# fbreitwieser/krakenuniq

Hardware: AMD Instinct MI355X
Metric: Mreads/s (150 bp) (higher is better)
Workload: dtype u64

## Files before the change

krakenuniq_amd/capi.py:

```python
from __future__ import annotations

import ctypes as C
import os

import numpy as np

_HERE = os.path.dirname(os.path.abspath(__file__))
LIB_PATH = os.environ.get("KU_LIB") or os.path.join(_HERE, "libkrakenuniq_amd.so")


def _hw_queues():
    try:
        have = int(os.environ.get("GPU_MAX_HW_QUEUES", "0"))
    except ValueError:
        have = 0
    try:
        want = int(os.environ["KU_HW_QUEUES"]) if "KU_HW_QUEUES" in os.environ else max(have, 8)
    except ValueError:
        want = max(have, 8)
    os.environ["GPU_MAX_HW_QUEUES"] = str(min(max(want, 4), 32))


_hw_queues()

# ... 231 lines not shown

    def __init__(self, kdb=None, idx=None, pairs=None, key_ct=None, k=None, offsets=None, nt=None, idx_type=2):
        self.h = C.c_void_p()
        if kdb is not None:
            _chk(lib().ku_db_open(kdb.encode(), idx.encode(), C.byref(self.h)), "ku_db_open")
        else:
            self._keep = (pairs, offsets)
            _chk(lib().ku_db_wrap(pairs.ctypes.data, key_ct, k, offsets.ctypes.data, nt, idx_type, C.byref(self.h)),
                 "ku_db_wrap")
        self.info = DbInfo()
        _chk(lib().ku_db_get_info(self.h, C.byref(self.info)), "ku_db_get_info")

    def close(self):
        if self.h and _lib is not None:
            _lib.ku_db_close(self.h)
            self.h = C.c_void_p()

    __del__ = close

    def shard_plan(self, n):
        b = np.zeros(n + 1, dtype=np.uint64)
        _chk(lib().ku_db_shard_plan(self.h, n, _p(b, u64p)), "ku_db_shard_plan")
        return b

    def chunk_plan(self, max_bytes, cap=4096):
        b = np.zeros(cap + 1, dtype=np.uint64)
        n = C.c_uint32()
        _chk(lib().ku_db_chunk_plan(self.h, max_bytes, _p(b, u64p), cap, C.byref(n)), "ku_db_chunk_plan")
        return b[:n.value + 1]

    def values(self):
        n = C.c_uint64()
        _chk(lib().ku_db_values(self.h, None, C.byref(n)), "ku_db_values")
        out = np.zeros(max(n.value, 1), dtype=np.uint32)
        n2 = C.c_uint64(len(out))
        _chk(lib().ku_db_values(self.h, _p(out, u32p), C.byref(n2)), "ku_db_values")
        return out[:n2.value]


class Tax:

    def __init__(self, path=None, ids=None, parents=None):
        self.h = C.c_void_p()
        if path is not None:
            _chk(lib().ku_tax_open(path.encode(), C.byref(self.h)), "ku_tax_open")
        else:
            ids = np.ascontiguousarray(ids, dtype=np.uint32)
            parents = np.ascontiguousarray(parents, dtype=np.uint32)
            _chk(lib().ku_tax_from_arrays(_p(ids, u32p), _p(parents, u32p), len(ids), C.byref(self.h)),
                 "ku_tax_from_arrays")

    def ids(self):
        out = np.zeros(max(int(lib().ku_tax_size(self.h)), 1), dtype=np.uint32)
        _chk(lib().ku_tax_ids(self.h, _p(out, u32p)), "ku_tax_ids")
        return out[:int(lib().ku_tax_size(self.h))]

    def close(self):
        if self.h and _lib is not None:
            _lib.ku_tax_close(self.h)
            self.h = C.c_void_p()

    __del__ = close

    def parent(self, taxid):
        return lib().ku_tax_parent(self.h, taxid)

    def __len__(self):
        return lib().ku_tax_size(self.h)


class UidMap:

    def __init__(self, path=None, blocks=None):
        self.h = C.c_void_p()
        if path is not None:
            _chk(lib().ku_uid_map_open(path.encode(), C.byref(self.h)), "ku_uid_map_open")
        else:
            b = np.ascontiguousarray(blocks, dtype=np.uint32).reshape(-1)
            _chk(lib().ku_uid_map_from_blocks(_p(b, u32p), len(b) // 2, C.byref(self.h)), "ku_uid_map_from_blocks")

    def __len__(self):
        return int(lib().ku_uid_map_size(self.h))

    def close(self):
        if self.h:
            lib().ku_uid_map_close(self.h)
            self.h = C.c_void_p()

    def __del__(self):
        try:
            self.close()
        except Exception:
            pass


def resolve_uids(tax, uid_map, rle, lens, k, n_threads=1):
    runs = np.ascontiguousarray(rle["runs"], dtype=np.uint32)
    roff = np.ascontiguousarray(rle["run_off"], dtype=np.uint64)
    rcnt = np.ascontiguousarray(rle["run_cnt"], dtype=np.uint32)
    lens = np.ascontiguousarray(lens, dtype=np.uint32)
    calls = np.zeros(max(len(lens), 1), dtype=np.uint32)
    _chk(lib().ku_resolve_uids(tax.h, uid_map.h, runs.ctypes.data, _p(roff, u64p), _p(rcnt, u32p), _p(lens, u32p), len(lens), k,
                               n_threads, _p(calls, u32p)), "ku_resolve_uids")
    return calls[:len(lens)]


class Ctx:

    def __init__(self, device=0, borrowed=None):
        self._keep = []
        self._borrowed = borrowed is not None
        if borrowed is not None:
            self.h = C.c_void_p(borrowed)
            return
        self.h = C.c_void_p()
        _chk(lib().ku_ctx_create(device, C.byref(self.h)), "ku_ctx_create")

    def close(self):
        if getattr(self, "h", None) and _lib is not None and not getattr(self, "_borrowed", False):
            _lib.ku_ctx_destroy(self.h)
        self.h = C.c_void_p()

    __del__ = close

    def load_db(self, db: Db, bin_lo=0, bin_hi=None):
        if bin_hi is None:
            bin_hi = db.info.n_bins
        _chk(lib().ku_ctx_load_db(self.h, db.h, bin_lo, bin_hi), "ku_ctx_load_db")

    def swap_shard(self, db: Db, bin_lo, bin_hi):
        _chk(lib().ku_ctx_swap_shard(self.h, db.h, int(bin_lo), int(bin_hi)), "ku_ctx_swap_shard")

    def prefetch_shard(self, db: Db, bin_lo, bin_hi):
        _chk(lib().ku_ctx_prefetch_shard(self.h, db.h, int(bin_lo), int(bin_hi)), "ku_ctx_prefetch_shard")

    def batch(self, buf, off, lens):
        return Batch(self, buf, off, lens)

    def add_db(self, db: Db):
        _chk(lib().ku_ctx_add_db(self.h, db.h), "ku_ctx_add_db")

    def adopt_db(self, d_pairs_ptr, n_pairs, d_offsets_ptr, k, nt, idx_type=2, bin_lo=0, bin_hi=None, keep=None):
        if bin_hi is None:
            bin_hi = 4 ** nt
        self._keep.append(keep)
        _chk(lib().ku_ctx_adopt_db(self.h, d_pairs_ptr, n_pairs, d_offsets_ptr, k, nt, idx_type, bin_lo, bin_hi),
             "ku_ctx_adopt_db")

    def db_layout(self):
        h, b = C.c_uint32(), C.c_uint64()
        _chk(lib().ku_ctx_db_layout(self.h, C.byref(h), C.byref(b)), "ku_ctx_db_layout")
        return {"hash": bool(h.value), "resident_bytes": b.value}

    def db_values(self):
        n = C.c_uint64()
        _chk(lib().ku_ctx_db_values(self.h, None, C.byref(n)), "ku_ctx_db_values")
        out = np.zeros(max(n.value, 1), dtype=np.uint32)
        n2 = C.c_uint64(len(out))
        _chk(lib().ku_ctx_db_values(self.h, _p(out, u32p), C.byref(n2)), "ku_ctx_db_values")
        return out[:n2.value]

    def set_taxonomy(self, tax: Tax, all_values=None):
        if all_values is None:
            _chk(lib().ku_ctx_set_taxonomy(self.h, tax.h, None, 0), "ku_ctx_set_taxonomy")
        else:
            v = np.ascontiguousarray(all_values, dtype=np.uint32)
            _chk(lib().ku_ctx_set_taxonomy(self.h, tax.h, _p(v, u32p), len(v)), "ku_ctx_set_taxonomy")

    def count_taxons(self, db_index=0):
        n = C.c_uint64()
        _chk(lib().ku_ctx_count_taxons_db(self.h, db_index, None, None, C.byref(n)), "ku_ctx_count_taxons_db")
        t = np.zeros(max(n.value, 1), dtype=np.uint32)
        c = np.zeros(max(n.value, 1), dtype=np.uint64)
        n2 = C.c_uint64(len(t))
        _chk(lib().ku_ctx_count_taxons_db(self.h, db_index, _p(t, u32p), _p(c, u64p), C.byref(n2)), "ku_ctx_count_taxons_db")
        return t[:n2.value], c[:n2.value]

    def enable_exact(self, capacity_log2=20):
        _chk(lib().ku_ctx_enable_exact(self.h, capacity_log2), "ku_ctx_enable_exact")

    def exact_counts(self):
        d = CountsDims()
        _chk(lib().ku_counts_dims_get(self.h, C.byref(d)), "ku_counts_dims_get")
        out = np.zeros(d.n_slots, dtype=np.uint64)
        _chk(lib().ku_counts_export_exact(self.h, _p(out, u64p)), "ku_counts_export_exact")
        return out

    def reset_counts(self):
        _chk(lib().ku_ctx_reset_counts(self.h), "ku_ctx_reset_counts")

    def enable_sparse(self, work_unit_nt=500000, global_log2=0):
        _chk(lib().ku_ctx_enable_sparse(self.h, work_unit_nt, global_log2), "ku_ctx_enable_sparse")

    def disable_sparse(self):
        _chk(lib().ku_ctx_disable_sparse(self.h), "ku_ctx_disable_sparse")

    def sparse_close_unit(self):
        _chk(lib().ku_sparse_close_unit(self.h), "ku_sparse_close_unit")

    def sparse_state(self):
        return lib().ku_ctx_sparse_state(self.h)

    def report(self, tax: "Tax", counts_paths=(), flags=0):
        out, n = C.c_void_p(), C.c_size_t()
        paths = (C.c_char_p * len(counts_paths))(*[p.encode() for p in counts_paths])
        if flags:
            _chk(lib().ku_ctx_report_cols(self.h, tax.h, paths, len(counts_paths), flags, C.byref(out), C.byref(n)), "ku_ctx_report_cols")
        else:
            _chk(lib().ku_ctx_report(self.h, tax.h, paths, len(counts_paths), C.byref(out), C.byref(n)), "ku_ctx_report")
        s = C.string_at(out, n.value).decode()
        lib().ku_free(out)
        return s

    def sparse_export(self):
        d = CountsDims()
        _chk(lib().ku_counts_dims_get(self.h, C.byref(d)), "ku_counts_dims_get")
        flags = np.zeros(d.n_slots, dtype=np.uint8)
        n = C.c_uint64()
        _chk(lib().ku_sparse_export(self.h, _p(flags, u8p), None, C.byref(n)), "ku_sparse_export")
        pairs = np.zeros(max(n.value, 1), dtype=np.uint64)
        n2 = C.c_uint64(len(pairs))
        _chk(lib().ku_sparse_export(self.h, _p(flags, u8p), _p(pairs, u64p), C.byref(n2)), "ku_sparse_export")
        return flags, pairs[:n2.value]

    def classify_batch(self, buf, off, lens, flags=0, min_hits=1, want_taxa=True):
        arr = np.frombuffer(buf, dtype=np.uint8) if isinstance(buf, (bytes, bytearray)) else buf
        off = np.ascontiguousarray(off, dtype=np.uint64)
        lens = np.ascontiguousarray(lens, dtype=np.uint32)
        n = len(lens)
        calls = np.zeros(max(n, 1), dtype=np.uint32)
        hits = np.zeros(max(n, 1), dtype=np.uint32)
        taxa = np.zeros(max(len(arr), 1), dtype=np.uint32) if want_taxa else None
        o = Opts(flags, min_hits, 0, 0)
        _chk(lib().ku_classify_batch(self.h, arr.ctypes.data, len(arr), _p(off, u64p), _p(lens, u32p), n, C.byref(o),
                                     _p(calls, u32p), _p(taxa, u32p), _p(hits, u32p)), "ku_classify_batch")
        return {"calls": calls[:n], "taxa": taxa, "hits": hits[:n]}

    def classify_batch_rle(self, buf, off, lens, flags=0, min_hits=1, out=None):
        arr = np.frombuffer(buf, dtype=np.uint8) if isinstance(buf, (bytes, bytearray)) else buf
        off = np.ascontiguousarray(off, dtype=np.uint64)
        lens = np.ascontiguousarray(lens, dtype=np.uint32)
        n = len(lens)
        out = out or {}
        calls = out["calls"] if "calls" in out else np.zeros(max(n, 1), dtype=np.uint32)
        hits = out["hits"] if "hits" in out else np.zeros(max(n, 1), dtype=np.uint32)
        roff = out["run_off"] if "run_off" in out else np.zeros(max(n, 1), dtype=np.uint64)
        rcnt = out["run_cnt"] if "run_cnt" in out else np.zeros(max(n, 1), dtype=np.uint32)
        o = Opts(flags, min_hits, 0, 0)
        total = C.c_uint64()
        _chk(lib().ku_classify_batch_rle(self.h, arr.ctypes.data, len(arr), _p(off, u64p), _p(lens, u32p), n, C.byref(o),
                                         _p(calls, u32p), _p(hits, u32p), _p(roff, u64p), _p(rcnt, u32p),
                                         C.byref(total)), "ku_classify_batch_rle")
        runs = out.get("runs")
        if runs is None or len(runs) < total.value:
            runs = np.zeros((max(total.value, 1), 2), dtype=np.uint32)
        _chk(lib().ku_fetch_runs(self.h, runs.ctypes.data, total.value), "ku_fetch_runs")
        return {"calls": calls[:n], "hits": hits[:n], "runs": runs[:total.value], "run_off": roff[:n], "run_cnt": rcnt[:n]}

    def replace_calls(self, new_calls):
        nc = np.ascontiguousarray(new_calls, dtype=np.uint32)
        dropped = C.c_uint64()
        _chk(lib().ku_ctx_replace_calls(self.h, _p(nc, u32p), len(nc), C.byref(dropped)), "ku_ctx_replace_calls")
        return int(dropped.value)

    def lookup_device(self, d_seqs, n_bytes, d_taxa, flags=0, stream=None):
        o = Opts(flags, 1, 0, 0)
        _chk(lib().ku_lookup_device(self.h, d_seqs, n_bytes, C.byref(o), d_taxa, stream), "ku_lookup_device")

    def resolve_device(self, d_seqs, d_off, d_len, n_reads, d_calls, d_taxa, d_hits=None, flags=0, min_hits=1,
                       max_read_len=0, stream=None):
        o = Opts(flags, min_hits, max_read_len, 0)
        _chk(lib().ku_resolve_device(self.h, d_seqs, d_off, d_len, n_reads, C.byref(o), d_calls, d_taxa, d_hits,
                                     stream), "ku_resolve_device")

    def rle_enqueue(self, buf, off, lens, flags=0, min_hits=1, runs_cap=0, out=None):
        arr = np.ascontiguousarray(np.frombuffer(buf, dtype=np.uint8) if isinstance(buf, (bytes, bytearray)) else buf, dtype=np.uint8)
        off = np.ascontiguousarray(off, dtype=np.uint64)
        lens = np.ascontiguousarray(lens, dtype=np.uint32)
        n = len(off)
        out = out or {}
        job = {"arr": arr, "off": off, "lens": lens, "n": n,
               "calls": out["calls"] if "calls" in out else np.zeros(max(n, 1), np.uint32),
               "hits": out["hits"] if "hits" in out else np.zeros(max(n, 1), np.uint32),
               "run_off": out["run_off"] if "run_off" in out else np.zeros(max(n, 1), np.uint64),
               "run_cnt": out["run_cnt"] if "run_cnt" in out else np.zeros(max(n, 1), np.uint32)}
        o = Opts(flags, min_hits, 0, 0)
        job["runs"] = out["runs"] if "runs" in out else (np.zeros((runs_cap, 2), np.uint32) if runs_cap else None)
        rc = len(job["runs"]) if job["runs"] is not None else 0
        _chk(lib().ku_classify_batch_rle_enqueue(self.h, arr.ctypes.data, len(arr), _p(off, u64p), _p(lens, u32p), n, C.byref(o),
                                                 _p(job["calls"], u32p), _p(job["hits"], u32p), _p(job["run_off"], u64p),
                                                 _p(job["run_cnt"], u32p), job["runs"].ctypes.data if rc else None, rc),
             "ku_classify_batch_rle_enqueue")
        return job

    def rle_finish(self, job):
        total = C.c_uint64(0)
        _chk(lib().ku_classify_batch_rle_finish(self.h, C.byref(total)), "ku_classify_batch_rle_finish")
        if job.get("runs") is not None and total.value <= lib().ku_classify_batch_rle_copied(self.h):
            runs = job["runs"][:total.value]
        else:
            runs = np.zeros((total.value, 2), np.uint32)
            _chk(lib().ku_fetch_runs(self.h, runs.ctypes.data, total.value), "ku_fetch_runs")
        n = job.get("n", len(job.get("calls", ())))
        return {"calls": job["calls"][:n], "hits": job["hits"][:n], "run_off": job["run_off"][:n], "run_cnt": job["run_cnt"][:n], "runs": runs}

    def rle_in_flight(self):
# ... 533 lines not shown
```

krakenuniq_amd/csrc/ku_api.cpp:

```cpp
#include "ku_build.h"
#include "ku_ctx.h"

static thread_local std::string g_last_error;
void ku_set_error(const std::string &s) { g_last_error = s; }

extern "C" const char *ku_strerror(int status) {
  switch (status) {
    case KU_OK: return "ok";
    case KU_EINVAL: return "invalid argument";
    case KU_EDATA: return "malformed database / index / taxonomy data";
    case KU_ENOINPUT: return "cannot open input";
    case KU_ENOMEM: return "out of memory";
    case KU_EHIP: return "HIP runtime error or no usable gfx950 device";
    case KU_ESTATE: return "call order violated";
    case KU_EUNSUP: return "not supported by this build";
    default: return "unknown status";
  }
}
extern "C" const char *ku_last_error(void) { return g_last_error.c_str(); }
extern "C" int ku_abi_version(void) { return KU_ABI_VERSION; }
extern "C" int ku_device_count(void) {
  int n = 0;
  if (hipGetDeviceCount(&n) != hipSuccess) return 0;
  return n;
// ... 131 lines not shown
  uint64_t last_dbx = 0;
  while (idx_pos < nb) {
    uint64_t first = idx_pos, count = nb - idx_pos;
    const uint64_t orig = idx_pos, data0 = db->offsets[orig];
    while (count > 0) {
      uint64_t step = count / 2, it = first + step;
      uint64_t size_index = (it + 1 - orig) * 8;
      uint64_t size_data = (db->offsets[it + 1] - data0) * ps;
      if (size_index + size_data + 8 <= max_bytes) { first = it + 1; count -= step + 1; }
      else count = step;
    }
    if (first == idx_pos) return fail(KU_EINVAL, "preload size too small for the largest minimizer bin");
    idx_pos = first;
    uint64_t dbx = db->offsets[idx_pos];
    if (dbx == last_dbx) continue;
    last_dbx = dbx;
    ++n;
    if (n <= cap) bounds[n] = idx_pos;
  }
  *n_chunks = n;
  return n <= cap ? KU_OK : fail(KU_EINVAL, "ku_db_chunk_plan: bounds array too small");
}

int ku_db_raw(const ku_db *db, const uint8_t **pairs, const uint64_t **offsets) {
  if (!db || !pairs || !offsets) return KU_EINVAL;
  *pairs = db->pairs;
  *offsets = db->offsets;
  return KU_OK;
}

extern "C" int ku_db_values(const ku_db *db, uint32_t *out, uint64_t *n) {
  if (!db || !n) return fail(KU_EINVAL, "ku_db_values: null argument");
  std::lock_guard<std::mutex> lk(db->values_mu);
  if (!db->values_ready) {
    const uint64_t np = db->info.key_ct, ps = db->info.key_len + 4, kl = db->info.key_len;
    constexpr uint32_t SMALL = 1u << 26;
    std::vector<std::atomic<uint64_t>> bits(SMALL / 64);
    for (auto &w : bits) w.store(0, std::memory_order_relaxed);
    unsigned nthr = std::max(1u, std::min(16u, std::thread::hardware_concurrency()));
    if (np < (1u << 20)) nthr = 1;
    std::vector<std::vector<uint32_t>> large(nthr);
    std::vector<std::thread> team;
    for (unsigned t = 0; t < nthr; ++t)
      team.emplace_back([&, t] {
        const uint64_t lo = np * t / nthr, hi = np * (t + 1) / nthr;
        uint32_t last = 0;
        for (uint64_t i = lo; i < hi; ++i) {
          uint32_t v;
          memcpy(&v, db->pairs + i * ps + kl, 4);
          if (v == last) continue;
          last = v;
          if (v >= SMALL) {
            large[t].push_back(v);
            if (large[t].size() >= (1u << 20)) {
              std::sort(large[t].begin(), large[t].end());
              large[t].erase(std::unique(large[t].begin(), large[t].end()), large[t].end());
            }
            continue;
          }
          std::atomic<uint64_t> &w = bits[v >> 6];
          const uint64_t m = 1ull << (v & 63);
          if (!(w.load(std::memory_order_relaxed) & m)) w.fetch_or(m, std::memory_order_relaxed);
        }
      });
    for (auto &th : team) th.join();
    std::vector<uint32_t> &vals = db->values;
    for (uint64_t wi = 0; wi < bits.size(); ++wi) {
      uint64_t w = bits[wi].load(std::memory_order_relaxed);
      if (wi == 0) w &= ~1ull;
      while (w) {
        vals.push_back((uint32_t)(wi * 64 + (uint64_t)__builtin_ctzll(w)));
        w &= w - 1;
      }
    }
    const size_t n_small = vals.size();
    for (auto &l : large) vals.insert(vals.end(), l.begin(), l.end());
    std::sort(vals.begin() + n_small, vals.end());
    vals.erase(std::unique(vals.begin() + n_small, vals.end()), vals.end());
    db->values_ready = true;
  }
  const uint64_t count = db->values.size();
  if (out) {
    if (count > *n) return fail(KU_EINVAL, "ku_db_values: output array too small");
    memcpy(out, db->values.data(), count * 4);
  }
  *n = count;
  return KU_OK;
}

extern "C" int ku_tax_open(const char *path, ku_tax **out) {
  if (!path || !out) return fail(KU_EINVAL, "ku_tax_open: null argument");
  *out = nullptr;
  FILE *f = fopen(path, "r");
  if (!f) return fail(KU_ENOINPUT, std::string("unable to open taxonomy index file ") + path);
  ku_tax *t = new ku_tax();
  char *line = nullptr;
  size_t lcap = 0;
  ssize_t ll;
  while ((ll = getline(&line, &lcap, f)) > 0) {
    if (line[ll - 1] == '\n') line[--ll] = 0;
    if (ll == 0) continue;
    char *p = line, *end;
    unsigned long id = strtoul(p, &end, 10);
    if (end == p) continue;
    p = end;
    unsigned long par = strtoul(p, &end, 10);
    if (end == p) continue;
    p = end;
    if (*p) ++p;
    char *tab = strchr(p, '\t');
    std::string name, rank;
    if (tab) { name.assign(p, tab - p); rank.assign(tab + 1); } else name.assign(p);
    if ((uint32_t)id > 1 && id == par) {
      free(line); fclose(f); delete t;
      return fail(KU_EDATA, "taxDB: the parent of " + std::to_string(id) + " is itself");
    }
    t->add((uint32_t)id, (uint32_t)par, name, rank);
  }
  free(line);
  fclose(f);
  t->add(0, 0, "unclassified", "no rank");
  t->finish();
  *out = t;
  return KU_OK;
}

extern "C" int ku_tax_from_arrays(const uint32_t *ids, const uint32_t *parents, uint64_t n, ku_tax **out) {
  if (!out || (n && (!ids || !parents))) return fail(KU_EINVAL, "ku_tax_from_arrays: null argument");
  ku_tax *t = new ku_tax();
  for (uint64_t i = 0; i < n; ++i) t->add(ids[i], parents[i], "", "");
  t->add(0, 0, "unclassified", "no rank");
  t->finish();
  *out = t;
  return KU_OK;
}
extern "C" void ku_tax_close(ku_tax *t) { delete t; }
extern "C" uint64_t ku_tax_size(const ku_tax *t) { return t ? t->ids.size() : 0; }
extern "C" int ku_tax_ids(const ku_tax *t, uint32_t *ids) {
  if (!t || (!ids && !t->ids.empty())) return fail(KU_EINVAL, "ku_tax_ids: null argument");
  if (!t->ids.empty()) memcpy(ids, t->ids.data(), t->ids.size() * 4);
  return KU_OK;
}
extern "C" uint32_t ku_tax_parent(const ku_tax *t, uint32_t taxid) {
  if (!t || taxid == 0) return KU_AMBIG;
  auto it = t->row.find(taxid);
  return it == t->row.end() ? KU_AMBIG : t->parent_map[it->second];
}

hipStream_t ku_ctx_stream_of(ku_ctx *ctx) { return ctx->stream; }
unsigned long long *ku_ctx_exact_unique_of(ku_ctx *ctx) { return ctx->d_exact_unique; }
int ku_ctx_device_of(const ku_ctx *ctx) { return ctx->device; }
int ku_ctx_cus_of(const ku_ctx *ctx) { return ctx->n_cu; }
uint32_t ku_ctx_k_of(const ku_ctx *ctx) { return ctx->m.db.k; }

int ctx_activate(ku_ctx *ctx) {
  if (hipSetDevice(ctx->device) != hipSuccess) return fail(KU_EHIP, "hipSetDevice failed");
  return KU_OK;
}

extern "C" int ku_ctx_create(int device, ku_ctx **out) {
  if (!out) return fail(KU_EINVAL, "ku_ctx_create: null argument");
  *out = nullptr;
  KU_TRY(ku_check_device(device));
  hipDeviceProp_t prop;
  HIP_TRY(hipGetDeviceProperties(&prop, device));
  if (strncmp(prop.gcnArchName, "gfx950", 6) != 0)
    return fail(KU_EHIP, std::string("device is ") + prop.gcnArchName + ", this library is built for gfx950 only");
  ku_ctx *ctx = new ku_ctx();
  ctx->device = device;
  ctx->n_cu = prop.multiProcessorCount > 0 ? prop.multiProcessorCount : 256;
  HIP_TRY(hipSetDevice(device));
  HIP_TRY(hipStreamCreateWithFlags(&ctx->stream, hipStreamNonBlocking));
  HIP_TRY(hipMalloc((void **)&ctx->d_scalar, 128));
  if (const char *e = getenv("KU_LAYOUT")) ctx->hash_layout = strcmp(e, "sorted") != 0;
  if (const char *e = getenv("KU_LOAD_FACTOR")) {
    double f = atof(e);
    if (f >= 0.05 && f <= 0.9) { ctx->load_factor = f; ctx->load_factor_set = true; }
  }
  *out = ctx;
  return KU_OK;
}

void store_free(DbStore &d) {
  if (d.d_table) (void)hipFree(d.d_table);
  if (d.db_owned && d.d_pairs) (void)hipFree(d.d_pairs);
  if (d.offsets_owned && d.d_offsets) (void)hipFree(d.d_offsets);
  d = DbStore{};
}
void ctx_drop_count_cache(ku_ctx *ctx) {
  ctx->count_cache.clear();
  ctx->count_cache_store = ctx->count_cache_pairs = nullptr;
  ctx->count_cache_lines = 0;
}
static void ctx_free_db(ku_ctx *ctx) {
  ctx_drop_count_cache(ctx);
  if (ctx->pf.valid) store_free(ctx->pf.store);
  ctx->pf.valid = false;
  store_free(ctx->m);
  for (DbStore &e : ctx->extra) store_free(e);
  ctx->extra.clear();
  ctx->db_loaded = false;
}
void ctx_free_sparse(ku_ctx *ctx) {
  KuSparseDev &d = ctx->sp.dev;
  for (void *p : {(void *)d.l_key, (void *)d.l_first, (void *)d.u_key, (void *)d.u_distinct, (void *)d.u_last, (void *)d.u_maxfirst,
                  (void *)d.g_key, (void *)d.dense, (void *)d.err, (void *)ctx->sp.d_counters})
    if (p) (void)hipFree(p);
  for (DevBuf *b : {&ctx->sp.unit, &ctx->sp.carry_l, &ctx->sp.carry_u, &ctx->sp.out, &ctx->sp.u_cnt, &ctx->sp.u_flag, &ctx->sp.list, &ctx->sp.tail_row,
                    &ctx->sp.t_seqs, &ctx->sp.t_off, &ctx->sp.t_len, &ctx->sp.t_taxa, &ctx->sp.t_unit})
    b->release();
  ctx->sp = ku_ctx::Sparse{};
}
int sparse_give_up(ku_ctx *ctx, hipStream_t also) {
  (void)ctx_sync_all_streams(ctx);
  if (also) (void)hipStreamSynchronize(also);
  (void)hipGetLastError();
  ctx_free_sparse(ctx);
  ctx->sp.gave_up = true;
  return KU_OK;
}
static void ctx_free_tax(ku_ctx *ctx) {
  for (uint32_t **p : {&ctx->d_node_parent, &ctx->d_node_slot, &ctx->d_node_taxid, &ctx->d_slot_node, &ctx->d_slot_taxid,
                       &ctx->d_slot_anc_off, &ctx->d_slot_anc}) {
    if (*p) (void)hipFree(*p);
    *p = nullptr;
  }
  if (ctx->cnt.registers) (void)hipFree(ctx->cnt.registers);
  if (ctx->cnt.hll_floor) (void)hipFree(ctx->cnt.hll_floor);
  if (ctx->cnt.n_kmers) (void)hipFree(ctx->cnt.n_kmers);
  if (ctx->cnt.n_reads) (void)hipFree(ctx->cnt.n_reads);
  if (ctx->d_exact_set) (void)hipFree(ctx->d_exact_set);
  if (ctx->d_exact_unique) (void)hipFree(ctx->d_exact_unique);
  ctx->d_exact_set = ctx->d_exact_unique = nullptr;
  ctx->exact_mask = 0;
  ctx_free_sparse(ctx);
  ctx->cnt = KuCountsDev{};
  ctx->tax_set = false;
}

int ctx_sync_all_streams(ku_ctx *ctx) {
  int st = KU_OK;
  for (hipStream_t s : {ctx->stream, ctx->k_streams[0], ctx->k_streams[1], ctx->h2d_stream, ctx->d2h_stream, ctx->fetch_stream, ctx->pf.stream})
    if (s && hipStreamSynchronize(s) != hipSuccess && st == KU_OK) st = fail(KU_EHIP, "ku_ctx_synchronize: a stream of the context failed");
  return st;
}

extern "C" void ku_ctx_destroy(ku_ctx *ctx) {
  if (!ctx) return;
  rle_times_print();
  (void)hipSetDevice(ctx->device);
  (void)ctx_sync_all_streams(ctx);
  ctx_free_db(ctx);
  ctx_free_tax(ctx);
  for (DevBuf *b : {&ctx->b_seqs, &ctx->b_off, &ctx->b_len, &ctx->b_calls, &ctx->b_taxa, &ctx->b_hits, &ctx->b_ws, &ctx->b_runs,
                    &ctx->b_roff, &ctx->b_rcnt})
    b->release();
  if (ctx->d_scalar) (void)hipFree(ctx->d_scalar);
  if (ctx->pf.d_scalar) (void)hipFree(ctx->pf.d_scalar);
  if (ctx->pf.stream) (void)hipStreamDestroy(ctx->pf.stream);
  for (RleJob &j : ctx->rle) j.release();
  if (ctx->h2d_stream) (void)hipStreamDestroy(ctx->h2d_stream);
  if (ctx->d2h_stream) (void)hipStreamDestroy(ctx->d2h_stream);
  for (hipStream_t &ks : ctx->k_streams) if (ks) { (void)hipStreamDestroy(ks); ks = nullptr; }
  if (ctx->main_ev) (void)hipEventDestroy(ctx->main_ev);
  if (ctx->fetch_stream) (void)hipStreamDestroy(ctx->fetch_stream);
  if (ctx->stream) (void)hipStreamDestroy(ctx->stream);
  delete ctx;
}

static int store_scan_values(ku_ctx *ctx, DbStore &d) {
  d.values.clear();
  uint32_t *d_bitmap = nullptr, *d_list = nullptr, *d_count = ctx->d_scalar;
  const uint32_t cap = 1u << 24;
  HIP_TRY(hipMalloc((void **)&d_bitmap, 1ull << 29));
  if (hipMalloc((void **)&d_list, (size_t)cap * 4) != hipSuccess) { (void)hipFree(d_bitmap); return fail(KU_ENOMEM, "hipMalloc values list"); }
  int st = KU_OK;
  uint32_t count = 0;
  if (hipMemsetAsync(d_bitmap, 0, 1ull << 29, ctx->stream) != hipSuccess ||
      hipMemsetAsync(d_count, 0, 4, ctx->stream) != hipSuccess)
    st = fail(KU_EHIP, "memset failed");
  if (st == KU_OK) st = ku_launch_mark_values(d.d_pairs, d.db.n_pairs, d_bitmap, ctx->stream);
  if (st == KU_OK) st = ku_launch_collect_values(d_bitmap, d_list, cap, d_count, ctx->stream);
  if (st == KU_OK && hipMemcpyAsync(&count, d_count, 4, hipMemcpyDeviceToHost, ctx->stream) != hipSuccess) st = fail(KU_EHIP, "memcpy failed");
  if (st == KU_OK && hipStreamSynchronize(ctx->stream) != hipSuccess) st = fail(KU_EHIP, "value scan kernel failed");
  if (st == KU_OK && count > cap) st = fail(KU_EUNSUP, "more than 2^24 distinct taxids in the database");
  if (st == KU_OK) {
    d.values.resize(count);
    if (count && hipMemcpy(d.values.data(), d_list, (size_t)count * 4, hipMemcpyDeviceToHost) != hipSuccess) st = fail(KU_EHIP, "memcpy failed");
    std::sort(d.values.begin(), d.values.end());
    if (!d.values.empty() && d.values[0] == 0) d.values.erase(d.values.begin());
  }
  (void)hipFree(d_bitmap);
  (void)hipFree(d_list);
  return st;
}

static void fill_db_dev(DbStore &d, uint64_t n_pairs, uint64_t pair_base, uint32_t k, uint32_t nt, uint32_t idx_type,
                        uint64_t bin_lo, uint64_t bin_hi) {
  d.db.pairs = d.d_pairs;
  d.db.table = nullptr;
  d.db.n_lines = 0;
  d.db.offsets = d.d_offsets;
  d.db.pair_base = pair_base;
  d.db.n_pairs = n_pairs;
  d.db.bin_lo = bin_lo;
  d.db.bin_hi = bin_hi;
  d.db.k = k;
  d.db.nt = nt;
  d.db.xor_mask = idx_type == 1 ? 0u : ku_index2_xor_mask(nt);
}

int store_upload(ku_ctx *ctx, DbStore &d, const ku_db *db, uint64_t bin_lo, uint64_t bin_hi, bool scan_values, hipStream_t stream) {
  if (!stream) stream = ctx->stream;
  const uint64_t p0 = db->offsets[bin_lo], p1 = db->offsets[bin_hi], np = p1 - p0;
  const uint32_t kl = db->info.key_len, ps = kl + 4;
  HIP_TRY(hipMalloc((void **)&d.d_pairs, std::max<uint64_t>(np, 1) * 12));
  d.db_owned = true;
  if (kl == 8) {
    if (np) HIP_TRY(hipMemcpy(d.d_pairs, db->pairs + p0 * 12, np * 12, hipMemcpyHostToDevice));
  } else if (np) {
    void *d_raw = nullptr;
    HIP_TRY(hipMalloc(&d_raw, np * ps));
    hipError_t e = hipMemcpy(d_raw, db->pairs + p0 * ps, np * ps, hipMemcpyHostToDevice);
    int st = e == hipSuccess ? ku_launch_repack((const uint8_t *)d_raw, np, kl, d.d_pairs, stream) : KU_EHIP;
    if (st == KU_OK && hipStreamSynchronize(stream) != hipSuccess) st = KU_EHIP;
    (void)hipFree(d_raw);
    if (st != KU_OK) return fail(st, "pair repack failed");
  }
  const uint64_t no = bin_hi - bin_lo + 1;
  HIP_TRY(hipMalloc((void **)&d.d_offsets, no * 8));
  d.offsets_owned = true;
  HIP_TRY(hipMemcpy(d.d_offsets, db->offsets + bin_lo, no * 8, hipMemcpyHostToDevice));
  fill_db_dev(d, np, p0, db->info.k, db->info.nt, db->info.idx_type, bin_lo, bin_hi);
  return scan_values ? store_scan_values(ctx, d) : KU_OK;
}

extern "C" int ku_ctx_load_db(ku_ctx *ctx, const ku_db *db, uint64_t bin_lo, uint64_t bin_hi) {
  if (!ctx || !db) return fail(KU_EINVAL, "ku_ctx_load_db: null argument");
  KU_TRY(rle_idle(ctx, "ku_ctx_load_db"));
  if (bin_lo > bin_hi || bin_hi > db->info.n_bins) return fail(KU_EINVAL, "bin range out of bounds");
  KU_TRY(ctx_activate(ctx));
  ctx_free_tax(ctx);
  ctx_free_db(ctx);
  KU_TRY(store_upload(ctx, ctx->m, db, bin_lo, bin_hi));
  ctx->db_loaded = true;
  return KU_OK;
}

bool store_whole(const DbStore &d) { return d.db.bin_lo == 0 && d.db.bin_hi == (1ull << (2 * d.db.nt)); }

extern "C" int ku_ctx_add_db(ku_ctx *ctx, const ku_db *db) {
  if (!ctx || !db) return fail(KU_EINVAL, "ku_ctx_add_db: null argument");
  KU_TRY(rle_idle(ctx, "ku_ctx_add_db"));
  if (!ctx->db_loaded) return fail(KU_ESTATE, "load the first database before adding further ones");
  if (ctx->tax_set) return fail(KU_ESTATE, "add every database before the taxonomy is set");
  if (db->info.k != ctx->m.db.k)
    return fail(KU_EINVAL, "different k-mer sizes in the databases: " + std::to_string(ctx->m.db.k) + " vs " + std::to_string(db->info.k));
  if (!store_whole(ctx->m)) return fail(KU_EUNSUP, "hierarchical multi-database runs need the first database resident as a whole");
  if (ctx->extra.size() >= 7) return fail(KU_EUNSUP, "at most 8 databases");
  KU_TRY(ctx_activate(ctx));
  ctx->extra.emplace_back();
  int st = store_upload(ctx, ctx->extra.back(), db, 0, db->info.n_bins);
  if (st != KU_OK) { store_free(ctx->extra.back()); ctx->extra.pop_back(); }
  return st;
}

extern "C" int ku_ctx_adopt_db(ku_ctx *ctx, void *d_pairs, uint64_t n_pairs, const uint64_t *d_offsets, uint32_t k,
                               uint32_t nt, uint32_t idx_type, uint64_t bin_lo, uint64_t bin_hi) {
  if (!ctx || (!d_pairs && n_pairs) || !d_offsets) return fail(KU_EINVAL, "ku_ctx_adopt_db: null argument");
  KU_TRY(rle_idle(ctx, "ku_ctx_adopt_db"));
  if (k < 1 || k > 31 || nt < 1 || nt > 15 || nt > k || (idx_type != 1 && idx_type != 2) || bin_lo > bin_hi ||
      bin_hi > (1ull << (2 * nt)))
    return fail(KU_EINVAL, "ku_ctx_adopt_db: bad geometry");
  KU_TRY(ctx_activate(ctx));
  ctx_free_tax(ctx);
  ctx_free_db(ctx);
  ctx->m.d_pairs = (uint32_t *)d_pairs;
  ctx->m.d_offsets = const_cast<uint64_t *>(d_offsets);
  uint64_t pair_base = 0;
  HIP_TRY(hipMemcpy(&pair_base, d_offsets, 8, hipMemcpyDeviceToHost));
  fill_db_dev(ctx->m, n_pairs, pair_base, k, nt, idx_type, bin_lo, bin_hi);
  ctx->db_loaded = true;
  return store_scan_values(ctx, ctx->m);
}

extern "C" int ku_ctx_db_layout(ku_ctx *ctx, uint32_t *is_hash, uint64_t *resident_bytes) {
  if (!ctx) return fail(KU_EINVAL, "null context");
  if (!ctx->db_loaded) return fail(KU_ESTATE, "no database loaded");
  const bool hash = ctx->m.db.table != nullptr;
  if (is_hash) *is_hash = hash ? 1u : 0u;
  if (resident_bytes)
    *resident_bytes = (hash ? ctx->m.db.n_lines * 128 : ctx->m.db.n_pairs * 12) + (ctx->m.db.bin_hi - ctx->m.db.bin_lo + 1) * 8;
  return KU_OK;
}

static std::vector<uint32_t> ctx_all_values(const ku_ctx *ctx) {
  std::vector<uint32_t> v(ctx->m.values);
  for (const DbStore &e : ctx->extra) v.insert(v.end(), e.values.begin(), e.values.end());
  std::sort(v.begin(), v.end());
  v.erase(std::unique(v.begin(), v.end()), v.end());
  return v;
}

extern "C" int ku_ctx_db_values(ku_ctx *ctx, uint32_t *out, uint64_t *n) {
  if (!ctx || !n) return fail(KU_EINVAL, "ku_ctx_db_values: null argument");
  if (!ctx->db_loaded) return fail(KU_ESTATE, "no database loaded");
  const std::vector<uint32_t> v = ctx_all_values(ctx);
  if (out) {
    if (*n < v.size()) return fail(KU_EINVAL, "output array too small");
    if (!v.empty()) memcpy(out, v.data(), v.size() * 4);
  }
  *n = v.size();
  return KU_OK;
}

template <typename T> static int upload(T **dst, const std::vector<T> &src) {
  HIP_TRY(hipMalloc((void **)dst, std::max<size_t>(src.size(), 1) * sizeof(T)));
  if (!src.empty()) HIP_TRY(hipMemcpy(*dst, src.data(), src.size() * sizeof(T), hipMemcpyHostToDevice));
  return KU_OK;
}

int store_finalize(ku_ctx *ctx, DbStore &d, hipStream_t stream, uint32_t *d_scalar) {
  if (!stream) stream = ctx->stream;
  if (!d_scalar) d_scalar = ctx->d_scalar;
  HIP_TRY(hipMemsetAsync(d_scalar, 0, 4, stream));
  KU_TRY(ku_launch_remap_values(d.d_pairs, d.db.n_pairs, ctx->d_slot_taxid, ctx->tax.n_slots, d_scalar, stream));
  uint32_t err = 0;
  HIP_TRY(hipMemcpyAsync(&err, d_scalar, 4, hipMemcpyDeviceToHost, stream));
  HIP_TRY(hipStreamSynchronize(stream));
  if (err) return fail(KU_EDATA, "internal: " + std::to_string(err) + " DB values missing from the slot table");
  d.hash_layout = ctx->hash_layout;
  if (d.hash_layout) {
    uint64_t n_lines = 0;
    size_t free_b = 0, total_b = 0;
    (void)hipMemGetInfo(&free_b, &total_b);
    std::vector<double> chain;
    if (ctx->load_factor_set) chain.push_back(ctx->load_factor);
    else if ((double)d.db.n_pairs / 0.2 / 8.0 * 128.0 <= 0.4 * (double)free_b) chain.push_back(0.2);
    for (double lf : {0.3, 0.45, 0.6, 0.8})
      if (chain.empty() || lf > chain.back()) chain.push_back(lf);
    for (double lf : chain) {
      n_lines = (uint64_t)((double)d.db.n_pairs / lf / 8.0) + 1;
      if (n_lines >= (1ull << 32)) { n_lines = 0; continue; }
      if (hipMalloc(&d.d_table, n_lines * 128) == hipSuccess) { d.table_lines = n_lines; break; }
      (void)hipGetLastError();
      d.d_table = nullptr;
      n_lines = 0;
    }
    if (!d.d_table) d.hash_layout = false;
  }
  d.slot_counts.clear();
  if (d.hash_layout && d.db.n_pairs) {
    unsigned long long *d_c = nullptr;
    const uint32_t ns = ctx->tax.n_slots;
    if (hipMalloc((void **)&d_c, (size_t)ns * 8) == hipSuccess) {
      std::vector<unsigned long long> h(ns);
      const bool ok = hipMemsetAsync(d_c, 0, (size_t)ns * 8, stream) == hipSuccess &&
                      ku_launch_count_slots(d.d_pairs, d.db.n_pairs, d_c, ns, stream) == KU_OK &&
                      hipMemcpyAsync(h.data(), d_c, (size_t)ns * 8, hipMemcpyDeviceToHost, stream) == hipSuccess &&
                      hipStreamSynchronize(stream) == hipSuccess;
      (void)hipFree(d_c);
      if (ok) d.slot_counts.swap(h);
      else (void)hipGetLastError();
    } else (void)hipGetLastError();
  }
  if (d.hash_layout) {
    const uint64_t n_lines = d.table_lines;
    unsigned long long *d_dup = (unsigned long long *)(d_scalar + 2);
    HIP_TRY(hipMemsetAsync(d_dup, 0, 8, stream));
    KU_TRY(ku_launch_build_table(d.d_pairs, d.db.n_pairs, d.d_table, n_lines, d.db.k, d.db.nt, d.db.xor_mask, d_dup,
                                 stream));
    unsigned long long dup = 0;
    HIP_TRY(hipMemcpyAsync(&dup, d_dup, 8, hipMemcpyDeviceToHost, stream));
    HIP_TRY(hipStreamSynchronize(stream));
    d.n_dup = dup;
    d.db.table = (const uint4 *)d.d_table;
    d.db.n_lines = n_lines;
    if (d.db_owned) (void)hipFree(d.d_pairs);
    d.d_pairs = nullptr;
    d.db_owned = false;
    d.db.pairs = nullptr;
  }
  return KU_OK;
}

extern "C" int ku_ctx_set_taxonomy(ku_ctx *ctx, const ku_tax *tax, const uint32_t *all_values, uint64_t n_values) {
  if (!ctx || !tax) return fail(KU_EINVAL, "ku_ctx_set_taxonomy: null argument");
  KU_TRY(rle_idle(ctx, "ku_ctx_set_taxonomy"));
  if (!ctx->db_loaded) return fail(KU_ESTATE, "load a database before the taxonomy");
  if (ctx->tax_set) return fail(KU_ESTATE, "taxonomy already set for this shard (values are remapped once)");
  KU_TRY(ctx_activate(ctx));
  std::vector<uint32_t> slots;
  slots.push_back(0);
  if (all_values) {
    for (uint64_t i = 0; i < n_values; ++i) if (all_values[i]) slots.push_back(all_values[i]);
    std::sort(slots.begin() + 1, slots.end());
    slots.erase(std::unique(slots.begin(), slots.end()), slots.end());
    const std::vector<uint32_t> mine = ctx_all_values(ctx);
    if (!std::includes(slots.begin(), slots.end(), mine.begin(), mine.end()))
      return fail(KU_EINVAL, "all_values does not cover this shard's values");
  } else {
    const std::vector<uint32_t> mine = ctx_all_values(ctx);
    slots.insert(slots.end(), mine.begin(), mine.end());
  }
  std::vector<uint32_t> nodes(tax->ids);
  nodes.insert(nodes.end(), slots.begin(), slots.end());
  nodes.push_back(0);
  nodes.push_back(1);
  std::sort(nodes.begin(), nodes.end());
  nodes.erase(std::unique(nodes.begin(), nodes.end()), nodes.end());
  auto node_of = [&](uint32_t taxid) { return (uint32_t)(std::lower_bound(nodes.begin(), nodes.end(), taxid) - nodes.begin()); };
  std::vector<uint32_t> node_parent(nodes.size(), 0), node_slot(nodes.size(), 0), slot_node(slots.size(), 0);
  for (size_t i = 0; i < tax->ids.size(); ++i) {
    uint32_t p = tax->parent_map[i];
    if (tax->ids[i] != 0 && p != 0) node_parent[node_of(tax->ids[i])] = node_of(p);
  }
  for (size_t s = 1; s < slots.size(); ++s) {
    uint32_t nd = node_of(slots[s]);
    slot_node[s] = nd;
    node_slot[nd] = (uint32_t)s;
  }
  std::vector<uint32_t> anc_off(slots.size() + 1, 0), anc;
  for (size_t s = 0; s < slots.size(); ++s) {
    anc_off[s] = (uint32_t)anc.size();
    if (s == 0) continue;
    uint32_t node = slot_node[s];
    for (uint32_t guard = 0; node > 0 && guard < 4096; ++guard) {
      if (node_slot[node]) anc.push_back(node_slot[node]);
      node = node_parent[node];
    }
  }
  anc_off[slots.size()] = (uint32_t)anc.size();
  ctx_free_tax(ctx);
  ctx->h_node_taxid = nodes;
  ctx->h_slot_taxid = slots;
  KU_TRY(upload(&ctx->d_node_parent, node_parent));
  KU_TRY(upload(&ctx->d_node_slot, node_slot));
  KU_TRY(upload(&ctx->d_node_taxid, nodes));
  KU_TRY(upload(&ctx->d_slot_node, slot_node));
  KU_TRY(upload(&ctx->d_slot_taxid, slots));
  KU_TRY(upload(&ctx->d_slot_anc_off, anc_off));
  KU_TRY(upload(&ctx->d_slot_anc, anc));
  ctx->tax.node_parent = ctx->d_node_parent;
  ctx->tax.node_slot = ctx->d_node_slot;
  ctx->tax.node_taxid = ctx->d_node_taxid;
  ctx->tax.slot_node = ctx->d_slot_node;
  ctx->tax.slot_taxid = ctx->d_slot_taxid;
  ctx->tax.slot_anc_off = ctx->d_slot_anc_off;
  ctx->tax.slot_anc = ctx->d_slot_anc;
  ctx->tax.n_nodes = (uint32_t)nodes.size();
  ctx->tax.n_slots = (uint32_t)slots.size();
  ctx->tax.node_one = 1;
  if (hipMalloc((void **)&ctx->cnt.registers, (size_t)slots.size() * KU_HLL_M) != hipSuccess ||
      hipMalloc((void **)&ctx->cnt.hll_floor, slots.size() * 4) != hipSuccess ||
      hipMalloc((void **)&ctx->cnt.n_kmers, slots.size() * 8) != hipSuccess ||
      hipMalloc((void **)&ctx->cnt.n_reads, nodes.size() * 8) != hipSuccess) {
    (void)hipGetLastError();
    ctx_free_tax(ctx);
    return fail(KU_ENOMEM, "device memory for the per-taxon counters");
  }
  int st = store_finalize(ctx, ctx->m);
  for (size_t e = 0; st == KU_OK && e < ctx->extra.size(); ++e) st = store_finalize(ctx, ctx->extra[e]);
  if (st != KU_OK) {
    ctx_free_tax(ctx);
    ctx->db_loaded = false;
    return st;
  }
  ctx->tax_set = true;
  return ku_ctx_reset_counts(ctx);
}

extern "C" int ku_ctx_reset_counts(ku_ctx *ctx) {
  if (!ctx || !ctx->tax_set) return fail(KU_ESTATE, "taxonomy not set");
  KU_TRY(rle_idle(ctx, "ku_ctx_reset_counts"));
  KU_TRY(ctx_activate(ctx));
  HIP_TRY(hipMemsetAsync(ctx->cnt.registers, 0, (size_t)ctx->tax.n_slots * KU_HLL_M, ctx->stream));
  HIP_TRY(hipMemsetAsync(ctx->cnt.hll_floor, 0, (size_t)ctx->tax.n_slots * 4, ctx->stream));
  HIP_TRY(hipMemsetAsync(ctx->cnt.n_kmers, 0, (size_t)ctx->tax.n_slots * 8, ctx->stream));
  HIP_TRY(hipMemsetAsync(ctx->cnt.n_reads, 0, (size_t)ctx->tax.n_nodes * 8, ctx->stream));
  if (ctx->d_exact_set) {
    HIP_TRY(hipMemsetAsync(ctx->d_exact_set, 0, (ctx->exact_mask + 1) * 8, ctx->stream));
    HIP_TRY(hipMemsetAsync(ctx->d_exact_unique, 0, (size_t)ctx->tax.n_slots * 8, ctx->stream));
    HIP_TRY(hipMemsetAsync(ctx->d_scalar + 6, 0, 4, ctx->stream));
  }
  if (ctx->m.seen_dirty && ctx->m.d_table) {
    KU_TRY(ku_launch_seen(2, ctx->m.d_table, ctx->m.db.n_lines, KuSparseDev{}, nullptr, ctx->stream));
    ctx->m.seen_dirty = false;
  }
  if (ctx->sp.on) {
    KuSparseDev &d = ctx->sp.dev;
    HIP_TRY(hipMemsetAsync(d.g_key, 0, (d.g_mask + 1) * 8, ctx->stream));
    HIP_TRY(hipMemsetAsync(d.dense, 0, (size_t)ctx->tax.n_slots * 4, ctx->stream));
    HIP_TRY(hipMemsetAsync(d.err, 0, 4, ctx->stream));
    HIP_TRY(hipMemsetAsync(ctx->sp.d_counters, 0, 32, ctx->stream));
    ctx->sp.acc_nt = 0;
    ctx->sp.open = false;
    ctx->sp.n_carry_l = ctx->sp.n_carry_u = 0;
    ctx->sp.g_count = 0;
    ctx->sp.tail_open = false;
    ctx->sp.tail_text.clear();
    ctx->sp.tail_len.clear();
  }
  HIP_TRY(hipStreamSynchronize(ctx->stream));
  return KU_OK;
}

int sparse_pass(ku_ctx *ctx, const void *d_seqs, const uint64_t *d_off, const uint32_t *d_len, const uint64_t *h_off,
                       const uint32_t *h_len, uint64_t n_reads, uint64_t n_bytes, const uint32_t *d_taxa, uint32_t quick_min_hits,
                       hipStream_t s);

extern "C" int ku_ctx_enable_exact(ku_ctx *ctx, uint32_t capacity_log2) {
  KU_TRY(check_ready(ctx));
  KU_TRY(rle_idle(ctx, "ku_ctx_enable_exact"));
  if (capacity_log2 < 10 || capacity_log2 > 36) return fail(KU_EINVAL, "ku_ctx_enable_exact: capacity_log2 out of range (10..36)");
  if (ctx->d_exact_set) { (void)hipFree(ctx->d_exact_set); ctx->d_exact_set = nullptr; }
  if (ctx->d_exact_unique) { (void)hipFree(ctx->d_exact_unique); ctx->d_exact_unique = nullptr; }
  ctx->exact_mask = 0;
  const uint64_t cells = 1ull << capacity_log2;
  if (hipMalloc((void **)&ctx->d_exact_set, cells * 8) != hipSuccess) { ctx->d_exact_set = nullptr; return fail(KU_ENOMEM, "device memory for the exact k-mer set"); }
  if (hipMalloc((void **)&ctx->d_exact_unique, (size_t)ctx->tax.n_slots * 8) != hipSuccess) {
    (void)hipFree(ctx->d_exact_set);
    ctx->d_exact_set = ctx->d_exact_unique = nullptr;
    return fail(KU_ENOMEM, "device memory for the exact counters");
  }
// ... 80 lines not shown
```

krakenuniq_amd/csrc/ku_ctx.h:

```cpp
#pragma once
#include <fcntl.h>
#include <sys/mman.h>
#include <sys/stat.h>
#include <time.h>
#include <unistd.h>

#include <algorithm>
#include <atomic>
#include <mutex>
#include <thread>
#include <cstdio>
#include <cstdlib>
#include <cstring>
#include <string>
#include <unordered_map>
#include <vector>

#include "ku_host.h"
#include "ku_internal.h"

void ku_set_error(const std::string &s);
static inline int fail(int code, const std::string &msg) {
  ku_set_error(msg);
  return code;
}
#define HIP_TRY(expr)                                                                          \
  do {                                                                                         \
    hipError_t e_ = (expr);                                                                    \
    if (e_ != hipSuccess)                                                                      \
      return fail(e_ == hipErrorOutOfMemory ? KU_ENOMEM : KU_EHIP,                             \
                  std::string(#expr) + ": " + hipGetErrorString(e_));                          \
  } while (0)
#define KU_TRY(expr)            \
  do {                          \
    int s_ = (expr);            \
    if (s_ != KU_OK) return s_; \
  } while (0)

static inline int ensure_stream(hipStream_t &s) { if (!s) HIP_TRY(hipStreamCreateWithFlags(&s, hipStreamNonBlocking)); return KU_OK; }
static inline int ensure_event(hipEvent_t &e, unsigned flags = hipEventDisableTiming) { if (!e) HIP_TRY(hipEventCreateWithFlags(&e, flags)); return KU_OK; }
static inline uint32_t ku_max_kmers(uint32_t k, uint32_t len) { return len >= k ? len - k + 1 : 0; }

struct ku_db {
  const uint8_t *pairs = nullptr;
  const uint64_t *offsets = nullptr;
  ku_db_info info{};
  void *map_kdb = nullptr, *map_idx = nullptr;
  size_t map_kdb_sz = 0, map_idx_sz = 0;
  mutable std::mutex values_mu;
  mutable std::vector<uint32_t> values;
  mutable bool values_ready = false;
};

struct DevBuf {
  void *p = nullptr;
  size_t cap = 0;
  int reserve(size_t bytes) {
    if (bytes <= cap) return KU_OK;
    if (p) (void)hipFree(p);
    p = nullptr; cap = 0;
    size_t want = bytes + bytes / 4 + 256;
    if (hipMalloc(&p, want) != hipSuccess) {
      if (hipMalloc(&p, bytes) != hipSuccess) { p = nullptr; return KU_ENOMEM; }
      want = bytes;
    }
    cap = want;
    return KU_OK;
  }
  void release() { if (p) (void)hipFree(p); p = nullptr; cap = 0; }
};

struct PinBuf {
  void *p = nullptr;
  size_t cap = 0;
  int reserve(size_t bytes) {
    if (bytes <= cap) return KU_OK;
    if (p) (void)hipHostFree(p);
    p = nullptr; cap = 0;
    const size_t want = bytes + bytes / 4 + 256;
    if (hipHostMalloc(&p, want, hipHostMallocDefault) != hipSuccess) { (void)hipGetLastError(); p = nullptr; return KU_ENOMEM; }
    cap = want;
    return KU_OK;
  }
  void release() { if (p) (void)hipHostFree(p); p = nullptr; cap = 0; }
};

struct RleBatch {
  const char *seqs;
  uint64_t n_bytes;
  const uint64_t *seq_off;
  const uint32_t *seq_len;
  uint64_t n_reads;
  ku_opts o;
  uint32_t max_n;
  bool monotonic;
  uint32_t *calls, *hits, *run_cnt;
  uint64_t *run_off;
  ku_run *runs;
  uint64_t runs_cap;
};

struct RleJob {
  DevBuf seqs, off, len, calls, runs, roff, rcnt, ws, unit, u_cnt, u_flag;
  PinBuf pin;
  PinBuf pin_unit;
  unsigned long long *d_counter = nullptr;
  hipEvent_t kernels_done = nullptr, done = nullptr;
  hipEvent_t t_k0 = nullptr, t_k1 = nullptr;
  std::vector<hipEvent_t> seg_events;
  bool busy = false;
  bool settled = false;
  bool runs_in_ctx = false;
  uint64_t runs_copied = 0;
  uint64_t n_runs = 0;
  RleBatch b{};
  uint64_t runs_cap = 0;
  bool sparse = false;
  bool cont_carry = false;
  bool cont_tail = false;
  bool open_after = false;
  uint32_t n_units = 0;
  uint64_t kmers = 0;
  uint64_t acc_after = 0;
  std::vector<uint64_t> unit_first_read;
  std::vector<char> tail_text;
  std::vector<uint32_t> tail_len;
  int reserve(uint64_t n_bytes, uint64_t n_reads, uint64_t runs_cap_, uint64_t ws_bytes, size_t n_seg, bool sparse_, uint64_t units, uint64_t n_slots) {
    if (seqs.reserve(n_bytes + 16) || off.reserve(n_reads * 8) || len.reserve(n_reads * 4) || calls.reserve(n_reads * 4) ||
        runs.reserve(runs_cap_ * 8) || roff.reserve(n_reads * 8) || rcnt.reserve(n_reads * 4) || ws.reserve(ws_bytes))
      return fail(KU_ENOMEM, "device batch buffers");
    units = std::max<uint64_t>(units, 1);
    if (sparse_ && (pin_unit.reserve(n_reads * 4) || unit.reserve(n_reads * 4) || u_cnt.reserve(std::max<uint64_t>(units * n_slots, 1) * 4) ||
                    u_flag.reserve((units + 3) & ~3ull)))
      return fail(KU_ENOMEM, "device memory for the work-unit counters");
    if (pin.reserve(64 + (size_t)units + 64)) return fail(KU_ENOMEM, "page-locked memory for the batch totals");
    KU_TRY(ensure_event(done));
    KU_TRY(ensure_event(kernels_done));
    seg_events.resize(std::max(seg_events.size(), n_seg), nullptr);
    for (hipEvent_t &e : seg_events) KU_TRY(ensure_event(e));
    return KU_OK;
  }
  void release() {
    for (DevBuf *d : {&seqs, &off, &len, &calls, &runs, &roff, &rcnt, &ws, &unit, &u_cnt, &u_flag}) d->release();
    pin.release();
    pin_unit.release();
    for (hipEvent_t *e : {&kernels_done, &done, &t_k0, &t_k1}) { if (*e) (void)hipEventDestroy(*e); *e = nullptr; }
    for (hipEvent_t e : seg_events) if (e) (void)hipEventDestroy(e);
    seg_events.clear();
  }
};

struct DbStore {
  bool db_owned = false, offsets_owned = false;
  bool hash_layout = true;
  bool seen_dirty = false;
  void *d_table = nullptr;
  uint64_t n_dup = 0;
  uint64_t table_lines = 0;
  uint32_t *d_pairs = nullptr;
  uint64_t *d_offsets = nullptr;
  KuDbDev db{};
  std::vector<uint32_t> values;
  std::vector<unsigned long long> slot_counts;
};

struct ku_ctx {
  int device = 0;
  int n_cu = 256;
  hipStream_t stream = nullptr;
  bool db_loaded = false, tax_set = false;
  bool hash_layout = true;
  double load_factor = 0.2;
  bool load_factor_set = false;
  DbStore m;
  std::vector<DbStore> extra;
  std::vector<uint32_t> h_node_taxid, h_slot_taxid;
  uint32_t *d_node_parent = nullptr, *d_node_slot = nullptr, *d_node_taxid = nullptr, *d_slot_node = nullptr,
           *d_slot_taxid = nullptr, *d_slot_anc_off = nullptr, *d_slot_anc = nullptr;
  KuTaxDev tax{};
  KuCountsDev cnt{};
  DevBuf b_seqs, b_off, b_len, b_calls, b_taxa, b_hits, b_ws, b_runs, b_roff, b_rcnt;
  hipStream_t h2d_stream = nullptr, d2h_stream = nullptr, fetch_stream = nullptr;
  hipStream_t k_streams[2] = {nullptr, nullptr};
  hipEvent_t main_ev = nullptr;
  hipEvent_t prev_kernels_done = nullptr;
  uint32_t *d_scalar = nullptr;
  RleJob rle[KU_RLE_MAX_IN_FLIGHT];
  int rle_head = 0, rle_in_flight = 0;
  const void *fetch_runs_src = nullptr;
  const void *last_calls_dev = nullptr;
  uint64_t last_runs_copied = 0;
  std::vector<unsigned long long> count_cache;
  const void *count_cache_store = nullptr, *count_cache_pairs = nullptr;
  uint64_t count_cache_lines = 0;
  uint64_t n_runs = 0;
  unsigned long long *d_exact_set = nullptr, *d_exact_unique = nullptr;
  uint64_t exact_mask = 0;
  struct Prefetch {
    bool valid = false;
    const ku_db *db = nullptr;
    uint64_t bin_lo = 0, bin_hi = 0;
    DbStore store;
    hipStream_t stream = nullptr;
    uint32_t *d_scalar = nullptr;
  } pf;
  struct Sparse {
    bool on = false;
    uint64_t unit_nt = 500000;
    uint64_t acc_nt = 0;
    bool open = false;
    KuSparseDev dev{};
    unsigned long long *d_counters = nullptr;
    DevBuf unit, carry_l, carry_u, out;
    DevBuf u_cnt, u_flag, list;
    uint64_t n_carry_l = 0, n_carry_u = 0, cap_carry_l = 0, cap_carry_u = 0;
    uint64_t g_count = 0;
    bool gave_up = false;
    bool tail_open = false;
    std::vector<char> tail_text;
    std::vector<uint32_t> tail_len;
    DevBuf tail_row;
    DevBuf t_seqs, t_off, t_len, t_taxa, t_unit;
  } sp;
};


struct ku_batch {
  ku_ctx *ctx = nullptr;
  uint64_t n_bytes = 0, n_reads = 0;
  uint32_t max_len = 0;
  bool finished = false;
  void *d_seqs = nullptr;
  uint64_t *d_off = nullptr;
  uint32_t *d_len = nullptr, *d_taxa = nullptr;
  std::vector<uint64_t> h_off;
  std::vector<uint32_t> h_len;
};

int ctx_activate(ku_ctx *ctx);
int ctx_sync_all_streams(ku_ctx *ctx);
void store_free(DbStore &d);
void ctx_drop_count_cache(ku_ctx *ctx);
void ctx_free_sparse(ku_ctx *ctx);
int sparse_give_up(ku_ctx *ctx, hipStream_t also = nullptr);
int store_upload(ku_ctx *ctx, DbStore &d, const ku_db *db, uint64_t bin_lo, uint64_t bin_hi, bool scan_values = true, hipStream_t stream = nullptr);
bool store_whole(const DbStore &d);
int store_finalize(ku_ctx *ctx, DbStore &d, hipStream_t stream = nullptr, uint32_t *d_scalar = nullptr);
int sparse_reserve_global(ku_ctx *ctx, uint64_t incoming, hipStream_t s);
int sparse_pass_tables(ku_ctx *ctx, uint64_t n_entries, KuSparseDev *view, hipStream_t s);
int sparse_pass(ku_ctx *ctx, const void *d_seqs, const uint64_t *d_off, const uint32_t *d_len, const uint64_t *h_off, const uint32_t *h_len, uint64_t n_reads, uint64_t n_bytes, const uint32_t *d_taxa, uint32_t quick_min_hits, hipStream_t s);
int sparse_close_open_unit(ku_ctx *ctx);
int ctx_seen_harvest(ku_ctx *ctx);
int check_ready(ku_ctx *ctx);
int classify_device_impl(ku_ctx *ctx, const void *d_seqs, uint64_t n_bytes, const uint64_t *d_seq_off, const uint32_t *d_seq_len, uint64_t n_reads, const ku_opts *opts, uint32_t *d_calls, uint32_t *d_taxa, uint32_t *d_hits, void *stream, const uint64_t *h_off, const uint32_t *h_len);
int rle_and_fetch(ku_ctx *ctx, const uint32_t *d_taxa, const uint64_t *d_off, const uint32_t *d_len, uint64_t n_reads, uint64_t runs_cap, bool quick, uint32_t *calls, uint32_t *hits, uint64_t *run_off, uint32_t *run_cnt, uint64_t *n_runs);
int sparse_tail_to_carry(ku_ctx *ctx);
int sparse_tail_close(ku_ctx *ctx);
void rle_times_print();
int rle_idle(const ku_ctx *ctx, const char *who);
int rle_drain_batches(ku_ctx *ctx);
```

krakenuniq_amd/csrc/ku_device.h:

```cpp
#pragma once
#include "ku_internal.h"

#define KU_CT_LOG2 9
#define KU_CT_CAP (1 << KU_CT_LOG2)

__device__ __forceinline__ uint64_t ku_fmix64(uint64_t key) {
  key += 1;
  key ^= key >> 33;
  key *= 0xff51afd7ed558ccdULL;
  key ^= key >> 33;
  key *= 0xc4ceb9fe1a85ec53ULL;
  key ^= key >> 33;
  return key;
}

__device__ __forceinline__ uint64_t ku_revcomp64(uint64_t x, uint32_t n) {
  uint64_t r = __builtin_bitreverse64(x);
  r = ((r >> 1) & 0x5555555555555555ULL) | ((r & 0x5555555555555555ULL) << 1);
  return (~r) >> (64 - 2 * n);
}
__device__ __forceinline__ uint32_t ku_revcomp32(uint32_t x, uint32_t n) {
  uint32_t r = __builtin_bitreverse32(x);
  r = ((r >> 1) & 0x55555555u) | ((r & 0x55555555u) << 1);
  return (~r) >> (32 - 2 * n);
// ... 38 lines not shown
}
template <int LOG2 = KU_CT_LOG2>
__device__ __forceinline__ void ku_ct_clear(uint32_t *ct_key, uint32_t *ct_cnt, uint32_t *used) {
  for (int i = threadIdx.x; i < (1 << LOG2); i += blockDim.x) {
    ct_key[i] = 0;
    ct_cnt[i] = 0;
  }
  if (threadIdx.x == 0) *used = 0;
}
template <int LOG2 = KU_CT_LOG2>
__device__ __forceinline__ void ku_ct_flush(uint32_t *ct_key, uint32_t *ct_cnt, unsigned long long *global) {
  for (int i = threadIdx.x; i < (1 << LOG2); i += blockDim.x) {
    uint32_t kk = ct_key[i];
    if (kk) atomicAdd(&global[kk - 1], (unsigned long long)ct_cnt[i]);
  }
}
template <int LOG2 = KU_CT_LOG2>
__device__ __forceinline__ void ku_ct_maybe_flush(uint32_t *ct_key, uint32_t *ct_cnt, uint32_t *used,
                                                  unsigned long long *global) {
  if (*used > (1u << LOG2) / 2) {
    __syncthreads();
    ku_ct_flush<LOG2>(ct_key, ct_cnt, global);
    __syncthreads();
    ku_ct_clear<LOG2>(ct_key, ct_cnt, used);
    __syncthreads();
  }
}

__device__ __forceinline__ uint8_t *ku_hll_locate(uint8_t *registers, uint32_t slot, uint64_t h, uint32_t &rank) {
  const uint32_t idx = (uint32_t)(h >> (64 - KU_HLL_P));
  const uint64_t rest = (h << KU_HLL_P) | (1ull << (KU_HLL_P - 1));
  rank = (uint32_t)__builtin_clzll(rest) + 1;
  return registers + (size_t)slot * KU_HLL_M + idx;
}
__device__ __forceinline__ void ku_hll_raise(uint8_t *r, uint32_t seen, uint32_t rank) {
  if (seen < rank) {
    uint32_t *w = (uint32_t *)((uintptr_t)r & ~(uintptr_t)3);
    uint32_t sh = ((uint32_t)(uintptr_t)r & 3u) * 8;
    uint32_t old = __hip_atomic_load(w, __ATOMIC_RELAXED, __HIP_MEMORY_SCOPE_AGENT);
    while (((old >> sh) & 0xffu) < rank) {
      uint32_t nw = (old & ~(0xffu << sh)) | (rank << sh);
      uint32_t prev = atomicCAS(w, old, nw);
      if (prev == old) break;
      old = prev;
    }
  }
}
__device__ __forceinline__ void ku_hll_update(uint8_t *registers, uint32_t slot, uint64_t h) {
  uint32_t rank;
  uint8_t *r = ku_hll_locate(registers, slot, h, rank);
  ku_hll_raise(r, *r, rank);
}

#define KS_PPRIME 25
__device__ __forceinline__ uint32_t ks_encode(uint64_t h) {
  const uint32_t idx = (uint32_t)(h >> (64 - KS_PPRIME)) << (32 - KS_PPRIME);
  if ((uint32_t)(idx << KU_HLL_P) == 0) {
    const uint64_t rest = h << KS_PPRIME;
    const uint32_t add = rest ? (uint32_t)__builtin_clzll(rest) + 1 : (64 - KS_PPRIME + 1);
    return idx | (add << 1) | 1u;
  }
  return idx;
}

__device__ __forceinline__ uint64_t ks_mix(unsigned long long k) {
  k ^= k >> 31;
  k *= 0x9E3779B97F4A7C15ULL;
  k ^= k >> 29;
  return k;
}

__device__ __forceinline__ bool ks_g_insert(unsigned long long *g_key, uint64_t g_mask, uint32_t slot, uint32_t enc, uint32_t *err) {
  const unsigned long long gk = ((unsigned long long)(slot + 1) << 32) | enc;
  uint64_t h = ks_mix(gk) & g_mask;
  for (uint32_t probe = 0; probe < 4096; ++probe) {
    const unsigned long long old = atomicCAS(&g_key[h], 0ull, gk);
    if (old == 0ull) return true;
    if (old == gk) return false;
    h = (h + 1) & g_mask;
  }
  atomicOr(err, 4u);
  return false;
}

struct __attribute__((packed, aligned(4))) KuPair {
  uint32_t key_lo, key_hi, slot;
};

__device__ __forceinline__ void ku_pack_dword(uint32_t d, uint32_t &codes8, uint32_t &amb4) {
  const uint32_t c = d & 0xDFDFDFDFu;
  const uint32_t x = ((c >> 1) ^ (c >> 2)) & 0x03030303u;
  codes8 = (x * 0x40100401u) >> 24;
  const uint32_t b0 = x & 0x01010101u, b1 = (x >> 1) & 0x01010101u, b01 = b0 & b1;
  const uint32_t expect = 0x41414141u + (b0 << 1) + (b1 << 2) + (b1 << 1) + (b01 << 3) + (b01 << 1) + b01;
  const uint32_t diff = c ^ expect;
  const uint32_t nz = (((diff & 0x7F7F7F7Fu) + 0x7F7F7F7Fu) | diff) & 0x80808080u;
  amb4 = (((nz >> 7) * 0x08040201u) >> 24) & 0xFu;
}

__device__ __forceinline__ void ku_pack_byte(uint32_t b, uint32_t j, uint32_t &word, uint32_t &amb) {
  uint32_t c = b & 0xDFu;
  uint32_t code = ((c >> 1) ^ (c >> 2)) & 3u;
  uint32_t valid = (c == 'A') | (c == 'C') | (c == 'G') | (c == 'T');
  word |= code << (30 - 2 * j);
  amb |= (valid ^ 1u) << (15 - j);
}

#define KU_LINE_DWORDS 32
#define KU_LINE_SLOTS 8
#define KU_LINE_ENTRY0 4
#define KU_LINE_SEEN0 28
__device__ __forceinline__ void ku_seen_mark(const uint32_t *line, uint32_t entry) {
  reinterpret_cast<uint8_t *>(const_cast<uint32_t *>(line) + KU_LINE_SEEN0)[entry] = 1;
}
__device__ __forceinline__ uint32_t ku_table_tag(uint64_t h) {
  const uint32_t t = (uint32_t)(h >> 28) & 0x7FFFu;
  return t ? t : 1u;
}
#ifdef KU_TAG_FIELDWISE
__device__ __forceinline__ uint32_t ku_tag_dword(uint32_t i) { return i >> 1; }
__device__ __forceinline__ uint32_t ku_tag_shift(uint32_t i) { return (i & 1u) * 16u; }
__device__ __forceinline__ uint32_t ku_tag_matches(uint4 h4, uint32_t tag) {
  uint32_t m = 0;
  m |= ((h4.x & 0x7FFFu) == tag) << 0;
  m |= ((h4.x >> 16) == tag) << 1;
  m |= ((h4.y & 0xFFFFu) == tag) << 2;
  m |= ((h4.y >> 16) == tag) << 3;
  m |= ((h4.z & 0xFFFFu) == tag) << 4;
  m |= ((h4.z >> 16) == tag) << 5;
  m |= ((h4.w & 0xFFFFu) == tag) << 6;
  m |= ((h4.w >> 16) == tag) << 7;
  return m;
}
#else
__device__ __forceinline__ uint32_t ku_tag_dword(uint32_t i) { return i & 3u; }
__device__ __forceinline__ uint32_t ku_tag_shift(uint32_t i) { return (i >> 2) * 16u; }
__device__ __forceinline__ uint32_t ku_pk_min_u16(uint32_t a, uint32_t b) {
  uint32_t r;
  asm("v_pk_min_u16 %0, %1, %2" : "=v"(r) : "v"(a), "v"(b));
  return r;
}
__device__ __forceinline__ uint32_t ku_tag_matches(uint4 h4, uint32_t tag) {
  const uint32_t t2 = tag | (tag << 16), one = 0x00010001u;
  const uint32_t e0 = ku_pk_min_u16((h4.x & 0xFFFF7FFFu) ^ t2, one);
  const uint32_t e1 = ku_pk_min_u16(h4.y ^ t2, one), e2 = ku_pk_min_u16(h4.z ^ t2, one), e3 = ku_pk_min_u16(h4.w ^ t2, one);
  const uint32_t differ = ((((e3 << 1) | e2) << 1 | e1) << 1) | e0;
  const uint32_t m = ~differ & 0x000F000Fu;
  return (m | (m >> 12)) & 0xFFu;
}
#endif
__device__ __forceinline__ bool ku_line_spilled(uint4 h4) { return (h4.x & 0x8000u) != 0; }

#define KU_FLANK 8
#ifndef KU_OFFCLASS
#define KU_OFFCLASS 4
#endif

__device__ __forceinline__ uint32_t ku_key_shift(uint32_t m) { return m > 13 ? 2 * m - 26 : 0; }
#define KU_PK_KEYSHIFT 6
__device__ __forceinline__ uint32_t ku_pk_make(uint32_t value, uint32_t key_shift, bool fwd_le) {
  return ((value >> key_shift) << KU_PK_KEYSHIFT) | (uint32_t)fwd_le;
}
__device__ __forceinline__ uint32_t ku_pk_combine(uint32_t own, uint32_t nb, uint32_t s, bool &tie) {
  nb += s << 1;
  tie |= (own ^ nb) < (1u << KU_PK_KEYSHIFT);
  return min(own, nb);
}
__device__ __forceinline__ uint32_t ku_pk_combine_overlap(uint32_t own, uint32_t nb, uint32_t s, bool &tie) {
  nb += s << 1;
  tie |= ((own ^ nb) - 2u) < (1u << KU_PK_KEYSHIFT) - 2u;
  return min(own, nb);
}
__device__ __forceinline__ uint32_t ku_anchor_exact(const uint32_t *raw, uint32_t w, uint32_t key_shift, bool is_fwd,
                                                    uint32_t &a, uint32_t &bin) {
  const int32_t j0 = is_fwd ? 0 : (int32_t)w - 1, dj = is_fwd ? 1 : -1;
  uint32_t best = 0xFFFFFFFFu, mn = 0xFFFFFFFFu;
  a = 0;
  for (uint32_t t = 0; t < w; ++t) {
    const uint32_t vv = raw[j0 + dj * (int32_t)t], kk = vv >> key_shift;
    const bool lt = kk < best;
    best = lt ? kk : best;
    a = lt ? t : a;
    mn = min(mn, vv);
  }
  bin = mn;
  return best;
}
__device__ __forceinline__ uint64_t ku_locus_assemble(uint64_t canon, uint32_t key, uint32_t a, bool plus, uint32_t k,
                                                      uint32_t m) {
  const uint32_t w = k - m + 1;
  const uint32_t ap = plus ? a : w - 1 - a;
  const uint32_t left = ap, right = w - 1 - ap;
  const bool use_r = right >= left;
  const uint32_t side = use_r ? right : left;
  const uint32_t flen = (w - 1) / 2 >= KU_FLANK ? (uint32_t)KU_FLANK : (side < KU_FLANK ? side : KU_FLANK);
  const uint32_t end = use_r ? ap + m + flen : ap;
  const uint32_t seg = (uint32_t)(canon >> (2 * (plus ? k - end : end - flen))) & ((1u << (2 * flen)) - 1u);
  const uint32_t flank = flen ? (plus ? seg : ku_revcomp32(seg, flen)) : 0u;
  return ((uint64_t)key << 32) | ((uint64_t)flank << 12) | (flen << 8) | ((side / KU_OFFCLASS) << 1) | (uint32_t)use_r;
}
__device__ __forceinline__ uint64_t ku_locus_key(uint64_t c, uint32_t k, uint32_t m, uint32_t xor_mask, uint32_t &bin) {
  const uint32_t w = k - m + 1, sh = ku_key_shift(m);
  const uint32_t mask = (1u << (2 * m)) - 1u;
  uint32_t best = 0xFFFFFFFFu, mn = 0xFFFFFFFFu, a = 0;
  bool plus = true;
  for (uint32_t j = 0; j < w; ++j) {
    const uint32_t mm = (uint32_t)(c >> (2 * (k - m - j))) & mask;
    const uint32_t rcmm = ku_revcomp32(mm, m);
    const uint32_t v = (mm < rcmm ? mm : rcmm) ^ xor_mask, kk = v >> sh;
    const bool lt = kk < best;
    best = lt ? kk : best;
    a = lt ? j : a;
    plus = lt ? (mm <= rcmm) : plus;
    mn = min(mn, v);
  }
  bin = mn;
  return ku_locus_assemble(c, best, a, plus, k, m);
}
__device__ __forceinline__ uint32_t ku_locus_prehash(uint64_t locus) {
  uint32_t g = (uint32_t)locus * 0x9E3779B1u ^ __builtin_rotateleft32((uint32_t)(locus >> 32) * 0x85EBCA77u, 15);
  g ^= g >> 15;
  g *= 0x2C1B3C6Du;
  g ^= g >> 13;
  return g;
}
__device__ __forceinline__ uint64_t ku_locus_line(uint64_t locus, uint64_t n_lines) {
  return __umulhi(ku_locus_prehash(locus), (uint32_t)n_lines);
}

__device__ __forceinline__ uint32_t ku_lca_nodes(const uint32_t *__restrict__ parent, uint32_t a, uint32_t b) {
  if (a == 0 || b == 0) return a ? a : b;
  for (uint32_t guard_b = 0; b > 1 && guard_b < 4096; ++guard_b) {
    uint32_t x = a;
    for (uint32_t guard_a = 0; x > 1 && guard_a < 4096; ++guard_a) {
      if (x == b) return b;
      x = parent[x];
    }
    b = parent[b];
  }
  return 1;
}
```

krakenuniq_amd/csrc/ku_internal.h:

```cpp
#pragma once
#include <hip/hip_runtime.h>
#include <stdint.h>

#include <string>

#include "../../include/krakenuniq_amd.h"

struct KuDbDev {
  const uint32_t *pairs;
  const uint4 *table;
  uint64_t n_lines;
  const uint64_t *offsets;
  uint64_t pair_base;
  uint64_t n_pairs;
  uint64_t bin_lo, bin_hi;
  uint32_t k, nt;
  uint32_t xor_mask;
  uint32_t pad;
};

struct KuTaxDev {
  const uint32_t *node_parent;
  const uint32_t *node_slot;
  const uint32_t *node_taxid;
  const uint32_t *slot_node;
  const uint32_t *slot_taxid;
  const uint32_t *slot_anc_off;
  const uint32_t *slot_anc;
  uint32_t n_nodes, n_slots;
  uint32_t node_one;
  uint32_t pad;
};

struct KuCountsDev {
  uint8_t *registers;
  unsigned long long *n_kmers;
  unsigned long long *n_reads;
  uint32_t *hll_floor;
};

#define KU_ROUTE_CHUNK 64u
#define KU_ROUTE_CURSOR_STRIDE 16u
#define KU_ROUTE_NONE (~0ull)
#define KU_ROUTE_MISS 0xFFFFFFFEu
#define KU_ROUTE_MAX_RECORDS ((1u << 27) - 2u)
__host__ __device__ static inline uint32_t ku_route_maxn(uint32_t k, uint32_t nt) {
  const uint32_t w = k - nt + 1, room = 57u - k;
  const uint32_t a = w < room ? w : room;
  return a < 31u ? a : 31u;
}
struct KuRouteDev {
  const uint64_t *own_lo, *own_hi;
  unsigned long long *cursor;
  uint4 *q_rec;
  uint64_t cap;
  uint32_t world;
  uint32_t chunk;
};
struct KuSparseDev {
  unsigned long long *l_key;
  uint32_t *l_first;
  uint64_t l_mask;
  unsigned long long *u_key;
  uint32_t *u_distinct, *u_last, *u_maxfirst;
  uint64_t u_mask;
  unsigned long long *g_key;
  uint64_t g_mask;
  uint32_t *dense;
  uint32_t *err;
  unsigned long long *g_count;
};
#define KU_SPARSE_MAX_UNITS 16000u
#define KU_SPARSE_MAX_SLOTS (1u << 18)
int ku_launch_sparse_insert(const KuSparseDev &s, uint32_t k, const uint8_t *d_seqs, const uint64_t *d_seq_off,
                            const uint32_t *d_seq_len, const uint32_t *d_unit, uint64_t n_reads, const uint32_t *d_taxa,
                            uint32_t quick_min_hits, int n_cu, hipStream_t stream);
int ku_launch_sparse_clear(const KuSparseDev &s, hipStream_t stream);
int ku_launch_zero3(void *a, uint64_t a_dwords, void *b, uint64_t b_dwords, void *c, uint64_t c_dwords, hipStream_t stream);
int ku_launch_add_u32(uint32_t *dst, const uint32_t *src, uint64_t n, hipStream_t stream);
int ku_launch_sparse_close(const KuSparseDev &s, uint32_t n_closed, hipStream_t stream, bool skip_hits = false);
int ku_launch_sparse_carry_out(const KuSparseDev &s, uint32_t unit, unsigned long long *d_carry_l, uint32_t *d_carry_u,
                               unsigned long long *d_counters, uint64_t cap_l, uint64_t cap_u, hipStream_t stream);
int ku_launch_sparse_carry_in(const KuSparseDev &s, const unsigned long long *d_carry_l, uint64_t n_l, const uint32_t *d_carry_u,
                              uint64_t n_u, hipStream_t stream);
int ku_launch_sparse_flag_units(const uint32_t *d_u_cnt, uint64_t n_cells, uint32_t n_slots, const uint32_t *d_dense, uint8_t *d_unit_flag,
                                hipStream_t stream);
int ku_launch_sparse_insert_runs(const KuSparseDev &s, uint32_t k, const uint8_t *d_seqs, const uint64_t *d_seq_off, const uint32_t *d_seq_len,
                                 const uint32_t *d_list_read, const uint32_t *d_list_unit, const uint32_t *d_list_urow, uint64_t n_list,
                                 const void *d_runs, const uint64_t *d_run_off, const uint32_t *d_run_cnt, const uint32_t *d_slot_taxid,
                                 uint32_t n_slots, const uint32_t *d_u_cnt, int n_cu, hipStream_t stream, uint32_t pos_base = 0);
int ku_launch_sparse_rehash(const KuSparseDev &s, const unsigned long long *d_old_keys, uint64_t old_cells, hipStream_t stream);
int ku_launch_sparse_export(const KuSparseDev &s, unsigned long long *d_out, uint64_t cap, unsigned long long *d_counter,
                            hipStream_t stream);
int ku_launch_warm_scratch(int n_cu, hipStream_t stream);
int ku_launch_seen(int what, void *d_table, uint64_t n_lines, const KuSparseDev &s, unsigned long long *d_count, hipStream_t stream);

#define KU_ROLLUP_BINS 80
int ku_launch_rollup_dense(const uint8_t *d_registers, const uint32_t *d_member_off, const uint32_t *d_member_slot,
                           const uint8_t *d_clade_dense, uint32_t n_clades, uint32_t *d_hist, hipStream_t stream);
#define KU_ROLLUP_HOT 48
struct KuRollupPlan {
  const uint32_t *dense;
  const uint32_t *slot_fast;
  const uint32_t *slot_off, *slot_clade;
  const unsigned long long *set_off;
  const uint32_t *set_cells;
  const uint16_t *clade_hot;
  const uint32_t *hot_clades;
  uint32_t n_hot, pad;
  uint32_t *set, *hist, *err;
  const uint32_t *bm_of;
  uint32_t *bm;
};
int ku_launch_rollup_sparse(const unsigned long long *d_g_key, uint64_t g_cells, const KuRollupPlan &plan, int n_cu, hipStream_t stream);
int ku_launch_rollup_table(const void *d_table, uint64_t n_lines, const KuRollupPlan &plan, int n_cu, hipStream_t stream);
#define KU_BM_WORDS (1u << 20)
#define KU_BM_NONE 0xFFFFFFFFu
#define KU_FAST_SKIP 0xFFFFFFFFu
#define KU_FAST_WALK 0xFFFFFFFEu
int ku_launch_bitmap_or_children(uint32_t *d_bm, const uint32_t *d_parents, uint32_t n_parents, const uint32_t *d_child_off,
                                 const uint32_t *d_child, hipStream_t stream);
int ku_launch_bitmap_hist(const uint32_t *d_bm, const uint32_t *d_bm_clade, uint32_t n_bm, uint32_t *d_hist, hipStream_t stream);
int ku_launch_replace_calls(const uint32_t *d_old, const uint32_t *d_new, uint64_t n, const uint32_t *d_node_taxid, uint32_t n_nodes,
                            unsigned long long *d_n_reads, unsigned long long *d_dropped, hipStream_t stream);

struct ku_db;
int ku_db_raw(const ku_db *db, const uint8_t **pairs, const uint64_t **offsets);

struct ku_ctx;
int ku_ctx_sparse_on(const ku_ctx *ctx);
uint64_t ku_ctx_sparse_unit_nt(const ku_ctx *ctx);
int ku_ctx_sparse_pass_slots(ku_ctx *ctx, const void *d_seqs, const uint64_t *d_off, const uint32_t *d_len, const uint64_t *h_off,
                             const uint32_t *h_len, uint64_t n_reads, uint64_t n_bytes, const uint32_t *d_taxa, uint32_t quick_min_hits,
                             hipStream_t s);
int ku_ctx_sparse_move_open_unit(ku_ctx *src, ku_ctx *dst);
int ku_ctx_sparse_finish(ku_ctx *ctx, uint32_t *h_dense);
int ku_ctx_sparse_set_dense(ku_ctx *ctx, const uint32_t *h_dense);
int ku_ctx_sparse_absorb(ku_ctx *dst, ku_ctx *src);
int ku_launch_sparse_absorb(const KuSparseDev &s, const unsigned long long *d_keys, uint64_t n, hipStream_t stream);

int ku_ctx_route_info(const ku_ctx *ctx, uint64_t *bin_lo, uint64_t *bin_hi, int *is_hash, int *single_db);
int ku_ctx_route_scan(ku_ctx *ctx, const void *d_seqs, uint64_t n_bytes, uint32_t *d_taxa, const KuRouteDev &rt, hipStream_t s);
int ku_ctx_route_resolve_prepare(ku_ctx *ctx, const ku_opts *opts, hipStream_t s);
int ku_ctx_route_resolve(ku_ctx *ctx, const uint64_t *d_off, const uint32_t *d_len, uint64_t n_reads, const ku_opts *opts, uint32_t *d_calls,
                         uint32_t *d_taxa, uint32_t *d_hits, const uint32_t *d_kb, const uint32_t *d_ret, hipStream_t s);
int ku_ctx_route_owner(ku_ctx *ctx, const void *d_rec, uint64_t n_rec, const uint32_t *d_kb, uint32_t *d_slots, bool do_counts, hipStream_t s);
struct ku_ctx;
hipStream_t ku_ctx_stream_of(ku_ctx *ctx);
unsigned long long *ku_ctx_exact_unique_of(ku_ctx *ctx);
int ku_ctx_device_of(const ku_ctx *ctx);
int ku_ctx_cus_of(const ku_ctx *ctx);
uint32_t ku_ctx_k_of(const ku_ctx *ctx);
void ku_set_error(const std::string &s);

int ku_launch_lookup(const KuDbDev &db, const KuCountsDev &cnt, const uint8_t *d_seqs, uint64_t n_bytes,
                     uint32_t *d_taxa, bool do_counts, bool prior, bool merge_chunk, int n_cu, hipStream_t stream);
int ku_launch_route_scan(const KuDbDev &db, const uint8_t *d_seqs, uint64_t n_bytes, uint32_t *d_taxa, const KuRouteDev &rt, int n_cu,
                         hipStream_t stream);
unsigned ku_route_scan_grid(uint64_t n_bytes, int n_cu);
uint64_t ku_route_prefix_work_bytes(uint64_t n_rec);
int ku_launch_route_prefix(const void *d_rec, uint64_t n_rec, uint64_t cap, const unsigned long long *d_cursor, uint32_t *d_kb,
                           unsigned long long *d_tot, void *d_work, hipStream_t stream);
int ku_launch_route_owner(const KuDbDev &db, const KuCountsDev &cnt, const void *d_rec, uint64_t n_rec, const uint32_t *d_kb,
                          uint32_t *d_slots, bool do_counts, int n_cu, hipStream_t stream);
int ku_launch_route_gather(uint32_t *d_taxa, uint64_t n, const uint32_t *d_kb, const uint32_t *d_ret, hipStream_t stream);
int ku_launch_lookup_stats(const KuDbDev &db, const uint8_t *d_seqs, uint64_t n_bytes, unsigned long long *d_stats,
                           int n_cu, hipStream_t stream);
int ku_launch_resolve(const KuDbDev &db, const KuTaxDev &tax, const KuCountsDev &cnt, const uint8_t *d_seqs,
                      const uint64_t *d_seq_off, const uint32_t *d_seq_len, uint64_t n_reads, uint32_t flags,
                      uint32_t min_hits, uint32_t max_read_len, uint32_t *d_calls, uint32_t *d_taxa,
                      uint32_t *d_hits, void *d_workspace, uint64_t workspace_bytes, int n_cu,
                      hipStream_t stream);
struct KuRunsOut {
  uint2 *runs;
  unsigned long long *counter;
  unsigned long long cap;
  uint64_t *run_off;
  uint32_t *run_cnt;
  uint32_t chunk;
  uint32_t pre_base1;
};
struct KuSparseFast {
  unsigned long long *g_key;
  uint64_t g_mask;
  unsigned long long *g_count;
  const uint32_t *dense;
  uint32_t *u_cnt;
  const uint32_t *unit_of;
  uint32_t *err;
  uint32_t n_slots;
  uint32_t unit_base;
};
struct KuRouteIn {
  const uint32_t *kb;
  const uint32_t *ret;
};
#define KU_SPARSE_SWITCH_INSERTS 1025u
uint32_t ku_short_max_kmers(const KuDbDev &db);
uint32_t ku_short_max_kmers_windowed(const KuDbDev &db);
uint64_t ku_short_workspace_bytes(uint32_t max_kmers, uint32_t n_slots, uint64_t n_reads, int n_cu);
int ku_launch_classify_short(const KuDbDev &db, const KuTaxDev &tax, const KuCountsDev &cnt, const uint8_t *d_seqs,
                             uint64_t n_bytes, const uint64_t *d_seq_off, const uint32_t *d_seq_len, uint64_t n_reads,
                             uint32_t max_kmers, uint32_t flags, uint32_t *d_calls, uint32_t *d_taxa, uint32_t *d_hits,
                             void *d_workspace, uint64_t workspace_bytes, int n_cu, hipStream_t stream,
                             const KuRunsOut *runs_out = nullptr, const KuSparseFast *sparse = nullptr);
uint32_t ku_route_resolve_max_kmers();
int ku_launch_route_resolve(const KuDbDev &db, const KuTaxDev &tax, const KuCountsDev &cnt, const uint64_t *d_seq_off,
                            const uint32_t *d_seq_len, uint64_t n_reads, uint32_t max_kmers, uint32_t flags, uint32_t *d_calls,
                            uint32_t *d_taxa, uint32_t *d_hits, const uint32_t *d_kb, const uint32_t *d_ret, void *d_workspace,
                            uint64_t workspace_bytes, int n_cu, hipStream_t stream, const KuRunsOut *runs_out = nullptr);
uint64_t ku_short_grid_waves(uint64_t n_reads, uint32_t max_kmers, int n_cu);
uint64_t ku_resolve_workspace_bytes(uint32_t max_read_len, uint32_t k, int n_cu);
int ku_launch_exact(uint32_t k, const uint8_t *d_seqs, const uint64_t *d_seq_off, const uint32_t *d_seq_len, uint64_t n_reads,
                    const uint32_t *d_taxa, unsigned long long *d_set, uint64_t mask, unsigned long long *d_unique,
                    uint32_t *d_overflow, int n_cu, hipStream_t stream, uint32_t quick_min_hits = 0);
int ku_launch_rle(const uint32_t *d_taxa, uint32_t k, const uint64_t *d_seq_off, const uint32_t *d_seq_len,
                  uint64_t n_reads, uint64_t n_bytes, void *d_runs, uint64_t runs_cap, unsigned long long *d_counter,
                  uint64_t *d_run_off, uint32_t *d_run_cnt, int n_cu, hipStream_t stream);
int ku_launch_max_len(const uint32_t *d_seq_len, uint64_t n_reads, uint32_t *d_out, hipStream_t stream);
int ku_launch_quick_chunked(const KuTaxDev &tax, const KuCountsDev &cnt, uint32_t k, const uint64_t *d_seq_off,
                            const uint32_t *d_seq_len, uint64_t n_reads, uint32_t flags, uint32_t min_hits, uint32_t *d_calls,
                            uint32_t *d_taxa, uint32_t *d_hits, int n_cu, hipStream_t stream);
int ku_launch_merge_max_u32(uint32_t *dst, const uint32_t *src, uint64_t n, hipStream_t stream);
int ku_launch_merge_max_u8(uint8_t *dst, const uint8_t *src, uint64_t n, hipStream_t stream);
int ku_launch_replace_u32(uint32_t *p, uint64_t n, uint32_t from, uint32_t to, hipStream_t stream);
#define KU_FOREIGN_MARK 0xFEFEFEFEu
int ku_exact_owned_step(ku_ctx *ctx, const void *d_seqs, const uint64_t *d_off, const uint32_t *d_len, uint64_t n_reads, uint64_t n_bytes,
                        const ku_opts *opts, uint32_t *d_taxa, hipStream_t s);
int ku_launch_merge_add_u64(unsigned long long *dst, const unsigned long long *src, uint64_t n, hipStream_t stream);
int ku_launch_repack(const uint8_t *d_raw, uint64_t n_pairs, uint32_t key_len, uint32_t *d_pairs,
                     hipStream_t stream);
int ku_launch_mark_values(const uint32_t *d_pairs, uint64_t n_pairs, uint32_t *d_bitmap, hipStream_t stream);
int ku_launch_collect_values(const uint32_t *d_bitmap, uint32_t *d_out, uint32_t cap, uint32_t *d_count,
                             hipStream_t stream);
int ku_launch_remap_values(uint32_t *d_pairs, uint64_t n_pairs, const uint32_t *d_slot_taxid, uint32_t n_slots,
                           uint32_t *d_err, hipStream_t stream);
int ku_launch_build_table(const uint32_t *d_pairs, uint64_t n_pairs, void *d_table, uint64_t n_lines, uint32_t k,
                          uint32_t m, uint32_t xor_mask, unsigned long long *d_spilled, hipStream_t stream);
int ku_launch_count_table(const void *d_table, uint64_t n_lines, unsigned long long *d_counts, hipStream_t stream);
int ku_launch_count_slots(const uint32_t *d_pairs, uint64_t n_pairs, unsigned long long *d_counts,
                          uint32_t n_slots, hipStream_t stream);
```

krakenuniq_amd/csrc/ku_kernels.hip:

```cpp
#include <algorithm>
#include <cstdlib>

#include "ku_device.h"

#define KU_THREADS 256
#ifndef KU_MIN_WAVES
#define KU_MIN_WAVES 8
#endif
#ifndef KU_ITEMS
#define KU_ITEMS 1
#endif
#define KU_CTL_MERGE 16u
#define KU_TILE (KU_THREADS * KU_ITEMS)
#define KU_PACKW ((KU_TILE + 64) / 16)

template <int MODE, int LAYOUT, bool SHARDED, bool PRIOR, int ITEMS = KU_ITEMS>
__global__ __launch_bounds__(KU_THREADS, KU_MIN_WAVES) void ku_lookup_kernel(KuDbDev db, KuCountsDev cnt,
                                                               const uint8_t *__restrict__ seqs,
                                                               uint64_t n_bytes, uint32_t *__restrict__ taxa,
                                                               unsigned long long *stats, uint32_t ablate, KuRouteDev rt) {
  constexpr int TILE = KU_THREADS * ITEMS;
  constexpr int PACKW = (TILE + 64) / 16;
  constexpr bool DO_COUNTS = MODE == 1;
  constexpr bool NEED_MIN = true;
// ... 40 lines not shown
    const uint64_t tile0 = tile * TILE;
    __syncthreads();
    if (DO_COUNTS) ku_ct_maybe_flush(s_ctk, s_ctc, &s_ctu, cnt.n_kmers);
    static_assert(4 * (PACKW + 4) <= KU_THREADS, "one packing pass");
    if (tid < 4 * (PACKW + 4)) {
      const uint32_t wi = tid >> 2, q4 = tid & 3u;
      const uint64_t b0 = tile0 + 4ull * tid;
      uint32_t c8 = 0, a4 = 0xFu;
      if (wi < PACKW && b0 < n_bytes) {
        const uint8_t *src = seqs + b0;
        const uintptr_t mis = (uintptr_t)src & 3u;
        uint32_t d;
        if (b0 + 8 - mis <= n_bytes) {
          const uint32_t *q = reinterpret_cast<const uint32_t *>(src - mis);
          d = mis ? __builtin_amdgcn_alignbyte(q[1], q[0], (uint32_t)mis) : q[0];
        } else {
          d = 0;
          for (uint32_t j = 0; j < 4; ++j) d |= (b0 + j < n_bytes ? (uint32_t)src[j] : (uint32_t)'N') << (8 * j);
        }
        ku_pack_dword(d, c8, a4);
      }
      uint32_t word = c8 << (24 - 8 * q4), amb = a4 << (12 - 4 * q4);
      word |= ku_quad_xor1(word);
      amb |= ku_quad_xor1(amb);
      word |= ku_quad_xor2(word);
      amb |= ku_quad_xor2(amb);
      if (q4 == 0) {
        s_codes[wi] = word;
        s_amb16[wi ^ 1u] = (uint16_t)amb;
      }
    }
    __syncthreads();

    uint64_t canon[ITEMS];
    uint64_t kfwd[ROUTE ? ITEMS : 1];
    bool is_fwd[ITEMS];
    bool ok[ITEMS];
    bool foreign[ITEMS];
    uint32_t pk[ITEMS + 1];
    bool tie = false;
#pragma unroll
    for (int j = 0; j <= ITEMS; ++j) {
      uint32_t p = j * KU_THREADS + tid;
      pk[j] = 0;
      if (j == ITEMS && (!NEED_MIN || p >= n_pos)) break;
      uint32_t wi = p >> 4, sh = (p & 15u) * 2;
      const uint32_t c0 = s_codes[wi], c1 = s_codes[wi + 1], c2 = s_codes[wi + 2];
      uint64_t x = ((((uint64_t)c0 << 32) | c1) << sh >> 32 << 32) | ((((uint64_t)c1 << 32) | c2) << sh >> 32);
      if (NEED_MIN) {
        uint32_t mm = (uint32_t)(x >> (64 - 2 * m));
        uint32_t mrc = ku_revcomp32(mm, m);
        const uint32_t val = (mm < mrc ? mm : mrc) ^ db.xor_mask;
        s_mm[p] = val;
        if (PK) {
          pk[j] = ku_pk_make(val, key_shift, mm <= mrc);
          s_pa[p] = pk[j];
          if ((m & 1u) == 0) tie |= mm == mrc;
        }
      }
      if (j < ITEMS) {
        uint64_t fwd = x >> (64 - 2 * k);
        if (ROUTE) {
          kfwd[j] = fwd;
          canon[j] = 0;
          is_fwd[j] = true;
        } else {
          uint64_t rc = ku_revcomp64(fwd, k);
          canon[j] = fwd <= rc ? fwd : rc;
          is_fwd[j] = fwd <= rc;
        }
        uint32_t ai = p >> 5, as = p & 31u;
        uint64_t a = (((uint64_t)s_amb[ai] << 32) | s_amb[ai + 1]) << as;
        ok[j] = (a >> (64 - k)) == 0 && (tile0 + p + k <= n_bytes);
        foreign[j] = false;
      }
    }

    uint32_t prior[ITEMS];
#pragma unroll
    for (int j = 0; j < ITEMS; ++j) prior[j] = (PRIOR && ok[j]) ? taxa[tile0 + (uint64_t)j * KU_THREADS + tid] : 0u;

    uint32_t n_b[ITEMS];
    uint32_t tro[ITEMS];
    const uint32_t *bp[ITEMS];
    uint64_t locus[ITEMS];
    if (NEED_MIN) {
      __syncthreads();
      uint32_t key[ITEMS], aoff[ITEMS], bin_v[ITEMS];
      bool plus[ITEMS];
#pragma unroll
      for (int j = 0; j < ITEMS; ++j) tro[j] = 0;
      if (PK) {
        uint32_t *src = s_pa, *dst = s_pb;
        uint32_t blk = 1;
        for (uint32_t st = 1; 2 * st <= w; st <<= 1) {
#pragma unroll
          for (int j = 0; j <= ITEMS; ++j) {
            const uint32_t p = j * KU_THREADS + tid;
            if (p < n_pos) {
              pk[j] = ku_pk_combine(pk[j], src[p + st], st, tie);
              dst[p] = pk[j];
            }
          }
          __syncthreads();
          uint32_t *t = src; src = dst; dst = t;
          blk = 2 * st;
        }
        if (w > blk) {
#pragma unroll
          for (int j = 0; j < ITEMS; ++j) {
            const uint32_t p = j * KU_THREADS + tid;
            pk[j] = ku_pk_combine_overlap(pk[j], src[p + (w - blk)], w - blk, tie);
          }
        }
        if (tie) s_tie = 1;
        __syncthreads();
        const bool exact = s_tie != 0;
#pragma unroll
        for (int j = 0; j < ITEMS; ++j) {
          const uint32_t p = j * KU_THREADS + tid;
          if (!exact) {
            const uint32_t t = (pk[j] >> 1) & 31u;
            key[j] = pk[j] >> KU_PK_KEYSHIFT;
            aoff[j] = is_fwd[j] ? t : w - 1 - t;
            plus[j] = ((pk[j] & 1u) != 0) == is_fwd[j];
            tro[j] = t;
            bin_v[j] = (SHARDED && key_shift) ? s_mm[p + t] : key[j];
          } else if (ok[j]) {
            if (ROUTE) is_fwd[j] = kfwd[j] <= ku_revcomp64(kfwd[j], k);
            key[j] = ku_anchor_exact(s_mm + p, w, key_shift, is_fwd[j], aoff[j], bin_v[j]);
            tro[j] = is_fwd[j] ? aoff[j] : w - 1 - aoff[j];
            const uint32_t q = p + tro[j];
            const uint32_t wi = q >> 4, sh = (q & 15u) * 2;
            const uint64_t two = ((uint64_t)s_codes[wi] << 32) | s_codes[wi + 1];
            const uint32_t mmf = (uint32_t)((two << sh) >> (64 - 2 * m));
            const uint32_t rcm = ku_revcomp32(mmf, m);
            plus[j] = is_fwd[j] ? (mmf <= rcm) : (rcm <= mmf);
          } else {
            key[j] = 0; aoff[j] = 0; plus[j] = true; bin_v[j] = 0;
          }
        }
        if (exact) {
          __syncthreads();
          if (tid == 0) s_tie = 0;
        }
      }
#pragma unroll
      for (int j = 0; j < ITEMS; ++j) {
        uint32_t p = j * KU_THREADS + tid;
        n_b[j] = 0;
        if (ok[j]) {
          uint32_t mn = 0xFFFFFFFFu;
          if (PK) {
            locus[j] = ku_locus_assemble(canon[j], key[j], aoff[j], plus[j], k, m);
            mn = bin_v[j];
          } else {
            for (uint32_t i = 0; i < w; ++i) mn = min(mn, s_mm[p + i]);
          }
          uint64_t bin = mn;
          if (ROUTE) {
            uint32_t q = 0;
            for (uint32_t nq = rt.world; nq > 1;) {
              const uint32_t half = nq >> 1;
              if (s_olo[q + half] <= bin) q += half;
              nq -= half;
            }
            n_b[j] = (bin >= s_olo[q] && bin < s_ohi[q]) ? q : 0xFFu;
          } else
          if (!SHARDED || (bin >= db.bin_lo && bin < db.bin_hi)) {
            if (LAYOUT == 0 || MODE == 2) {
              const uint64_t *o = db.offsets + (bin - db.bin_lo);
              uint64_t lo = o[0], hi = o[1];
              n_b[j] = (uint32_t)(hi - lo);
              bp[j] = db.pairs + 3 * (lo - db.pair_base);
            }
          } else {
            ok[j] = false;
            foreign[j] = true;
          }
        }
      }
    }

    if (ROUTE) {
      uint32_t idx[ITEMS], rs[ITEMS], rn[ITEMS];
      bool st[ITEMS];
      const uint32_t lane = tid & 63u;
      const unsigned long long below = (1ull << lane) - 1ull, incl = below | (1ull << lane);
      const uint32_t nmax = ku_route_maxn(k, m);
#pragma unroll
      for (int j = 0; j < ITEMS; ++j) {
        const uint32_t p = j * KU_THREADS + tid;
        const bool go = ok[j] && n_b[j] != 0xFFu;
        const uint32_t qa = p + tro[j];
        const uint32_t up_q = ku_wave_up1(qa), up_go = ku_wave_up1((uint32_t)go);
        bool start = go && (lane == 0 || up_go == 0 || up_q != qa);
        unsigned long long sm = __ballot(start);
        uint32_t r0 = (sm & incl) ? 63u - (uint32_t)__builtin_clzll(sm & incl) : lane;
        start = start || (go && lane - r0 == nmax);
        sm = __ballot(start);
        r0 = (sm & incl) ? 63u - (uint32_t)__builtin_clzll(sm & incl) : lane;
        rs[j] = r0;
        const unsigned long long bound = sm | ~__ballot(go);
        const unsigned long long rest = lane == 63u ? 0ull : (bound >> (lane + 1u));
        rn[j] = rest ? (uint32_t)__builtin_ctzll(rest) + 1u : 64u - lane;
        st[j] = start;
        idx[j] = start ? atomicAdd(&s_rcnt[n_b[j]], 1u) : 0u;
      }
      __syncthreads();
      if (tid < rt.world) {
        const uint32_t n = s_rcnt[tid], used = s_cused[tid];
        const unsigned long long base = s_cbase[tid];
        s_rbase[tid] = base == KU_ROUTE_NONE ? KU_ROUTE_NONE : base + used;
        if (used + n <= rt.chunk) {
          s_rsplit[tid] = n;
          s_cused[tid] = used + n;
        } else {
          const uint32_t need = n - (rt.chunk - used), nch = (need + rt.chunk - 1u) / rt.chunk;
          unsigned long long nb = atomicAdd(&rt.cursor[tid * KU_ROUTE_CURSOR_STRIDE], (unsigned long long)nch * rt.chunk);
          if (nb + (unsigned long long)nch * rt.chunk > rt.cap) nb = KU_ROUTE_NONE;
          s_rsplit[tid] = rt.chunk - used;
          s_rbase1[tid] = nb;
          s_cbase[tid] = nb == KU_ROUTE_NONE ? KU_ROUTE_NONE : nb + (unsigned long long)(nch - 1u) * rt.chunk;
          s_cused[tid] = need - (nch - 1u) * rt.chunk;
        }
      }
      __syncthreads();
#pragma unroll
      for (int j = 0; j < ITEMS; ++j) {
        const uint32_t p = j * KU_THREADS + tid;
        uint32_t e32 = 0xFFFFFFFFu;
        if (st[j]) {
          const uint32_t o = n_b[j], split = s_rsplit[o];
          const unsigned long long at = idx[j] < split ? s_rbase[o] : s_rbase1[o];
          if (at != KU_ROUTE_NONE) {
            const unsigned long long e = (unsigned long long)o * rt.cap + at + (idx[j] < split ? idx[j] : idx[j] - split);
            const uint32_t wi = p >> 4, sh = (p & 15u) * 2;
            const uint32_t c0 = s_codes[wi], c1 = s_codes[wi + 1], c2 = s_codes[wi + 2], c3 = s_codes[wi + 3], c4 = s_codes[wi + 4];
            uint4 rec;
            rec.x = (uint32_t)(((((uint64_t)c0 << 32) | c1) << sh) >> 32);
            rec.y = (uint32_t)(((((uint64_t)c1 << 32) | c2) << sh) >> 32);
            rec.z = (uint32_t)(((((uint64_t)c2 << 32) | c3) << sh) >> 32);
            rec.w = ((uint32_t)(((((uint64_t)c3 << 32) | c4) << sh) >> 32) & 0xFFFF0000u) | (tro[j] << 8) | rn[j];
            rt.q_rec[e] = rec;
            e32 = (uint32_t)e;
          }
        }
        const uint32_t eb = (uint32_t)__shfl((int)e32, (int)rs[j]);
        const uint64_t pos = tile0 + p;
        if (pos < n_bytes)
          taxa[pos] = !ok[j] ? KU_AMBIG : ((n_b[j] == 0xFFu || eb == 0xFFFFFFFFu) ? KU_ROUTE_MISS : ((eb << 5) | (lane - rs[j])));
      }
      __syncthreads();
      if (tid < 64) s_rcnt[tid] = 0;
      continue;
    }
    if (MODE == 2) {
#pragma unroll
      for (int j = 0; j < ITEMS; ++j)
        if (ok[j]) {
          st_q += 1;
          st_lg += n_b[j] ? 32 - __builtin_clz(n_b[j]) : 0;
          st_ne += n_b[j] != 0;
          st_nb += n_b[j];
        }
      continue;
    }

    uint32_t slot[ITEMS];
    uint64_t hh[ITEMS];
    if (LAYOUT == 1) {
      const uint32_t *lp[ITEMS];
      uint32_t tag[ITEMS], cand[ITEMS];
      bool act[ITEMS], ovf[ITEMS];
      uint4 h4[ITEMS];
      const uint32_t *tab = reinterpret_cast<const uint32_t *>(db.table);
#pragma unroll
      for (int j = 0; j < ITEMS; ++j) {
        hh[j] = ku_fmix64(canon[j]);
        lp[j] = tab + (ok[j] ? ku_locus_line(locus[j], db.n_lines) : 0) * KU_LINE_DWORDS;
        tag[j] = ku_table_tag(hh[j]);
        slot[j] = 0;
        act[j] = ok[j] && !(ablate & 1u) && !(PRIOR && prior[j]);
      }
#pragma unroll
      for (int j = 0; j < ITEMS; ++j)
        if (act[j]) h4[j] = *reinterpret_cast<const uint4 *>(lp[j]);
#pragma unroll
      for (int j = 0; j < ITEMS; ++j) {
        cand[j] = 0;
        ovf[j] = false;
        if (act[j]) {
          cand[j] = ku_tag_matches(h4[j], tag[j]);
          ovf[j] = ku_line_spilled(h4[j]);
          act[j] = cand[j] != 0 || ovf[j];
        }
      }
      KuPair pr[ITEMS];
#pragma unroll
      for (int j = 0; j < ITEMS; ++j)
        if (cand[j]) pr[j] = *reinterpret_cast<const KuPair *>(lp[j] + KU_LINE_ENTRY0 + 3 * (__builtin_ctz(cand[j])));
#pragma unroll
      for (int j = 0; j < ITEMS; ++j)
        if (cand[j]) {
          if ((((uint64_t)pr[j].key_hi << 32) | pr[j].key_lo) == canon[j]) {
            slot[j] = pr[j].slot;
            act[j] = false;
// ... 29 lines not shown
              if ((((uint64_t)e[j].key_hi << 32) | e[j].key_lo) == canon[j]) {
                slot[j] = e[j].slot;
                act[j] = false;
              }
            } else {
              cand[j] = ku_tag_matches(a4[j], tag[j]);
              ovf[j] = ku_line_spilled(a4[j]);
            }
            if (act[j]) act[j] = cand[j] != 0 || ovf[j];
            any |= act[j];
          }
        }
      }
    } else {
      uint32_t lo[ITEMS], hi[ITEMS];
#pragma unroll
      for (int j = 0; j < ITEMS; ++j) {
        lo[j] = 0;
        hi[j] = ((ablate & 1u) || (PRIOR && prior[j])) ? 0 : n_b[j];
        slot[j] = 0;
        if (DO_COUNTS) hh[j] = ku_fmix64(canon[j]);
      }
      bool any = true;
      while (any) {
        any = false;
        KuPair pr[ITEMS];
        uint32_t mid[ITEMS];
#pragma unroll
        for (int j = 0; j < ITEMS; ++j) {
          mid[j] = (lo[j] + hi[j]) >> 1;
          if (lo[j] < hi[j]) pr[j] = reinterpret_cast<const KuPair *>(bp[j])[mid[j]];
        }
#pragma unroll
        for (int j = 0; j < ITEMS; ++j) {
          if (lo[j] < hi[j]) {
            uint64_t key = ((uint64_t)pr[j].key_hi << 32) | pr[j].key_lo;
            if (key == canon[j]) {
              slot[j] = pr[j].slot;
              lo[j] = hi[j];
            } else if (key < canon[j]) {
              lo[j] = mid[j] + 1;
            } else {
              hi[j] = mid[j];
            }
            any |= lo[j] < hi[j];
          }
        }
      }
    }

#pragma unroll
    for (int j = 0; j < ITEMS; ++j) {
      uint64_t pos = tile0 + (uint64_t)j * KU_THREADS + tid;
      if (PRIOR && prior[j]) slot[j] = prior[j];
      if (DO_COUNTS) {
        if (ok[j] && !(ablate & 2u)) ku_hll_update(cnt.registers, slot[j], hh[j]);
        const bool okc = ok[j] && !(ablate & 4u);
        const unsigned long long booked = __ballot(okc);
        if (booked) {
          const uint32_t lead = (uint32_t)__ffsll((long long)booked) - 1;
          const uint32_t s0 = ku_wave_bcast(slot[j], lead);
          if (__ballot(okc && slot[j] == s0) == booked) {
            if ((tid & 63u) == lead) ku_ct_add(s_ctk, s_ctc, &s_ctu, s0, (uint32_t)__popcll(booked), cnt.n_kmers);
          } else if (okc) {
            ku_ct_add(s_ctk, s_ctc, &s_ctu, slot[j], 1, cnt.n_kmers);
          }
        }
      }
      if (pos < n_bytes && !(ablate & 8u) && !((ablate & KU_CTL_MERGE) && foreign[j])) {
        taxa[pos] = ok[j] ? slot[j] : (foreign[j] ? 0u : KU_AMBIG);
      }
    }
  }
  if (DO_COUNTS) {
    __syncthreads();
    ku_ct_flush(s_ctk, s_ctc, cnt.n_kmers);
  }
  if (ROUTE) {
    __syncthreads();
    for (uint32_t o = 0; o < rt.world; ++o) {
      const unsigned long long base = s_cbase[o];
      if (base == KU_ROUTE_NONE) continue;
      for (uint32_t i = s_cused[o] + tid; i < rt.chunk; i += KU_THREADS)
        rt.q_rec[(unsigned long long)o * rt.cap + base + i] = make_uint4(0u, 0u, 0u, 0u);
    }
  }
  if (MODE == 2) {
    unsigned long long v[4] = {st_q, st_lg, st_ne, st_nb};
#pragma unroll
    for (int i = 0; i < 4; ++i) {
#pragma unroll
      for (int o = 32; o > 0; o >>= 1) v[i] += __shfl_xor(v[i], o);
      if ((tid & 63) == 0 && v[i]) atomicAdd(&stats[i], v[i]);
    }
  }
}

static unsigned ku_lookup_grid(uint64_t n_bytes, int n_cu) {
  uint64_t n_tiles = (n_bytes + KU_TILE - 1) / KU_TILE;
  uint64_t max_blocks = (uint64_t)n_cu * 2 * KU_MIN_WAVES;
  return (unsigned)(n_tiles < max_blocks ? n_tiles : max_blocks);
}

int ku_launch_lookup(const KuDbDev &db, const KuCountsDev &cnt, const uint8_t *d_seqs, uint64_t n_bytes,
                     uint32_t *d_taxa, bool do_counts, bool prior, bool merge_chunk, int n_cu, hipStream_t stream) {
  if (n_bytes == 0) return KU_OK;
  const dim3 grid(ku_lookup_grid(n_bytes, n_cu)), block(KU_THREADS);
  unsigned long long *ns = nullptr;
  const bool sharded = !(db.bin_lo == 0 && db.bin_hi == (1ull << (2 * db.nt)));
  const char *ab = getenv("KU_ABLATE");
  const uint32_t ablate = ((ab ? (uint32_t)atoi(ab) : 0u) & ~KU_CTL_MERGE) | (merge_chunk ? KU_CTL_MERGE : 0u);
  if (prior && sharded) return KU_EUNSUP;
#define KU_LAUNCH(M, L, S, P) hipLaunchKernelGGL((ku_lookup_kernel<M, L, S, P>), grid, block, 0, stream, db, cnt, d_seqs, n_bytes, d_taxa, ns, ablate, KuRouteDev{})
  if (prior) {
    if (db.table) { if (do_counts) KU_LAUNCH(1, 1, false, true); else KU_LAUNCH(0, 1, false, true); }
    else { if (do_counts) KU_LAUNCH(1, 0, true, true); else KU_LAUNCH(0, 0, true, true); }
  } else if (db.table) {
    if (do_counts) { if (sharded) KU_LAUNCH(1, 1, true, false); else KU_LAUNCH(1, 1, false, false); }
    else { if (sharded) KU_LAUNCH(0, 1, true, false); else KU_LAUNCH(0, 1, false, false); }
  } else {
    if (do_counts) KU_LAUNCH(1, 0, true, false); else KU_LAUNCH(0, 0, true, false);
  }
#undef KU_LAUNCH
  return hipGetLastError() == hipSuccess ? KU_OK : KU_EHIP;
}

int ku_launch_lookup_stats(const KuDbDev &db, const uint8_t *d_seqs, uint64_t n_bytes, unsigned long long *d_stats,
                           int n_cu, hipStream_t stream) {
  if (n_bytes == 0) return KU_OK;
  hipLaunchKernelGGL((ku_lookup_kernel<2, 0, true, false>), dim3(ku_lookup_grid(n_bytes, n_cu)), dim3(KU_THREADS), 0, stream,
                     db, KuCountsDev{}, d_seqs, n_bytes, (uint32_t *)nullptr, d_stats, 0u, KuRouteDev{});
  return hipGetLastError() == hipSuccess ? KU_OK : KU_EHIP;
}

#ifndef KU_ROUTE_ITEMS
#define KU_ROUTE_ITEMS 2
#endif
unsigned ku_route_scan_grid(uint64_t n_bytes, int n_cu) {
  const uint64_t tile = (uint64_t)KU_THREADS * KU_ROUTE_ITEMS, n_tiles = (n_bytes + tile - 1) / tile;
  const uint64_t max_blocks = (uint64_t)n_cu * 2 * KU_MIN_WAVES;
  return (unsigned)std::max<uint64_t>(1, std::min<uint64_t>(std::min(n_tiles, max_blocks), (n_tiles + 7) / 8));
}
int ku_launch_route_scan(const KuDbDev &db, const uint8_t *d_seqs, uint64_t n_bytes, uint32_t *d_taxa, const KuRouteDev &rt, int n_cu,
                         hipStream_t stream) {
  if (n_bytes == 0) return KU_OK;
  if (!db.table || rt.world == 0 || rt.world > 64 || rt.cap == 0 || rt.chunk == 0 || rt.chunk % KU_ROUTE_CHUNK || rt.cap % rt.chunk) return KU_EINVAL;
  if ((uint64_t)rt.world * rt.cap > KU_ROUTE_MAX_RECORDS) return KU_EUNSUP;
  hipLaunchKernelGGL((ku_lookup_kernel<3, 1, true, false, KU_ROUTE_ITEMS>), dim3(ku_route_scan_grid(n_bytes, n_cu)), dim3(KU_THREADS), 0, stream, db,
                     KuCountsDev{}, d_seqs, n_bytes, d_taxa, (unsigned long long *)nullptr, 0u, rt);
  return hipGetLastError() == hipSuccess ? KU_OK : KU_EHIP;
}

__global__ void ku_build_table_kernel(const uint32_t *__restrict__ pairs, uint64_t n, uint32_t *table, uint64_t n_lines,
                                      uint32_t k, uint32_t m, uint32_t xor_mask, unsigned long long *n_spilled) {
  for (uint64_t i = blockIdx.x * (uint64_t)blockDim.x + threadIdx.x; i < n; i += (uint64_t)gridDim.x * blockDim.x) {
    const uint32_t klo = pairs[3 * i], khi = pairs[3 * i + 1], val = pairs[3 * i + 2];
    const uint64_t key = ((uint64_t)khi << 32) | klo;
    const uint32_t tag = ku_table_tag(ku_fmix64(key));
    uint32_t bin;
    uint64_t line = ku_locus_line(ku_locus_key(key, k, m, xor_mask, bin), n_lines);
    for (uint32_t hops = 0;; ++hops) {
      uint32_t *lp = table + line * KU_LINE_DWORDS;
      int got = -1;
      for (int i = 0; i < KU_LINE_SLOTS && got < 0; ++i) {
        uint32_t *w = lp + ku_tag_dword((uint32_t)i);
        const uint32_t sh = ku_tag_shift((uint32_t)i);
        uint32_t cur = __hip_atomic_load(w, __ATOMIC_RELAXED, __HIP_MEMORY_SCOPE_AGENT);
        while (((cur >> sh) & 0x7FFFu) == 0) {
          const uint32_t prev = atomicCAS(w, cur, cur | (tag << sh));
          if (prev == cur) { got = i; break; }
          cur = prev;
        }
      }
      if (got >= 0) {
        uint32_t *e = lp + KU_LINE_ENTRY0 + 3 * got;
        e[0] = klo; e[1] = khi; e[2] = val;
        if (hops) atomicAdd(n_spilled, 1ull);
        break;
      }
      atomicOr(lp, 0x8000u);
      line = line + 1 == n_lines ? 0 : line + 1;
    }
  }
}
int ku_launch_build_table(const uint32_t *d_pairs, uint64_t n_pairs, void *d_table, uint64_t n_lines, uint32_t k,
                          uint32_t m, uint32_t xor_mask, unsigned long long *d_spilled, hipStream_t stream) {
  if (hipMemsetAsync(d_table, 0, n_lines * 128, stream) != hipSuccess) return KU_EHIP;
  if (n_pairs == 0) return KU_OK;
  uint64_t nb = (n_pairs + 255) / 256;
  hipLaunchKernelGGL(ku_build_table_kernel, dim3((unsigned)(nb < 8192 ? nb : 8192)), dim3(256), 0, stream, d_pairs,
                     n_pairs, (uint32_t *)d_table, n_lines, k, m, xor_mask, d_spilled);
  return hipGetLastError() == hipSuccess ? KU_OK : KU_EHIP;
}

__global__ __launch_bounds__(256) void ku_count_table_kernel(const uint32_t *__restrict__ table, uint64_t n_lines,
                                                             unsigned long long *counts) {
  __shared__ uint32_t s_ctk[KU_CT_CAP];
  __shared__ uint32_t s_ctc[KU_CT_CAP];
  __shared__ uint32_t s_ctu;
  ku_ct_clear(s_ctk, s_ctc, &s_ctu);
  __syncthreads();
  const uint64_t stride = (uint64_t)gridDim.x * blockDim.x;
  for (uint64_t base = blockIdx.x * (uint64_t)blockDim.x; base < n_lines; base += stride) {
    uint64_t l = base + threadIdx.x;
    if (l < n_lines) {
      const uint32_t *lp = table + l * KU_LINE_DWORDS;
      for (uint32_t i = 0; i < KU_LINE_SLOTS; ++i)
        if ((lp[ku_tag_dword(i)] >> ku_tag_shift(i)) & 0x7FFFu) ku_ct_add(s_ctk, s_ctc, &s_ctu, lp[KU_LINE_ENTRY0 + 3 * i + 2], 1, counts);
    }
    __syncthreads();
    ku_ct_maybe_flush(s_ctk, s_ctc, &s_ctu, counts);
  }
  __syncthreads();
  ku_ct_flush(s_ctk, s_ctc, counts);
}
int ku_launch_count_table(const void *d_table, uint64_t n_lines, unsigned long long *d_counts, hipStream_t stream) {
  hipLaunchKernelGGL(ku_count_table_kernel, dim3(2048), dim3(256), 0, stream, (const uint32_t *)d_table, n_lines,
                     d_counts);
  return hipGetLastError() == hipSuccess ? KU_OK : KU_EHIP;
}

template <int MODE> struct KuResolveCfg;
template <> struct KuResolveCfg<0> { static constexpr int GROUP = 64, CAP_LOG2 = 9, MAX_N = 384; };
template <> struct KuResolveCfg<1> { static constexpr int GROUP = 1024, CAP_LOG2 = 14, MAX_N = 12288; };
template <> struct KuResolveCfg<2> { static constexpr int GROUP = 256, CAP_LOG2 = 0, MAX_N = 0x7fffffff; };

template <int GROUP> __device__ __forceinline__ uint32_t ku_group_max(uint32_t v, uint32_t *s_red) {
  v = ku_wave_max_u32(v);
  if (GROUP > 64) {
    __syncthreads();
    if ((threadIdx.x & 63) == 0) s_red[threadIdx.x >> 6] = v;
    __syncthreads();
    v = s_red[0];
#pragma unroll
    for (int i = 1; i < GROUP / 64; ++i) v = max(v, s_red[i]);
  }
  return v;
}
template <int GROUP> __device__ __forceinline__ uint32_t ku_group_min(uint32_t v, uint32_t *s_red) {
  return ~ku_group_max<GROUP>(~v, s_red);
}
template <int GROUP> __device__ __forceinline__ uint32_t ku_group_sum(uint32_t v, uint32_t *s_red) {
#pragma unroll
  for (int o = 32; o > 0; o >>= 1) v += (uint32_t)__shfl_xor((int)v, o);
  if (GROUP > 64) {
    __syncthreads();
    if ((threadIdx.x & 63) == 0) s_red[threadIdx.x >> 6] = v;
    __syncthreads();
    v = 0;
#pragma unroll
    for (int i = 0; i < GROUP / 64; ++i) v += s_red[i];
  }
  return v;
}

template <int MODE>
__global__ __launch_bounds__(KuResolveCfg<MODE>::GROUP) void ku_resolve_kernel(
    KuTaxDev tax, KuCountsDev cnt, uint32_t k, const uint64_t *__restrict__ seq_off,
    const uint32_t *__restrict__ seq_len, uint64_t n_reads, uint32_t min_n, uint32_t flags,
    uint32_t *__restrict__ calls, uint32_t *__restrict__ taxa, uint32_t *__restrict__ hits_out, uint32_t *ws,
    uint32_t ws_cap_log2) {
  using Cfg = KuResolveCfg<MODE>;
  constexpr int GROUP = Cfg::GROUP;
  extern __shared__ __attribute__((aligned(16))) uint32_t smem[];
  __shared__ uint32_t s_red[16];
  __shared__ uint32_t s_n_list;
  __shared__ uint32_t s_bcast;
  constexpr int RCT = 7;
  __shared__ uint32_t s_ctk[1 << RCT];
  __shared__ uint32_t s_ctc[1 << RCT];
  __shared__ uint32_t s_ctu;

  const uint32_t tid = threadIdx.x;
  auto gsync = [&]() {
    if (GROUP == 64) {
      __builtin_amdgcn_fence(__ATOMIC_RELEASE, "wavefront");
      __builtin_amdgcn_wave_barrier();
      __builtin_amdgcn_fence(__ATOMIC_ACQUIRE, "wavefront");
    } else {
      __syncthreads();
    }
  };
  const uint32_t cap_log2 = MODE == 2 ? ws_cap_log2 : (uint32_t)Cfg::CAP_LOG2;
  const uint32_t cap = 1u << cap_log2;
  uint32_t *t_key, *t_cnt, *t_score, *t_list;
  if (MODE == 2) {
    uint32_t *base = ws + (size_t)blockIdx.x * 4 * cap;
    t_key = base;
    t_cnt = base + cap;
    t_score = base + 2 * (size_t)cap;
    t_list = base + 3 * (size_t)cap;
  } else {
    t_key = smem;
    t_cnt = smem + cap;
    t_score = nullptr;
    t_list = smem + 2 * cap;
  }
  uint16_t *t_list16 = reinterpret_cast<uint16_t *>(t_list);
  const bool do_counts = !(flags & KU_F_NO_COUNTS);
  const bool keep_slots = (flags & KU_F_KEEP_SLOTS) != 0;

  ku_ct_clear<RCT>(s_ctk, s_ctc, &s_ctu);
  for (uint32_t i = tid; i < cap; i += GROUP) {
    t_key[i] = 0;
    t_cnt[i] = 0;
    if (MODE == 2) t_score[i] = 0;
  }
  __syncthreads();

  constexpr int NV = MODE == 0 ? (Cfg::MAX_N + 63) / 64 : 1;
  const uint64_t stride = gridDim.x;
  uint32_t p_len = 0, pp_len = 0, pv[NV];
  uint64_t p_off = 0, pp_off = 0;
  auto request_codes = [&](uint32_t plen, uint64_t poff) {
    const uint32_t pn = plen >= k ? plen - k + 1 : 0;
#pragma unroll
    for (int c = 0; c < NV; ++c) {
      const uint32_t i = c * 64 + tid;
      pv[c] = (i < pn && pn <= (uint32_t)Cfg::MAX_N) ? taxa[poff + i] : 0u;
    }
  };
  if (MODE == 0) {
    const uint64_t r0 = blockIdx.x;
    if (r0 < n_reads) { p_len = seq_len[r0]; p_off = seq_off[r0]; request_codes(p_len, p_off); }
    if (r0 + stride < n_reads) { pp_len = seq_len[r0 + stride]; pp_off = seq_off[r0 + stride]; }
  }

  for (uint64_t r = blockIdx.x; r < n_reads; r += gridDim.x) {
    const uint32_t len = MODE == 0 ? p_len : seq_len[r];
    const uint64_t off = MODE == 0 ? p_off : seq_off[r];
    uint32_t v[NV];
    if (MODE == 0) {
#pragma unroll
      for (int c = 0; c < NV; ++c) v[c] = pv[c];
      p_len = pp_len;
      p_off = pp_off;
      if (r + stride < n_reads) request_codes(p_len, p_off);
      if (r + 2 * stride < n_reads) { pp_len = seq_len[r + 2 * stride]; pp_off = seq_off[r + 2 * stride]; }
    }
    const uint32_t n = len >= k ? len - k + 1 : 0;
    if (n < min_n || n > (uint32_t)Cfg::MAX_N) continue;
    if (GROUP > 64 || s_ctu > (1u << RCT) / 2) ku_ct_maybe_flush<RCT>(s_ctk, s_ctc, &s_ctu, cnt.n_reads);
    uint32_t call_node = 0, uni_taxid = 0;
    bool resolved = false;
// ... 647 lines not shown
```

krakenuniq_amd/csrc/ku_mgpu.cpp:

```cpp
#include <set>

#include "ku_mgpu_route.h"

extern "C" int ku_mgpu_unique_id(uint8_t *id) {
  if (!id) return mfail(KU_EINVAL, "ku_mgpu_unique_id: null argument");
  M_TRY(rccl_ready());
  static_assert(sizeof(ncclUniqueId) == KU_MGPU_ID_BYTES, "RCCL unique id size");
  ncclUniqueId u;
  M_NCCL(g_rccl.GetUniqueId(&u));
  memcpy(id, &u, sizeof u);
  return KU_OK;
}

extern "C" void ku_mgpu_destroy(ku_mgpu *m) {
  if (!m) return;
  for (auto &r : m->ranks) {
    (void)hipSetDevice(r.device);
    if (r.ctx) (void)ku_ctx_synchronize(r.ctx);
    if (r.comm && g_rccl.CommDestroy) (void)g_rccl.CommDestroy(r.comm);
    r.release();
    if (r.ctx) ku_ctx_destroy(r.ctx);
  }
  if (m->sh.bar_init) pthread_barrier_destroy(&m->sh.bar);
  delete m;
}

extern "C" int ku_mgpu_create(const int *devices, uint32_t n_local, uint32_t first_rank, uint32_t world, const uint8_t *id,
                              uint32_t flags, ku_mgpu **out) {
  if (!out || !devices || n_local == 0 || world == 0 || first_rank + n_local > world)
    return mfail(KU_EINVAL, "ku_mgpu_create: bad rank layout");
  *out = nullptr;
  const bool all_here = first_rank == 0 && n_local == world;
  if (!all_here && !id) return mfail(KU_EINVAL, "ku_mgpu_create: a world that spans processes needs the unique id of rank 0");
  if (!all_here && n_local != 1) return mfail(KU_EUNSUP, "ku_mgpu_create: one rank per process, or all ranks in one process");
  ku_mgpu *m = new ku_mgpu();
  m->world = world;
  m->first_rank = first_rank;
  m->n_local = n_local;
  m->flags = flags;
  m->ranks.resize(n_local);
  for (auto *v : {&m->sh.ptr_a, &m->sh.ptr_b, &m->sh.ptr_c}) v->assign(n_local, nullptr);
  m->sh.vals.resize(n_local);
  m->sh.u64s.resize(n_local);
  m->sh.offs.assign(n_local, nullptr);
  m->sh.dev.assign(devices, devices + n_local);
  std::set<int> distinct(devices, devices + n_local);
  m->use_rccl = (world > 1 || getenv("KU_MGPU_FORCE_RCCL")) &&
                (!all_here || (distinct.size() == n_local && !(flags & KU_MGPU_NO_RCCL)));
  if (n_local > 1) {
    if (pthread_barrier_init(&m->sh.bar, nullptr, n_local) != 0) { delete m; return mfail(KU_ENOMEM, "pthread_barrier_init"); }
    m->sh.bar_init = true;
  }
  for (uint32_t i = 0; i < n_local; ++i) {
    auto &r = m->ranks[i];
    r.rank = first_rank + i;
    r.local = i;
    r.device = devices[i];
    int st = ku_ctx_create(devices[i], &r.ctx);
    if (st != KU_OK) { ku_mgpu_destroy(m); return st; }
  }
  if (m->use_rccl) {
    int st = rccl_ready();
    if (st != KU_OK) { ku_mgpu_destroy(m); return st; }
    if (all_here && !(id && n_local == 1)) {
      std::vector<ncclComm_t> comms(n_local);
      ncclResult_t e = g_rccl.CommInitAll(comms.data(), (int)n_local, devices);
      if (e != ncclSuccess) { ku_mgpu_destroy(m); return mfail(KU_EHIP, std::string("ncclCommInitAll: ") + g_rccl.GetErrorString(e)); }
      for (uint32_t i = 0; i < n_local; ++i) m->ranks[i].comm = comms[i];
    } else {
      ncclUniqueId u;
      memcpy(&u, id, sizeof u);
      if (hipSetDevice(devices[0]) != hipSuccess) { ku_mgpu_destroy(m); return mfail(KU_EHIP, "hipSetDevice failed"); }
      ncclResult_t e = g_rccl.CommInitRank(&m->ranks[0].comm, (int)world, u, (int)first_rank);
      if (e != ncclSuccess) { ku_mgpu_destroy(m); return mfail(KU_EHIP, std::string("ncclCommInitRank: ") + g_rccl.GetErrorString(e)); }
    }
  }
  *out = m;
  return KU_OK;
}

extern "C" ku_ctx *ku_mgpu_ctx(ku_mgpu *m, uint32_t local_index) {
  return (m && local_index < m->n_local) ? m->ranks[local_index].ctx : nullptr;
}
extern "C" int ku_mgpu_uses_rccl(const ku_mgpu *m) { return m && m->use_rccl ? 1 : 0; }
extern "C" int ku_mgpu_uses_routing(const ku_mgpu *m) { return m && m->route && !m->exact ? 1 : 0; }

extern "C" int ku_mgpu_set_timing(ku_mgpu *m, int on) {
  if (!m) return mfail(KU_EINVAL, "ku_mgpu_set_timing: null argument");
  m->timing = on != 0;
  return KU_OK;
}
extern "C" int ku_mgpu_step_times(ku_mgpu *m, uint32_t local_index, double *out) {
  if (!m || !out || local_index >= m->n_local) return mfail(KU_EINVAL, "ku_mgpu_step_times: bad argument");
  ku_mgpu::Rank &r = m->ranks[local_index];
  for (int i = 0; i < 6; ++i) out[i] = 0;
  if (hipSetDevice(r.device) != hipSuccess) return mfail(KU_EHIP, "hipSetDevice failed");
  for (auto &t : r.tev) {
    float ms = 0;
    if (hipEventSynchronize(t.second.second) != hipSuccess || hipEventElapsedTime(&ms, t.second.first, t.second.second) != hipSuccess)
      return mfail(KU_EHIP, "ku_mgpu_step_times: an event of the last step is not complete");
    if (t.first >= 0 && t.first < 3) out[t.first] += ms;
  }
  out[3] = r.t_rounds;
  out[4] = r.t_rec;
  out[5] = r.t_kmers;
  return KU_OK;
}

extern "C" int ku_mgpu_set_taxonomy(ku_mgpu *m, const ku_tax *tax) {
  if (!m || !tax) return mfail(KU_EINVAL, "ku_mgpu_set_taxonomy: null argument");
  M_TRY(ranks_idle(m, "ku_mgpu_set_taxonomy"));
  M_TRY(run_all(m, [&](ku_mgpu::Rank &r) -> int {
    uint64_t n = 0;
    int st = ku_ctx_db_values(r.ctx, nullptr, &n);
    std::vector<uint32_t> mine(st == KU_OK ? n : 0), all;
    if (st == KU_OK && n) st = ku_ctx_db_values(r.ctx, mine.data(), &n);
    st = comm_allgather_values(m, r, st, mine, all);
    if (st != KU_OK) return st;
    st = ku_ctx_set_taxonomy(r.ctx, tax, all.data(), all.size());
    uint64_t info[4] = {0, 0, 0, 0};
    int is_hash = 0, single = 0;
    if (st == KU_OK) st = ku_ctx_route_info(r.ctx, &info[0], &info[1], &is_hash, &single);
    info[2] = (uint64_t)(is_hash && single);
    std::vector<uint64_t> allinfo;
    st = comm_allgather_u64(m, r, st, info, 4, allinfo, ku_ctx_stream_of(r.ctx));
    if (st == KU_OK && r.local == 0) {
      m->own_lo.assign(m->world, 0);
      m->own_hi.assign(m->world, 0);
      bool ok = true;
      for (uint32_t q = 0; q < m->world; ++q) { m->own_lo[q] = allinfo[4 * q]; m->own_hi[q] = allinfo[4 * q + 1]; ok = ok && allinfo[4 * q + 2]; }
      for (uint32_t q = 0; q + 1 < m->world; ++q) ok = ok && m->own_lo[q] <= m->own_hi[q] && m->own_hi[q] <= m->own_lo[q + 1];
      if (std::getenv("KU_ROUTE_DEBUG")) {
        fprintf(stderr, "[ku_route] rank %u: hash+single everywhere / ascending ranges: %d;", r.rank, (int)ok);
        for (uint32_t q = 0; q < m->world; ++q) fprintf(stderr, " [%llu, %llu) flag %llu", (unsigned long long)m->own_lo[q], (unsigned long long)m->own_hi[q], (unsigned long long)allinfo[4 * q + 2]);
        fprintf(stderr, "\n");
      }
      const char *ex = getenv("KU_MGPU_EXCHANGE");
      m->ring_reduce = ex && !strcmp(ex, "reduce");
      m->route = ok && (m->world > 1 || std::getenv("KU_MGPU_FORCE_ROUTE")) && m->world <= 64 && !(m->flags & KU_MGPU_REPLICAS) && !(ex && (!strcmp(ex, "slots") || m->ring_reduce));
    }
    return st;
  }));
  m->tax_set = true;
  return KU_OK;
}

extern "C" int ku_mgpu_load_dbs(ku_mgpu *m, const ku_db *const *dbs, uint32_t n_dbs, const ku_tax *tax) {
  if (!m || !dbs || !n_dbs || !tax) return mfail(KU_EINVAL, "ku_mgpu_load_dbs: null argument");
  M_TRY(ranks_idle(m, "ku_mgpu_load_dbs"));
  if (n_dbs == 1) return ku_mgpu_load(m, dbs[0], tax);
  if (!(m->flags & KU_MGPU_REPLICAS)) return mfail(KU_EUNSUP, "several databases on several GPUs need the replicas mode (KU_MGPU_REPLICAS)");
  ku_db_info info;
  M_TRY(ku_db_get_info(dbs[0], &info));
  M_TRY(run_all(m, [&](ku_mgpu::Rank &r) -> int {
    M_TRY(ku_ctx_load_db(r.ctx, dbs[0], 0, info.n_bins));
    for (uint32_t i = 1; i < n_dbs; ++i) M_TRY(ku_ctx_add_db(r.ctx, dbs[i]));
    return KU_OK;
  }));
  m->loaded = true;
  return ku_mgpu_set_taxonomy(m, tax);
}

extern "C" int ku_mgpu_load(ku_mgpu *m, const ku_db *db, const ku_tax *tax) {
  if (!m || !db || !tax) return mfail(KU_EINVAL, "ku_mgpu_load: null argument");
  M_TRY(ranks_idle(m, "ku_mgpu_load"));
  ku_db_info info;
  M_TRY(ku_db_get_info(db, &info));
  std::vector<uint64_t> bounds(m->world + 1);
  M_TRY(ku_db_shard_plan(db, m->world, bounds.data()));
  const bool replicas = (m->flags & KU_MGPU_REPLICAS) != 0;
  M_TRY(run_all(m, [&](ku_mgpu::Rank &r) -> int {
    return replicas ? ku_ctx_load_db(r.ctx, db, 0, info.n_bins) : ku_ctx_load_db(r.ctx, db, bounds[r.rank], bounds[r.rank + 1]);
  }));
  m->loaded = true;
  return ku_mgpu_set_taxonomy(m, tax);
}

extern "C" int ku_mgpu_enable_sparse(ku_mgpu *m, uint64_t work_unit_nt, uint32_t global_log2) {
  if (!m) return mfail(KU_EINVAL, "ku_mgpu_enable_sparse: null argument");
  M_TRY(ranks_idle(m, "ku_mgpu_enable_sparse"));
  if (!m->tax_set) return mfail(KU_ESTATE, "ku_mgpu_enable_sparse: load the database and the taxonomy first");
  if (!single_process(m)) return mfail(KU_EUNSUP, "the sparse-mode emulation over several GPUs needs the group in one process");
  if (work_unit_nt == 0) return mfail(KU_EUNSUP, "ku_mgpu_enable_sparse: a work unit size is needed (the ranks take whole units)");
  M_TRY(run_all(m, [&](ku_mgpu::Rank &r) -> int { return ku_ctx_enable_sparse(r.ctx, work_unit_nt, global_log2); }));
  m->sparse = true;
  m->unit_nt = work_unit_nt;
  m->acc_nt = 0;
  m->open_rank = -1;
  return KU_OK;
}
extern "C" int ku_mgpu_sparse_close_unit(ku_mgpu *m) {
  if (!m) return mfail(KU_EINVAL, "ku_mgpu_sparse_close_unit: null argument");
  M_TRY(ranks_idle(m, "ku_mgpu_sparse_close_unit"));
  if (!m->sparse) return KU_OK;
  if (m->open_rank >= 0) {
    ku_mgpu::Rank &r = m->ranks[m->open_rank];
    if (hipSetDevice(r.device) != hipSuccess) return mfail(KU_EHIP, "hipSetDevice failed");
    M_TRY(ku_sparse_close_unit(r.ctx));
  }
  m->acc_nt = 0;
  m->open_rank = -1;
  return KU_OK;
}
extern "C" int ku_mgpu_sparse_state(const ku_mgpu *m) {
  if (!m) return 0;
  int worst = m->sparse_gave_up ? 2 : (m->sparse ? 1 : 0);
  for (const auto &r : m->ranks) {
    const int s = ku_ctx_sparse_state(r.ctx);
    if (s == 2) worst = 2;
  }
  return worst;
}
// ... 287 lines not shown
```

krakenuniq_amd/csrc/ku_route.hip:

```cpp
#include <algorithm>
#include <cstdlib>

#include "ku_device.h"

#define KR_WAVES 4
#define KR_ITEMS 2
#define KR_KCT_LOG2 8
#define KR_OWN_BYTES 2048

__device__ __forceinline__ void kr_wave_sync() {
  __builtin_amdgcn_fence(__ATOMIC_RELEASE, "wavefront");
  __builtin_amdgcn_wave_barrier();
  __builtin_amdgcn_fence(__ATOMIC_ACQUIRE, "wavefront");
}

#define KR_PFX_THREADS 256
#define KR_PFX_PER 4
#define KR_PFX_TILE (KR_PFX_THREADS * KR_PFX_PER)

__device__ __forceinline__ uint32_t kr_rec_n(const uint4 *__restrict__ rec, uint64_t i, uint64_t n_rec, uint64_t cap,
                                             const unsigned long long *__restrict__ cursor) {
  if (i >= n_rec) return 0;
  if (cap) {
    const uint64_t q = i / cap, within = i - q * cap;
// ... 65 lines not shown
    }
    carry += tot;
  }
  if (threadIdx.x == 0) bsum[n_blocks] = carry;
}
__global__ __launch_bounds__(KR_PFX_THREADS) void ku_route_prefix_write_kernel(const uint4 *__restrict__ rec, uint64_t n_rec, uint64_t cap,
                                                                                const unsigned long long *__restrict__ cursor,
                                                                                const uint32_t *__restrict__ bsum, uint32_t n_blocks,
                                                                                uint32_t *__restrict__ kb) {
  __shared__ uint32_t s_w[KR_PFX_THREADS / 64];
  if (blockIdx.x == 0 && threadIdx.x == 0) kb[n_rec] = bsum[n_blocks];
  if (kr_tile_unused((uint64_t)blockIdx.x * KR_PFX_TILE, n_rec, cap, cursor)) return;
  const uint64_t base = (uint64_t)blockIdx.x * KR_PFX_TILE + (uint64_t)threadIdx.x * KR_PFX_PER;
  uint32_t n[KR_PFX_PER], v = 0;
#pragma unroll
  for (int u = 0; u < KR_PFX_PER; ++u) {
    n[u] = kr_rec_n(rec, base + u, n_rec, cap, cursor);
    v += n[u];
  }
  uint32_t tot;
  uint32_t run = bsum[blockIdx.x] + kr_block_scan(v, s_w, &tot) - v;
#pragma unroll
  for (int u = 0; u < KR_PFX_PER; ++u) {
    if (base + u < n_rec) kb[base + u] = run;
    run += n[u];
  }
}
__global__ void ku_route_totals_kernel(const uint32_t *__restrict__ kb, uint64_t cap, uint32_t world,
                                       const unsigned long long *__restrict__ cursor, unsigned long long *__restrict__ tot) {
  const uint32_t q = threadIdx.x;
  if (q < world) {
    tot[2 * q] = cursor[q * KU_ROUTE_CURSOR_STRIDE];
    tot[2 * q + 1] = (unsigned long long)(kb[(uint64_t)(q + 1) * cap] - kb[(uint64_t)q * cap]);
  }
  if (q == world) tot[2 * world] = cap;
}

uint64_t ku_route_prefix_work_bytes(uint64_t n_rec) { return ((n_rec + KR_PFX_TILE - 1) / KR_PFX_TILE + 2) * 4; }

int ku_launch_route_prefix(const void *d_rec, uint64_t n_rec, uint64_t cap, const unsigned long long *d_cursor, uint32_t *d_kb,
                           unsigned long long *d_tot, void *d_work, hipStream_t stream) {
  if (!d_kb || !d_work || (n_rec && !d_rec) || (cap && (!d_cursor || n_rec % cap))) return KU_EINVAL;
  const uint64_t n_blocks = (n_rec + KR_PFX_TILE - 1) / KR_PFX_TILE;
  if (n_blocks >= (1ull << 31)) return KU_EUNSUP;
  const uint4 *rec = (const uint4 *)d_rec;
  uint32_t *bsum = (uint32_t *)d_work;
  if (n_blocks)
    hipLaunchKernelGGL(ku_route_prefix_sums_kernel, dim3((unsigned)n_blocks), dim3(KR_PFX_THREADS), 0, stream, rec, n_rec, cap, d_cursor, bsum);
  hipLaunchKernelGGL(ku_route_prefix_blocks_kernel, dim3(1), dim3(KR_PFX_THREADS), 0, stream, bsum, (uint32_t)n_blocks);
  hipLaunchKernelGGL(ku_route_prefix_write_kernel, dim3((unsigned)std::max<uint64_t>(n_blocks, 1)), dim3(KR_PFX_THREADS), 0, stream, rec, n_rec,
                     cap, d_cursor, bsum, (uint32_t)n_blocks, d_kb);
  if (d_tot && cap) {
    const uint32_t world = (uint32_t)(n_rec / cap);
    if (world > 64) return KU_EINVAL;
    hipLaunchKernelGGL(ku_route_totals_kernel, dim3(1), dim3(128), 0, stream, d_kb, cap, world, d_cursor, d_tot);
  }
  return hipGetLastError() == hipSuccess ? KU_OK : KU_EHIP;
}

__device__ __forceinline__ uint32_t kr_word(const uint4 &r, uint32_t i) { return i == 0 ? r.x : (i == 1 ? r.y : (i == 2 ? r.z : (i == 3 ? r.w : 0u))); }

template <int LOG2>
__device__ __forceinline__ void kr_ct_flush(uint32_t *key, uint32_t *cnt, uint32_t *used, unsigned long long *global, uint32_t lane) {
  kr_wave_sync();
  for (uint32_t i = lane; i < (1u << LOG2); i += 64) {
    const uint32_t kk = key[i];
    if (kk) atomicAdd(&global[kk - 1], (unsigned long long)cnt[i]);
    key[i] = 0;
    cnt[i] = 0;
  }
  if (lane == 0) *used = 0;
  kr_wave_sync();
}

template <bool DO_COUNTS, int KK, int MM>
__global__ __launch_bounds__(64 * KR_WAVES) void ku_route_owner_kernel(KuDbDev db, KuCountsDev cnt, const uint4 *__restrict__ rec,
                                                                        uint64_t n_groups, const uint32_t *__restrict__ kb,
                                                                        uint32_t *__restrict__ slots) {
  __shared__ uint4 s_rec[KR_WAVES][64];
  __shared__ uint32_t s_m0[KR_WAVES][64];
  __shared__ uint32_t s_m1[KR_WAVES][64];
  __shared__ uint8_t s_own[KR_WAVES][KR_OWN_BYTES];
  __shared__ uint32_t s_kk[KR_WAVES][1 << KR_KCT_LOG2], s_kc[KR_WAVES][1 << KR_KCT_LOG2];
  __shared__ uint32_t s_misc[KR_WAVES][2];

  const uint32_t lane = threadIdx.x & 63u;
  const uint32_t wv = (uint32_t)__builtin_amdgcn_readfirstlane((int)(threadIdx.x >> 6));
  uint4 *w_rec = s_rec[wv];
  uint32_t *w_m0 = s_m0[wv], *w_m1 = s_m1[wv], *misc = s_misc[wv];
  uint8_t *w_own = s_own[wv];
  const uint32_t k = KK ? (uint32_t)KK : db.k, m = KK ? (uint32_t)MM : db.nt, w = k - m + 1;
  const uint32_t key_shift = ku_key_shift(m);
  const uint32_t *tab = reinterpret_cast<const uint32_t *>(db.table);
  if (DO_COUNTS) {
    for (uint32_t i = lane; i < (1u << KR_KCT_LOG2); i += 64) { s_kk[wv][i] = 0; s_kc[wv][i] = 0; }
    if (lane == 0) misc[0] = 0;
  }
  kr_wave_sync();

  const uint64_t n_waves = (uint64_t)gridDim.x * KR_WAVES;
  uint4 R_n = make_uint4(0u, 0u, 0u, 0u);
  uint32_t kb_n = 0;
  {
    const uint64_t g0 = (uint64_t)blockIdx.x * KR_WAVES + wv;
    if (g0 < n_groups) { R_n = rec[g0 * 64 + lane]; kb_n = kb[g0 * 64 + lane]; }
  }
  for (uint64_t g = (uint64_t)blockIdx.x * KR_WAVES + wv; g < n_groups; g += n_waves) {
    if (DO_COUNTS && misc[0] > (1u << KR_KCT_LOG2) / 2) kr_ct_flush<KR_KCT_LOG2>(s_kk[wv], s_kc[wv], &misc[0], cnt.n_kmers, lane);
    const uint4 R = R_n;
    const uint32_t kb_l = kb_n;
    if (g + n_waves < n_groups) { R_n = rec[(g + n_waves) * 64 + lane]; kb_n = kb[(g + n_waves) * 64 + lane]; }
    const uint32_t kb0 = (uint32_t)__builtin_amdgcn_readfirstlane((int)kb_l);
    const uint32_t n = R.w & 31u, a0 = (R.w >> 8) & 63u, pre = kb_l - kb0;
    const uint32_t T = (uint32_t)__builtin_amdgcn_readlane((int)(pre + n), 63);
    {
      const uint32_t wi = a0 >> 4, sh = (a0 & 15u) * 2;
      const uint64_t two = ((uint64_t)kr_word(R, wi) << 32) | kr_word(R, wi + 1);
      const uint32_t mmf = (uint32_t)((two << sh) >> (64 - 2 * m));
      const uint32_t rcm = ku_revcomp32(mmf, m);
      const uint32_t val = (mmf < rcm ? mmf : rcm) ^ db.xor_mask;
      w_m0[lane] = ((val >> key_shift) << 6) | a0;
      w_m1[lane] = pre | ((uint32_t)(mmf <= rcm) << 16) | ((uint32_t)(rcm <= mmf) << 17);
      w_rec[lane] = R;
      for (uint32_t i = 0; i < n; ++i) w_own[pre + i] = (uint8_t)lane;
    }
    kr_wave_sync();

    for (uint32_t e0 = 0; e0 < T; e0 += 64 * KR_ITEMS) {
      uint32_t v[KR_ITEMS];
      uint64_t hh[KR_ITEMS], canon[KR_ITEMS];
      bool ok[KR_ITEMS];
      const uint32_t *lp[KR_ITEMS];
      uint32_t tag[KR_ITEMS], cand[KR_ITEMS];
      bool act[KR_ITEMS], ovf[KR_ITEMS];
#pragma unroll
      for (int j = 0; j < KR_ITEMS; ++j) {
        const uint32_t e = e0 + j * 64 + lane;
        ok[j] = e < T;
        const uint32_t r = (uint32_t)w_own[ok[j] ? e : 0u];
        const uint4 Q = w_rec[r];
        const uint32_t m0 = w_m0[r], m1 = w_m1[r];
        const uint32_t pj = ok[j] ? e - (m1 & 0xFFFFu) : 0u;
        const uint32_t wi = pj >> 4, sh = (pj & 15u) * 2;
        const uint32_t c0 = wi ? Q.y : Q.x, c1 = wi ? Q.z : Q.y, c2 = wi ? Q.w : Q.z;
        const uint64_t x = ((((uint64_t)c0 << 32) | c1) << sh >> 32 << 32) | ((((uint64_t)c1 << 32) | c2) << sh >> 32);
        const uint64_t fwd = x >> (64 - 2 * k);
        const uint64_t rc = ku_revcomp64(fwd, k);
        const bool is_fwd = fwd <= rc;
        canon[j] = is_fwd ? fwd : rc;
        const uint32_t anc = m0 & 63u;
        const uint32_t t = ok[j] ? anc - pj : 0u;
        const uint32_t aoff = is_fwd ? t : w - 1 - t;
        const bool plus = ((m1 >> (is_fwd ? 16 : 17)) & 1u) != 0;
        const uint64_t locus = ku_locus_assemble(canon[j], m0 >> 6, aoff, plus, k, m);
        hh[j] = ku_fmix64(canon[j]);
        const uint64_t line = ku_locus_line(locus, db.n_lines);
        lp[j] = tab + (ok[j] ? line : 0) * KU_LINE_DWORDS;
        tag[j] = ku_table_tag(hh[j]);
        act[j] = ok[j];
        v[j] = 0;
      }
      uint4 h4[KR_ITEMS];
#pragma unroll
      for (int j = 0; j < KR_ITEMS; ++j) h4[j] = *reinterpret_cast<const uint4 *>(lp[j]);
      KuPair pr[KR_ITEMS];
      const uint32_t *ep[KR_ITEMS];
#pragma unroll
      for (int j = 0; j < KR_ITEMS; ++j) {
        cand[j] = ku_tag_matches(h4[j], tag[j]) & (act[j] ? 0xFFu : 0u);
        ovf[j] = act[j] && ku_line_spilled(h4[j]);
        ep[j] = lp[j] + KU_LINE_ENTRY0 + 3 * (__builtin_ctz(cand[j] | 0x100u) & 7u);
      }
#pragma unroll
      for (int j = 0; j < KR_ITEMS; ++j) pr[j] = *reinterpret_cast<const KuPair *>(ep[j]);
#pragma unroll
      for (int j = 0; j < KR_ITEMS; ++j) {
        const bool hit = cand[j] != 0 && (((uint64_t)pr[j].key_hi << 32) | pr[j].key_lo) == canon[j];
        v[j] = hit ? pr[j].slot : 0u;
        cand[j] &= cand[j] - 1;
        act[j] = !hit && (cand[j] != 0 || ovf[j]);
      }
      bool any = false;
#pragma unroll
      for (int j = 0; j < KR_ITEMS; ++j) any |= act[j];
      while (any) {
        any = false;
        KuPair en[KR_ITEMS];
        uint4 a4[KR_ITEMS];
#pragma unroll
        for (int j = 0; j < KR_ITEMS; ++j) {
          if (act[j]) {
            if (cand[j]) {
              en[j] = *reinterpret_cast<const KuPair *>(lp[j] + KU_LINE_ENTRY0 + 3 * (__builtin_ctz(cand[j])));
            } else {
              lp[j] += KU_LINE_DWORDS;
              if (lp[j] == tab + db.n_lines * KU_LINE_DWORDS) lp[j] = tab;
              a4[j] = *reinterpret_cast<const uint4 *>(lp[j]);
            }
          }
        }
#pragma unroll
        for (int j = 0; j < KR_ITEMS; ++j) {
          if (act[j]) {
            if (cand[j]) {
              cand[j] &= cand[j] - 1;
              if ((((uint64_t)en[j].key_hi << 32) | en[j].key_lo) == canon[j]) {
                v[j] = en[j].slot;
                act[j] = false;
              }
            } else {
              cand[j] = ku_tag_matches(a4[j], tag[j]);
              ovf[j] = ku_line_spilled(a4[j]);
            }
            if (act[j]) act[j] = cand[j] != 0 || ovf[j];
            any |= act[j];
          }
        }
      }
      if (DO_COUNTS) {
        uint8_t *reg[KR_ITEMS];
        uint32_t rank[KR_ITEMS], seen[KR_ITEMS];
#pragma unroll
        for (int j = 0; j < KR_ITEMS; ++j) {
          reg[j] = ku_hll_locate(cnt.registers, ok[j] ? v[j] : 0u, hh[j], rank[j]);
          seen[j] = ok[j] ? (uint32_t)*reg[j] : 0xFFu;
        }
#pragma unroll
        for (int j = 0; j < KR_ITEMS; ++j) {
          ku_hll_raise(reg[j], seen[j], rank[j]);
          unsigned long long todo = __ballot(ok[j]);
          while (todo) {
            const uint32_t lead = (uint32_t)__ffsll((long long)todo) - 1u;
            const uint32_t s0 = ku_wave_bcast(v[j], lead);
            const unsigned long long same = __ballot(ok[j] && v[j] == s0);
            if (lane == lead) ku_ct_add<KR_KCT_LOG2>(s_kk[wv], s_kc[wv], &misc[0], s0, (uint32_t)__popcll(same), cnt.n_kmers);
            todo &= ~same;
          }
        }
      }
#pragma unroll
      for (int j = 0; j < KR_ITEMS; ++j)
        if (ok[j]) slots[(uint64_t)kb0 + e0 + j * 64 + lane] = v[j];
    }
    kr_wave_sync();
  }
  if (DO_COUNTS) kr_ct_flush<KR_KCT_LOG2>(s_kk[wv], s_kc[wv], &misc[0], cnt.n_kmers, lane);
}

int ku_launch_route_owner(const KuDbDev &db, const KuCountsDev &cnt, const void *d_rec, uint64_t n_rec, const uint32_t *d_kb,
                          uint32_t *d_slots, bool do_counts, int n_cu, hipStream_t stream) {
  if (n_rec == 0) return KU_OK;
  if (!db.table || !d_rec || !d_kb || !d_slots || n_rec % 64) return KU_EINVAL;
  const uint64_t n_groups = n_rec / 64, want = (n_groups + KR_WAVES - 1) / KR_WAVES;
  const char *oe = getenv("KU_ROUTE_BLOCKS_PER_CU");
  const uint64_t cap = (uint64_t)n_cu * (oe ? (uint64_t)atoi(oe) : 6ull);
  const dim3 grid((unsigned)(want < cap ? want : cap)), block(64 * KR_WAVES);
  const int geo = db.k != 31 ? 0 : (db.nt == 13 ? 13 : (db.nt == 15 ? 15 : 0));
#define KR_LAUNCH(C, K, M) \
  hipLaunchKernelGGL((ku_route_owner_kernel<C, K, M>), grid, block, 0, stream, db, cnt, (const uint4 *)d_rec, n_groups, d_kb, d_slots)
  if (do_counts) { if (geo == 13) KR_LAUNCH(true, 31, 13); else if (geo == 15) KR_LAUNCH(true, 31, 15); else KR_LAUNCH(true, 0, 0); }
  else { if (geo == 13) KR_LAUNCH(false, 31, 13); else if (geo == 15) KR_LAUNCH(false, 31, 15); else KR_LAUNCH(false, 0, 0); }
#undef KR_LAUNCH
  return hipGetLastError() == hipSuccess ? KU_OK : KU_EHIP;
}

__global__ void ku_route_gather_kernel(uint32_t *__restrict__ taxa, uint64_t n, const uint32_t *__restrict__ kb,
                                       const uint32_t *__restrict__ ret) {
  for (uint64_t i = blockIdx.x * (uint64_t)blockDim.x + threadIdx.x; i < n; i += (uint64_t)gridDim.x * blockDim.x) {
    const uint32_t t = taxa[i];
    if (t == KU_AMBIG) continue;
    taxa[i] = t == KU_ROUTE_MISS ? 0u : ret[(uint64_t)kb[t >> 5] + (t & 31u)];
  }
}

int ku_launch_route_gather(uint32_t *d_taxa, uint64_t n, const uint32_t *d_kb, const uint32_t *d_ret, hipStream_t stream) {
  if (n == 0) return KU_OK;
  if (!d_taxa || !d_kb) return KU_EINVAL;
  const uint64_t want = (n + 255) / 256;
  hipLaunchKernelGGL(ku_route_gather_kernel, dim3((unsigned)(want < 16384 ? want : 16384)), dim3(256), 0, stream, d_taxa, n, d_kb, d_ret);
  return hipGetLastError() == hipSuccess ? KU_OK : KU_EHIP;
}
```

krakenuniq_amd/csrc/ku_short.hip:

```cpp
#include <cstdlib>
#include <type_traits>

#include "ku_device.h"

#define KS_WAVES 4
#ifndef KS_KCT_LOG2
#define KS_KCT_LOG2 8
#endif
#define KS_FLOOR_EVERY 64u
#define KS_HQ 64
#define KS_PAD 16
#ifdef KU_ABLATION
#define KS_ABL(bit) ((ablate & (bit)) != 0)
#else
#define KS_ABL(bit) false
#endif

template <int ITEMS> struct KsGeom {
  static constexpr int MAXN = 64 * ITEMS;
  static constexpr int NWORDS = (MAXN + 31 + 15) / 16 + 3;
  static constexpr int NCODES = (MAXN + 64) / 16 + 4;
  static constexpr int NAMB = (NWORDS + 1) / 2 + 2;
  static constexpr int NMM = MAXN + 64 + 32;
  static constexpr int TCAP_LOG2 = ITEMS <= 2 ? 8 : (ITEMS <= 4 ? 9 : 10);
  static constexpr int KCT_LOG2 = KS_KCT_LOG2;
  static constexpr int RCT_LOG2 = 6;
};

template <int ITEMS, bool WIN, bool SCAN, bool HQ> struct KsWaveLds {
  using G = KsGeom<ITEMS>;
  static constexpr int TCAP = 1 << G::TCAP_LOG2;
  std::conditional_t<HQ, uint2, uint32_t> hq[HQ ? KS_HQ : 0];
  uint32_t codes[SCAN ? G::NCODES : 0];
  uint32_t amb[SCAN ? G::NAMB : 0];
  uint32_t mm[SCAN ? G::NMM : 0];
  uint32_t tkey[TCAP];
  uint32_t tcnt[TCAP];
  uint32_t kk[SCAN ? 1 << G::KCT_LOG2 : 0], kc[SCAN ? 1 << G::KCT_LOG2 : 0];
  uint32_t rk[1 << G::RCT_LOG2], rc[1 << G::RCT_LOG2];
  uint32_t misc[4];
  uint16_t tlist[WIN ? TCAP : G::MAXN];
};

struct __attribute__((packed, aligned(4))) KsQuad {
  uint32_t x, y, z, w;
};
__device__ __forceinline__ uint64_t ks_quad_key(const KsQuad &q) { return ((uint64_t)q.y << 32) | q.x; }
__device__ __forceinline__ uint4 ks_quad_header(const KsQuad &q) { return make_uint4(q.x, q.y, q.z, q.w); }

__device__ __forceinline__ bool ks_less64(uint64_t a, uint64_t b) { return (int64_t)(a - b) < 0; }

__device__ __forceinline__ void ks_wave_sync() {
  __builtin_amdgcn_fence(__ATOMIC_RELEASE, "wavefront");
  __builtin_amdgcn_wave_barrier();
  __builtin_amdgcn_fence(__ATOMIC_ACQUIRE, "wavefront");
}

template <int LOG2>
__device__ __forceinline__ void ks_ct_flush(uint32_t *key, uint32_t *cnt, uint32_t *used, unsigned long long *global,
                                            uint32_t lane, uint32_t *hot = nullptr) {
  ks_wave_sync();
  for (uint32_t i = lane; i < (1u << LOG2); i += 64) {
    uint32_t kk = key[i];
#ifdef KS_DIAG_NOHOT
    if (kk == 1) kk = 0;
#endif
    if (hot && kk == 1) { *hot = cnt[i]; kk = 0; }
    if (kk) atomicAdd(&global[kk - 1], (unsigned long long)cnt[i]);
    key[i] = 0;
    cnt[i] = 0;
  }
  if (lane == 0) *used = 0;
  ks_wave_sync();
}

__device__ __forceinline__ uint32_t ks_bmin4(uint32_t a, uint32_t b) {
  const uint32_t m = ((((a | 0x80808080u) - b) & 0x80808080u) >> 7) * 0xFFu;
  return (b & m) | (a & ~m);
}

#define KS_RCT_SLOT 0x40000000u
__device__ __forceinline__ uint32_t ks_rct_node(uint32_t id, const KuTaxDev &tax) {
  return (id & KS_RCT_SLOT) ? ((id & ~KS_RCT_SLOT) ? tax.slot_node[id & ~KS_RCT_SLOT] : 0u) : id;
}
template <int LOG2>
__device__ __forceinline__ void ks_rct_add(uint32_t *key, uint32_t *cnt, uint32_t *used, uint32_t id, const KuTaxDev &tax,
                                           unsigned long long *global) {
  uint32_t h = (id * 2654435761u) >> (32 - LOG2);
#pragma unroll 1
  for (int probe = 0; probe < 8; ++probe) {
    uint32_t cur = key[h];
    if (cur == 0) { key[h] = id + 1; *used += 1; cur = id + 1; }
    if (cur == id + 1) { cnt[h] += 1; return; }
    h = (h + 1) & ((1u << LOG2) - 1);
  }
  atomicAdd(&global[ks_rct_node(id, tax)], 1ull);
}
template <int LOG2>
__device__ __forceinline__ void ks_rct_flush(uint32_t *key, uint32_t *cnt, uint32_t *used, const KuTaxDev &tax,
                                             unsigned long long *global, uint32_t lane, uint32_t *hot = nullptr) {
  ks_wave_sync();
  for (uint32_t i = lane; i < (1u << LOG2); i += 64) {
    uint32_t kk = key[i];
#ifdef KS_DIAG_NOHOT
    if (kk - 1 == KS_RCT_SLOT) kk = 0;
#endif
    if (hot && kk - 1 == KS_RCT_SLOT) { *hot = cnt[i]; kk = 0; }
    if (kk) atomicAdd(&global[ks_rct_node(kk - 1, tax)], (unsigned long long)cnt[i]);
    key[i] = 0;
    cnt[i] = 0;
  }
  if (lane == 0) *used = 0;
  ks_wave_sync();
}

template <int LOG2, bool TRACK>
__device__ __forceinline__ void ks_tab_add(uint32_t *t_key, uint32_t *t_cnt, uint32_t *n_distinct, uint32_t slot, uint32_t count) {
  uint32_t h = (slot * 2654435761u) >> (32 - LOG2);
  for (;;) {
    uint32_t cur = __hip_atomic_load(&t_key[h], __ATOMIC_RELAXED, __HIP_MEMORY_SCOPE_WORKGROUP);
    if (cur == 0) {
      uint32_t old = atomicCAS(&t_key[h], 0u, slot + 1);
      if (TRACK && old == 0) atomicAdd(n_distinct, 1u);
      cur = old == 0 ? slot + 1 : old;
    }
    if (cur == slot + 1) {
      atomicAdd(&t_cnt[h], count);
      break;
    }
    h = (h + 1) & ((1u << LOG2) - 1);
  }
}

template <int LOG2>
__device__ __forceinline__ uint32_t ks_tab_resolve(uint32_t *t_key, uint32_t *t_cnt, uint16_t *t_list, uint32_t *list_len,
                                                   const KuTaxDev &tax, uint32_t lane, uint32_t *urow = nullptr) {
  constexpr uint32_t TCAP = 1u << LOG2;
  if (lane == 0) *list_len = 0;
  ks_wave_sync();
  for (uint32_t i = lane; i < TCAP; i += 64)
    if (t_key[i]) t_list[atomicAdd(list_len, 1u)] = (uint16_t)i;
  ks_wave_sync();
  const uint32_t n_list = *list_len;
  uint32_t my_max = 0;
  for (uint32_t e = lane; e < n_list; e += 64) {
    const uint32_t pos = t_list[e];
    const uint32_t sl = t_key[pos] - 1;
    if (urow) atomicAdd(&urow[sl], t_cnt[pos] & 0xffffu);
    uint32_t score = 0;
    for (uint32_t i = tax.slot_anc_off[sl], i_end = tax.slot_anc_off[sl + 1]; i < i_end; ++i) {
      const uint32_t s = tax.slot_anc[i];
      uint32_t h = (s * 2654435761u) >> (32 - LOG2);
      for (;;) {
        const uint32_t cur = t_key[h];
        if (cur == s + 1) { score += t_cnt[h] & 0xffffu; break; }
        if (cur == 0) break;
        h = (h + 1) & (TCAP - 1);
      }
    }
    atomicAdd(&t_cnt[pos], score << 16);
    my_max = max(my_max, score);
  }
  my_max = ku_wave_max_u32(my_max);
  ks_wave_sync();
// ... 290 lines not shown
      static_assert(G::NCODES - 1 >= G::NWORDS && 2 * G::NAMB - 1 >= G::NWORDS + 1, "no dump element behind the code words");
      const bool text_inside = ks_less64(off + len + 6, n_bytes);
      const uint32_t *text = reinterpret_cast<const uint32_t *>(seqs + (off & ~3ull));
      const uint32_t text_sh = (uint32_t)off & 3u, last_dw = (len - 1u) & ~3u;
#pragma unroll
      for (uint32_t pl = lane; pl < S1_LANES; pl += 64) {
        const uint32_t b0 = 4 * pl;
        const uint32_t valid = len - min(b0, len);
        uint32_t c8 = 0, a4 = 0xFu;
        if (text_inside) {
          const uint32_t *q = text + (min(b0, last_dw) >> 2);
          ku_pack_dword(__builtin_amdgcn_alignbyte(q[1], q[0], text_sh), c8, a4);
        } else if (b0 < len) {
          const uint64_t a = off + b0;
          uint32_t d = 0;
          for (uint32_t j = 0; j < 4; ++j) d |= (a + j < n_bytes ? (uint32_t)seqs[a + j] : (uint32_t)'N') << (8 * j);
          ku_pack_dword(d, c8, a4);
        }
        if (valid < 4) a4 |= (1u << (4 - valid)) - 1u;
        const uint32_t q4 = pl & 3u;
        uint32_t word = c8 << (24 - 8 * q4), ab = a4 << (12 - 4 * q4);
        word |= ku_quad_xor1(word);
        ab |= ku_quad_xor1(ab);
        word |= ku_quad_xor2(word);
        ab |= ku_quad_xor2(ab);
        const uint32_t wi = pl >> 2;
        codes[S1_CLAMP ? min(wi, (uint32_t)G::NCODES - 1u) : wi] = word;
        amb16[(S1_CLAMP ? min(wi, 2u * G::NAMB - 1u) : wi) ^ 1u] = (uint16_t)ab;
      }
      ks_wave_sync();

      const uint32_t P = n + w - 1;
      uint64_t canon[ITEMS];
      bool is_fwd[ITEMS], ok[ITEMS];
      uint32_t pk[ITEMS + 1], wr[ITEMS + 1];
      uint32_t tacc = 0xFFFFFFFFu;
      bool tie = false;
      static_assert(G::MAXN + 30 + 63 < G::NMM - 1, "the sentinels reach the dump slot");
      mmv[P + lane] = (0x03FFFFFFu - lane) << KU_PK_KEYSHIFT;
      const bool tail_round = P > (uint32_t)ITEMS * 64u;
      pk[ITEMS] = 0;
      wr[ITEMS] = (uint32_t)G::NMM - 1u;
#pragma unroll
      for (int j = 0; j <= ITEMS; ++j) {
        if (j == ITEMS && !tail_round) break;
        const uint32_t p = j * 64 + lane;
        wr[j] = p < P ? p : (uint32_t)G::NMM - 1u;
        const uint32_t wi = p >> 4, sh = (p & 15u) * 2;
        const uint32_t c0 = codes[wi], c1 = codes[wi + 1], c2 = codes[wi + 2];
        const uint64_t x = ((((uint64_t)c0 << 32) | c1) << sh >> 32 << 32) | ((((uint64_t)c1 << 32) | c2) << sh >> 32);
        const uint32_t mm = (uint32_t)(x >> (64 - 2 * m));
        const uint32_t mrc = ku_revcomp32(mm, m);
        pk[j] = ku_pk_make((mm < mrc ? mm : mrc) ^ db.xor_mask, key_shift, mm <= mrc);
        if ((m & 1u) == 0) tie |= p < P && mm == mrc;
        mmv[wr[j]] = pk[j];
        if (j < ITEMS) {
          const uint64_t fwd = x >> (64 - 2 * k);
          const uint64_t rc = ku_revcomp64(fwd, k);
          is_fwd[j] = fwd <= rc;
          canon[j] = is_fwd[j] ? fwd : rc;
          const uint32_t ai = p >> 5, as = p & 31u;
          const uint32_t a = __funnelshift_l(amb[ai + 1], amb[ai], as);
          amb_k[j] = p < n && (a >> (32 - k)) != 0;
          ok[j] = p < n && !amb_k[j];
        }
      }
      ks_wave_sync();

      uint32_t key[ITEMS], aoff[ITEMS];
      bool plus[ITEMS];
      if (KS_ABL(64u)) {
#pragma unroll
        for (int j = 0; j < ITEMS; ++j) { key[j] = 0; aoff[j] = 0; plus[j] = true; }
      } else {
        uint32_t blk = 1;
        uint32_t tj[ITEMS + 1];
#pragma unroll
        for (int j = 0; j <= ITEMS; ++j) tj[j] = 0xFFFFFFFFu;
        auto doubling = [&](auto nr_c) {
          constexpr int NR = decltype(nr_c)::value;
#pragma unroll
          for (uint32_t sft = 0; sft < 5; ++sft) {
            const uint32_t st = 1u << sft;
            if (2 * st > w) break;
            uint32_t nb[NR];
#pragma unroll
            for (int j = 0; j < NR; ++j) nb[j] = mmv[j * 64 + lane + st] + (st << 1);
            ks_wave_sync();
#pragma unroll
            for (int j = 0; j < NR; ++j) {
              tj[j] = min(tj[j], (pk[j] ^ nb[j]) - 2u);
              pk[j] = min(pk[j], nb[j]);
              mmv[wr[j]] = pk[j];
            }
            ks_wave_sync();
            blk = 2 * st;
          }
        };
        if (tail_round) doubling(std::integral_constant<int, ITEMS + 1>{});
        else doubling(std::integral_constant<int, ITEMS>{});
        if (w > blk) {
#pragma unroll
          for (int j = 0; j < ITEMS; ++j) {
            const uint32_t nbj = mmv[j * 64 + lane + (w - blk)] + ((w - blk) << 1);
            tj[j] = min(tj[j], (pk[j] ^ nbj) - 2u);
            pk[j] = min(pk[j], nbj);
          }
        }
#pragma unroll
        for (int j = 0; j <= ITEMS; ++j) tacc = min(tacc, j * 64 + lane < P ? tj[j] : 0xFFFFFFFFu);
        tie |= tacc < (1u << KU_PK_KEYSHIFT) - 2u;
#pragma unroll
        for (int j = 0; j < ITEMS; ++j) {
          const uint32_t t = (pk[j] >> 1) & 31u;
          key[j] = pk[j] >> KU_PK_KEYSHIFT;
          aoff[j] = is_fwd[j] ? t : w - 1 - t;
          plus[j] = ((pk[j] & 1u) != 0) == is_fwd[j];
        }
        if (__any(tie)) {
          ks_wave_sync();
#pragma unroll
          for (int j = 0; j <= ITEMS; ++j) {
            const uint32_t p = j * 64 + lane;
            if (p < P) {
              const uint32_t wi = p >> 4, sh = (p & 15u) * 2;
              const uint64_t two = ((uint64_t)codes[wi] << 32) | codes[wi + 1];
              const uint32_t mm = (uint32_t)((two << sh) >> (64 - 2 * m));
              const uint32_t mrc = ku_revcomp32(mm, m);
              mmv[p] = (mm < mrc ? mm : mrc) ^ db.xor_mask;
            }
          }
          ks_wave_sync();
#pragma unroll
          for (int j = 0; j < ITEMS; ++j) {
            const uint32_t p = j * 64 + lane;
            if (ok[j]) {
              uint32_t bin;
              key[j] = ku_anchor_exact(mmv + p, w, key_shift, is_fwd[j], aoff[j], bin);
              const uint32_t q = p + (is_fwd[j] ? aoff[j] : w - 1 - aoff[j]);
              const uint32_t wi = q >> 4, sh = (q & 15u) * 2;
              const uint64_t two = ((uint64_t)codes[wi] << 32) | codes[wi + 1];
              const uint32_t mmf = (uint32_t)((two << sh) >> (64 - 2 * m));
              const uint32_t rcm = ku_revcomp32(mmf, m);
              plus[j] = is_fwd[j] ? (mmf <= rcm) : (rcm <= mmf);
            }
          }
        }
      }
      const uint32_t *lp[ITEMS];
      uint32_t cand[ITEMS];
      bool act[ITEMS], ovf[ITEMS];
#pragma unroll
      for (int j = 0; j < ITEMS; ++j) {
        const uint64_t locus = ku_locus_assemble(canon[j], key[j], aoff[j], plus[j], k, m);
        hh[j] = ku_fmix64(canon[j]);
        const uint64_t line = ku_locus_line(locus, db.n_lines);
        lp[j] = tab + (ok[j] ? line : 0) * KU_LINE_DWORDS;
        act[j] = ok[j] && !KS_ABL(1u);
        if (KS_ABL(64u)) lp[j] = tab;
      }

      uint4 h4[ITEMS];
#pragma unroll
      for (int j = 0; j < ITEMS; ++j) h4[j] = *reinterpret_cast<const uint4 *>(lp[j]);
      KsQuad q[ITEMS];
      const uint32_t *ep[ITEMS];
      bool nxt[ITEMS];
      const uint32_t *const tab_end = tab + db.n_lines * KU_LINE_DWORDS;
#pragma unroll
      for (int j = 0; j < ITEMS; ++j) {
        cand[j] = ku_tag_matches(h4[j], ku_table_tag(hh[j])) & (act[j] ? 0xFFu : 0u);
        ovf[j] = act[j] && ku_line_spilled(h4[j]);
        nxt[j] = ovf[j] && cand[j] == 0;
        const uint32_t eo = nxt[j] ? (uint32_t)KU_LINE_DWORDS : KU_LINE_ENTRY0 + 3 * (__builtin_ctz(cand[j] | 0x100u) & 7u);
        ep[j] = lp[j] + eo;
        if (ep[j] == tab_end) ep[j] = tab;
      }
#pragma unroll
      for (int j = 0; j < ITEMS; ++j) q[j] = *reinterpret_cast<const KsQuad *>(ep[j]);
      uint32_t sb[ITEMS];
      if (OUT == 2 && DO_COUNTS) {
#pragma unroll
        for (int j = 0; j < ITEMS; ++j)
          sb[j] = reinterpret_cast<const uint8_t *>(lp[j] + KU_LINE_SEEN0)[__builtin_ctz(cand[j] | 0x100u) & 7u];
      }
#pragma unroll
      for (int j = 0; j < ITEMS; ++j) {
        const bool hit = cand[j] != 0 && ks_quad_key(q[j]) == canon[j];
        v[j] = hit ? q[j].z : 0u;
        if (OUT == 2 && DO_COUNTS) {
          if (hit && !sb[j] && !KS_ABL(128u)) ku_seen_mark(lp[j], (uint32_t)__builtin_ctz(cand[j]));
        }
        cand[j] &= cand[j] - 1;
        act[j] = !hit && (cand[j] != 0 || ovf[j]);
      }
      bool any = false;
#pragma unroll
      for (int j = 0; j < ITEMS; ++j) any |= act[j];
      while (any && !KS_ABL(1024u)) {
        bool pick[ITEMS], taken = false, fresh = false, ov = false;
        const uint32_t *l = tab;
        uint32_t cm = 0;
        uint64_t hsel = 0;
        KsQuad hq = {0, 0, 0, 0};
#pragma unroll
        for (int j = 0; j < ITEMS; ++j) {
          pick[j] = act[j] && !taken;
          taken |= act[j];
          if (pick[j]) { hsel = hh[j]; l = lp[j]; cm = cand[j]; ov = ovf[j]; fresh = nxt[j]; hq = q[j]; }
        }
        const uint32_t t = ku_table_tag(hsel);
        if (fresh) {
          l += KU_LINE_DWORDS;
          if (l == tab_end) l = tab;
        }
        for (;;) {
          if (fresh) {
            cm = ku_tag_matches(ks_quad_header(hq), t);
            ov = ku_line_spilled(ks_quad_header(hq));
          }
          if (cm == 0 && !ov) break;
          fresh = cm == 0;
          if (fresh) {
            l += KU_LINE_DWORDS;
            if (l == tab_end) l = tab;
          }
          const uint32_t ei = (uint32_t)__builtin_ctz(cm | 0x100u) & 7u;
          hq = *reinterpret_cast<const KsQuad *>(fresh ? l : l + KU_LINE_ENTRY0 + 3 * ei);
          if (!fresh) {
            cm &= cm - 1;
            bool same = false;
#pragma unroll
            for (int j = 0; j < ITEMS; ++j) same |= pick[j] && ks_quad_key(hq) == canon[j];
            if (same) {
#pragma unroll
              for (int j = 0; j < ITEMS; ++j)
                if (pick[j]) v[j] = hq.z;
              if (OUT == 2 && DO_COUNTS && !KS_ABL(128u)) ku_seen_mark(l, ei);
              break;
            }
          }
        }
        any = false;
#pragma unroll
        for (int j = 0; j < ITEMS; ++j) {
          if (pick[j]) act[j] = false;
          any |= act[j];
        }
      }

    }

    bool uni = false;
    uint32_t uni_slot = 0;
    uint32_t hit_first = 0;
    if (!KS_ABL(32u)) {
      uint32_t mine = 0;
#pragma unroll
      for (int j = 0; j < ITEMS; ++j)
        if (mine == 0) mine = v[j];
      const unsigned long long bal = __ballot(mine != 0);
      const uint32_t first = bal ? ku_wave_bcast(mine, (uint32_t)__ffsll((long long)bal) - 1) : 0u;
      bool diff = false;
#pragma unroll
      for (int j = 0; j < ITEMS; ++j) diff |= (v[j] != 0 && v[j] != first);
      uni = !__any(diff);
      uni_slot = uni ? first : 0u;
      hit_first = first;
      if (!WIN) {
        if (!uni) {
#pragma unroll
          for (int j = 0; j < ITEMS; ++j)
            if (v[j] != 0) ks_tab_add<G::TCAP_LOG2, false>(t_key, t_cnt, nullptr, v[j], 1u);
          uint32_t *urow_hits = nullptr;
          if (OUT == 2 && DO_COUNTS && !KS_ABL(512u)) urow_hits = sf.u_cnt + (size_t)(sf.unit_of[r] - sf.unit_base) * sf.n_slots;
          call_node = ks_tab_resolve<G::TCAP_LOG2>(t_key, t_cnt, t_list, &misc[2], tax, lane, urow_hits);
        }
      } else if (bal) {
        uint32_t w_hits = 0;
#pragma unroll
        for (int j = 0; j < ITEMS; ++j) w_hits += (uint32_t)__popcll(__ballot(v[j] != 0));
        if (!rd_table && !(uni && (rd_first == 0 || rd_first == first))) {
          if (rd_first && lane == 0) ks_tab_add<G::TCAP_LOG2, true>(t_key, t_cnt, &misc[3], rd_first, rd_cnt);
          rd_table = true;
        }
        if (!rd_table) {
          rd_first = first;
          rd_cnt += w_hits;
        } else {
          ks_wave_sync();
          if (!rd_spill && misc[3] > TCAP - (uint32_t)G::MAXN - 32u) {
            ks_spill_migrate(t_key, t_cnt, TCAP, g_key, g_cnt, spill_cap - 1, !spill_used, lane);
            spill_used = true;
            rd_spill = true;
          }
          if (!rd_spill) {
            if (uni) {
              if (lane == 0) ks_tab_add<G::TCAP_LOG2, true>(t_key, t_cnt, &misc[3], first, w_hits);
            } else {
#pragma unroll
              for (int j = 0; j < ITEMS; ++j)
                if (v[j] != 0) ks_tab_add<G::TCAP_LOG2, true>(t_key, t_cnt, &misc[3], v[j], 1u);
            }
          } else {
            if (uni) {
              if (lane == 0) ks_spill_add(g_key, g_cnt, spill_cap - 1, first, w_hits);
            } else {
#pragma unroll
              for (int j = 0; j < ITEMS; ++j)
                if (v[j] != 0) ks_spill_add(g_key, g_cnt, spill_cap - 1, v[j], 1u);
            }
          }
        }
      }
    }

    const uint32_t uni_code = uni && uni_slot ? tax.slot_taxid[uni_slot] : 0u;
    const bool fl_on = DO_COUNTS && !ROUTE && floor_every != 0 && n > 0;
    uint32_t fl_miss = 0, fl_hit = 0;
    if (fl_on && uni) {
      fl_miss = ks_gload(&cnt.hll_floor[0]);
      fl_hit = ks_gload(&cnt.hll_floor[uni_slot]);
    }

    uint32_t n_hit = 0, n_miss = 0;
    if (DO_COUNTS && !ROUTE && n > 0) {
      uint32_t rank[ITEMS], fl[ITEMS];
      if (fl_on && !uni) {
#pragma unroll
        for (int j = 0; j < ITEMS; ++j) fl[j] = ks_gload(&cnt.hll_floor[v[j]]);
      } else {
#pragma unroll
        for (int j = 0; j < ITEMS; ++j) fl[j] = v[j] ? fl_hit : fl_miss;
      }
      bool go[ITEMS];
      unsigned long long gob[ITEMS];
      uint32_t n_go = 0;
#pragma unroll
      for (int j = 0; j < ITEMS; ++j) {
        const bool okc = j * 64 + lane < n && !amb_k[j];
        (void)ku_hll_locate(cnt.registers, 0u, hh[j], rank[j]);
        go[j] = okc && rank[j] > fl[j] && !KS_ABL(2u);
        gob[j] = __ballot(go[j]);
        n_go += (uint32_t)__popcll(gob[j]);
      }
      const bool direct = !fl_on || n_go > KS_HQ / 2;
      if (direct) {
        uint8_t *reg[ITEMS];
        uint32_t seen[ITEMS];
#pragma unroll
        for (int j = 0; j < ITEMS; ++j) {
          reg[j] = ku_hll_locate(cnt.registers, go[j] ? v[j] : 0u, hh[j], rank[j]);
          seen[j] = go[j] ? (uint32_t)*reg[j] : 0xFFu;
        }
#pragma unroll
        for (int j = 0; j < ITEMS; ++j) ku_hll_raise(reg[j], seen[j], rank[j]);
      } else {
        if (hq_fill + n_go > KS_HQ) {
          ks_hq_drain(hq, hq_fill, cnt.registers, lane);
          hq_fill = 0;
        }
#pragma unroll
        for (int j = 0; j < ITEMS; ++j) {
          const uint32_t at = hq_fill + __builtin_amdgcn_mbcnt_hi((uint32_t)(gob[j] >> 32), __builtin_amdgcn_mbcnt_lo((uint32_t)gob[j], 0u));
          if (go[j]) hq[at] = make_uint2(v[j], (uint32_t)(hh[j] >> (64 - KU_HLL_P)) | (rank[j] << KU_HLL_P));
          hq_fill += (uint32_t)__popcll(gob[j]);
        }
      }
#pragma unroll
      for (int j = 0; j < ITEMS; ++j) {
        const bool okc = j * 64 + lane < n && !amb_k[j];
        if (uni) {
          n_hit += (uint32_t)__popcll(__ballot(okc && v[j] != 0));
          n_miss += (uint32_t)__popcll(__ballot(okc && v[j] == 0));
        } else if (okc && !KS_ABL(4u)) {
          ku_ct_add<G::KCT_LOG2>(sw.kk, sw.kc, &misc[0], v[j], 1, cnt.n_kmers);
        }
      }
      if (uni && lane == 0 && !KS_ABL(4u)) {
        if (n_hit) ku_ct_add<G::KCT_LOG2>(sw.kk, sw.kc, &misc[0], uni_slot, n_hit, cnt.n_kmers);
        if (n_miss) ku_ct_add<G::KCT_LOG2>(sw.kk, sw.kc, &misc[0], 0u, n_miss, cnt.n_kmers);
      }
      if (fl_on && ((++fl_reads) & 0x7fffffffu) >= floor_every) {
        fl_reads = ~fl_reads & 0x80000000u;
        fl_scan = ((fl_reads >> 31) ? hit_first : 0u) + 1u;
      }
    }

    if (OUT == 2 && DO_COUNTS && n > 0) {
      uint32_t *urow = sf.u_cnt + (size_t)(sf.unit_of[r] - sf.unit_base) * sf.n_slots;
      bool any_miss;
      if (KS_ABL(512u)) {
        any_miss = false;
      } else if (uni) {
        if (lane == 0) {
          if (n_hit) atomicAdd(&urow[uni_slot], n_hit);
          if (n_miss) atomicAdd(&urow[0], n_miss);
        }
        any_miss = n_miss != 0;
      } else if (!WIN && !KS_ABL(32u)) {
// ... 274 lines not shown
```

Before: 607.4.

## Add adaptive locus class split and skip dead-line second probe loads

Replaces the fixed offset-class divisor in locus keys with a per-database class encoding. The table builder picks a 'halves' split instead of 'quarters' when the load is low and the k-mer window would otherwise waste a class, which changes how k-mers are spread across table lines. In the short-read lookup, the second probe load is skipped when no lane in the wave has a tag candidate or spill. Lanes with no candidates are also redirected to the table base so their loads all hit one cached line. The split choice adds build-time heuristics and must stay consistent between build and lookup; it is disabled for multi-GPU groups.

Result: slower. 600.6 (-1.1%).

```diff
diff --git a/krakenuniq_amd/capi.py b/krakenuniq_amd/capi.py
--- a/krakenuniq_amd/capi.py
+++ b/krakenuniq_amd/capi.py
@@ -407,6 +407,13 @@
         _chk(lib().ku_ctx_db_layout(self.h, C.byref(h), C.byref(b)), "ku_ctx_db_layout")
         return {"hash": bool(h.value), "resident_bytes": b.value}
 
+    def table_info(self):
+        n, s, lf, sp = C.c_uint64(), C.c_uint64(), C.c_double(), C.c_uint32()
+        f = lib().ku_ctx_table_info
+        f.restype, f.argtypes = C.c_int, [C.c_void_p, u64p, u64p, C.POINTER(C.c_double), u32p]
+        _chk(f(self.h, C.byref(n), C.byref(s), C.byref(lf), C.byref(sp)), "ku_ctx_table_info")
+        return {"n_lines": n.value, "n_spilled": s.value, "load": lf.value, "split": "halves" if sp.value else "quarters"}
+
     def db_values(self):
         n = C.c_uint64()
         _chk(lib().ku_ctx_db_values(self.h, None, C.byref(n)), "ku_ctx_db_values")
diff --git a/krakenuniq_amd/csrc/ku_api.cpp b/krakenuniq_amd/csrc/ku_api.cpp
--- a/krakenuniq_amd/csrc/ku_api.cpp
+++ b/krakenuniq_amd/csrc/ku_api.cpp
@@ -307,6 +307,7 @@
 int ku_ctx_device_of(const ku_ctx *ctx) { return ctx->device; }
 int ku_ctx_cus_of(const ku_ctx *ctx) { return ctx->n_cu; }
 uint32_t ku_ctx_k_of(const ku_ctx *ctx) { return ctx->m.db.k; }
+void ku_ctx_join_group(ku_ctx *ctx) { ctx->group_member = true; }
 
 int ctx_activate(ku_ctx *ctx) {
   if (hipSetDevice(ctx->device) != hipSuccess) return fail(KU_EHIP, "hipSetDevice failed");
@@ -317,6 +318,9 @@
   if (!out) return fail(KU_EINVAL, "ku_ctx_create: null argument");
   *out = nullptr;
   KU_TRY(ku_check_device(device));
+  const char *const split = getenv("KU_LOCUS_SPLIT");
+  if (split && strcmp(split, "halves") != 0 && strcmp(split, "quarters") != 0)
+    return fail(KU_EINVAL, std::string("KU_LOCUS_SPLIT is '") + split + "': halves or quarters");
   hipDeviceProp_t prop;
   HIP_TRY(hipGetDeviceProperties(&prop, device));
   if (strncmp(prop.gcnArchName, "gfx950", 6) != 0)
@@ -332,6 +336,7 @@
     double f = atof(e);
     if (f >= 0.05 && f <= 0.9) { ctx->load_factor = f; ctx->load_factor_set = true; }
   }
+  if (split) ctx->locus_split = strcmp(split, "halves") == 0;
   *out = ctx;
   return KU_OK;
 }
@@ -463,6 +468,7 @@
   d.db.k = k;
   d.db.nt = nt;
   d.db.xor_mask = idx_type == 1 ? 0u : ku_index2_xor_mask(nt);
+  d.db.cls = KU_CLS_QUARTERS;
 }
 
 int store_upload(ku_ctx *ctx, DbStore &d, const ku_db *db, uint64_t bin_lo, uint64_t bin_hi, bool scan_values, hipStream_t stream) {
@@ -546,6 +552,16 @@
   if (is_hash) *is_hash = hash ? 1u : 0u;
   if (resident_bytes)
     *resident_bytes = (hash ? ctx->m.db.n_lines * 128 : ctx->m.db.n_pairs * 12) + (ctx->m.db.bin_hi - ctx->m.db.bin_lo + 1) * 8;
+  return KU_OK;
+}
+
+extern "C" int ku_ctx_table_info(ku_ctx *ctx, uint64_t *n_lines, uint64_t *n_spilled, double *load, uint32_t *split) {
+  if (!ctx) return fail(KU_EINVAL, "null context");
+  if (!ctx->db_loaded || !ctx->m.db.table) return fail(KU_ESTATE, "no probe table (taxonomy not set, or the sorted layout)");
+  if (n_lines) *n_lines = ctx->m.db.n_lines;
+  if (n_spilled) *n_spilled = ctx->m.n_dup;
+  if (load) *load = ctx->m.table_load;
+  if (split) *split = ctx->m.db.cls == KU_CLS_QUARTERS ? 0u : 1u;
   return KU_OK;
 }
 
@@ -597,7 +613,7 @@
     for (double lf : chain) {
       n_lines = (uint64_t)((double)d.db.n_pairs / lf / 8.0) + 1;
       if (n_lines >= (1ull << 32)) { n_lines = 0; continue; }
-      if (hipMalloc(&d.d_table, n_lines * 128) == hipSuccess) { d.table_lines = n_lines; break; }
+      if (hipMalloc(&d.d_table, n_lines * 128) == hipSuccess) { d.table_lines = n_lines; d.table_load = lf; break; }
       (void)hipGetLastError();
       d.d_table = nullptr;
       n_lines = 0;
@@ -623,8 +639,12 @@
     const uint64_t n_lines = d.table_lines;
     unsigned long long *d_dup = (unsigned long long *)(d_scalar + 2);
     HIP_TRY(hipMemsetAsync(d_dup, 0, 8, stream));
-    KU_TRY(ku_launch_build_table(d.d_pairs, d.db.n_pairs, d.d_table, n_lines, d.db.k, d.db.nt, d.db.xor_mask, d_dup,
-                                 stream));
+    const uint32_t w = d.db.k - d.db.nt + 1;
+    const bool halves = !ctx->group_member && store_whole(d) &&
+                        (ctx->locus_split >= 0 ? ctx->locus_split == 1 : d.table_load <= KU_HALVES_MAX_LOAD && ku_quarters_waste_a_class(w));
+    d.db.cls = halves ? ku_cls_halves(w) : KU_CLS_QUARTERS;
+    KU_TRY(ku_launch_build_table(d.d_pairs, d.db.n_pairs, d.d_table, n_lines, d.db.k, d.db.nt, d.db.xor_mask, d.db.cls,
+                                 d_dup, stream));
     unsigned long long dup = 0;
     HIP_TRY(hipMemcpyAsync(&dup, d_dup, 8, hipMemcpyDeviceToHost, stream));
     HIP_TRY(hipStreamSynchronize(stream));
diff --git a/krakenuniq_amd/csrc/ku_ctx.h b/krakenuniq_amd/csrc/ku_ctx.h
--- a/krakenuniq_amd/csrc/ku_ctx.h
+++ b/krakenuniq_amd/csrc/ku_ctx.h
@@ -157,6 +157,7 @@
   void *d_table = nullptr;
   uint64_t n_dup = 0;
   uint64_t table_lines = 0;
+  double table_load = 0.0;
   uint32_t *d_pairs = nullptr;
   uint64_t *d_offsets = nullptr;
   KuDbDev db{};
@@ -172,6 +173,8 @@
   bool hash_layout = true;
   double load_factor = 0.2;
   bool load_factor_set = false;
+  int locus_split = -1;
+  bool group_member = false;
   DbStore m;
   std::vector<DbStore> extra;
   std::vector<uint32_t> h_node_taxid, h_slot_taxid;
diff --git a/krakenuniq_amd/csrc/ku_device.h b/krakenuniq_amd/csrc/ku_device.h
--- a/krakenuniq_amd/csrc/ku_device.h
+++ b/krakenuniq_amd/csrc/ku_device.h
@@ -214,9 +214,9 @@
 __device__ __forceinline__ bool ku_line_spilled(uint4 h4) { return (h4.x & 0x8000u) != 0; }
 
 #define KU_FLANK 8
-#ifndef KU_OFFCLASS
-#define KU_OFFCLASS 4
-#endif
+__device__ __forceinline__ uint32_t ku_locus_class(uint32_t side, uint32_t cls) {
+  return (side >> (cls & 31u)) + (uint32_t)(side >= (cls >> 8));
+}
 
 __device__ __forceinline__ uint32_t ku_key_shift(uint32_t m) { return m > 13 ? 2 * m - 26 : 0; }
 #define KU_PK_KEYSHIFT 6
@@ -249,7 +249,7 @@
   return best;
 }
 __device__ __forceinline__ uint64_t ku_locus_assemble(uint64_t canon, uint32_t key, uint32_t a, bool plus, uint32_t k,
-                                                      uint32_t m) {
+                                                      uint32_t m, uint32_t cls) {
   const uint32_t w = k - m + 1;
   const uint32_t ap = plus ? a : w - 1 - a;
   const uint32_t left = ap, right = w - 1 - ap;
@@ -259,9 +259,10 @@
   const uint32_t end = use_r ? ap + m + flen : ap;
   const uint32_t seg = (uint32_t)(canon >> (2 * (plus ? k - end : end - flen))) & ((1u << (2 * flen)) - 1u);
   const uint32_t flank = flen ? (plus ? seg : ku_revcomp32(seg, flen)) : 0u;
-  return ((uint64_t)key << 32) | ((uint64_t)flank << 12) | (flen << 8) | ((side / KU_OFFCLASS) << 1) | (uint32_t)use_r;
-}
-__device__ __forceinline__ uint64_t ku_locus_key(uint64_t c, uint32_t k, uint32_t m, uint32_t xor_mask, uint32_t &bin) {
+  return ((uint64_t)key << 32) | ((uint64_t)flank << 12) | (flen << 8) | ku_locus_class(side, cls) << 1 | (uint32_t)use_r;
+}
+__device__ __forceinline__ uint64_t ku_locus_key(uint64_t c, uint32_t k, uint32_t m, uint32_t xor_mask, uint32_t cls,
+                                                 uint32_t &bin) {
   const uint32_t w = k - m + 1, sh = ku_key_shift(m);
   const uint32_t mask = (1u << (2 * m)) - 1u;
   uint32_t best = 0xFFFFFFFFu, mn = 0xFFFFFFFFu, a = 0;
@@ -277,7 +278,7 @@
     mn = min(mn, v);
   }
   bin = mn;
-  return ku_locus_assemble(c, best, a, plus, k, m);
+  return ku_locus_assemble(c, best, a, plus, k, m, cls);
 }
 __device__ __forceinline__ uint32_t ku_locus_prehash(uint64_t locus) {
   uint32_t g = (uint32_t)locus * 0x9E3779B1u ^ __builtin_rotateleft32((uint32_t)(locus >> 32) * 0x85EBCA77u, 15);
diff --git a/krakenuniq_amd/csrc/ku_internal.h b/krakenuniq_amd/csrc/ku_internal.h
--- a/krakenuniq_amd/csrc/ku_internal.h
+++ b/krakenuniq_amd/csrc/ku_internal.h
@@ -16,8 +16,19 @@
   uint64_t bin_lo, bin_hi;
   uint32_t k, nt;
   uint32_t xor_mask;
-  uint32_t pad;
-};
+  uint32_t cls;
+};
+
+#define KU_CLS_QUARTERS (2u | (255u << 8))
+#define KU_HALVES_MAX_LOAD 0.2
+static inline uint32_t ku_cls_halves(uint32_t w) {
+  const uint32_t base = w / 2, div = (w - base + 1) / 2;
+  return 5u | ((base + div) << 8);
+}
+static inline bool ku_quarters_waste_a_class(uint32_t w) {
+  const uint32_t lo = w / 2, hi = w - 1;
+  return lo / 4 != hi / 4 && ((lo & 3u) == 3u || (hi & 3u) == 0u);
+}
 
 struct KuTaxDev {
   const uint32_t *node_parent;
@@ -151,6 +162,7 @@
 int ku_ctx_device_of(const ku_ctx *ctx);
 int ku_ctx_cus_of(const ku_ctx *ctx);
 uint32_t ku_ctx_k_of(const ku_ctx *ctx);
+void ku_ctx_join_group(ku_ctx *ctx);
 void ku_set_error(const std::string &s);
 
 int ku_launch_lookup(const KuDbDev &db, const KuCountsDev &cnt, const uint8_t *d_seqs, uint64_t n_bytes,
@@ -236,7 +248,7 @@
 int ku_launch_remap_values(uint32_t *d_pairs, uint64_t n_pairs, const uint32_t *d_slot_taxid, uint32_t n_slots,
                            uint32_t *d_err, hipStream_t stream);
 int ku_launch_build_table(const uint32_t *d_pairs, uint64_t n_pairs, void *d_table, uint64_t n_lines, uint32_t k,
-                          uint32_t m, uint32_t xor_mask, unsigned long long *d_spilled, hipStream_t stream);
+                          uint32_t m, uint32_t xor_mask, uint32_t cls, unsigned long long *d_spilled, hipStream_t stream);
 int ku_launch_count_table(const void *d_table, uint64_t n_lines, unsigned long long *d_counts, hipStream_t stream);
 int ku_launch_count_slots(const uint32_t *d_pairs, uint64_t n_pairs, unsigned long long *d_counts,
                           uint32_t n_slots, hipStream_t stream);
diff --git a/krakenuniq_amd/csrc/ku_kernels.hip b/krakenuniq_amd/csrc/ku_kernels.hip
--- a/krakenuniq_amd/csrc/ku_kernels.hip
+++ b/krakenuniq_amd/csrc/ku_kernels.hip
@@ -216,7 +216,7 @@
         if (ok[j]) {
           uint32_t mn = 0xFFFFFFFFu;
           if (PK) {
-            locus[j] = ku_locus_assemble(canon[j], key[j], aoff[j], plus[j], k, m);
+            locus[j] = ku_locus_assemble(canon[j], key[j], aoff[j], plus[j], k, m, db.cls);
             mn = bin_v[j];
           } else {
             for (uint32_t i = 0; i < w; ++i) mn = min(mn, s_mm[p + i]);
@@ -552,13 +552,13 @@
 }
 
 __global__ void ku_build_table_kernel(const uint32_t *__restrict__ pairs, uint64_t n, uint32_t *table, uint64_t n_lines,
-                                      uint32_t k, uint32_t m, uint32_t xor_mask, unsigned long long *n_spilled) {
+                                      uint32_t k, uint32_t m, uint32_t xor_mask, uint32_t cls, unsigned long long *n_spilled) {
   for (uint64_t i = blockIdx.x * (uint64_t)blockDim.x + threadIdx.x; i < n; i += (uint64_t)gridDim.x * blockDim.x) {
     const uint32_t klo = pairs[3 * i], khi = pairs[3 * i + 1], val = pairs[3 * i + 2];
     const uint64_t key = ((uint64_t)khi << 32) | klo;
     const uint32_t tag = ku_table_tag(ku_fmix64(key));
     uint32_t bin;
-    uint64_t line = ku_locus_line(ku_locus_key(key, k, m, xor_mask, bin), n_lines);
+    uint64_t line = ku_locus_line(ku_locus_key(key, k, m, xor_mask, cls, bin), n_lines);
     for (uint32_t hops = 0;; ++hops) {
       uint32_t *lp = table + line * KU_LINE_DWORDS;
       int got = -1;
@@ -584,12 +584,12 @@
   }
 }
 int ku_launch_build_table(const uint32_t *d_pairs, uint64_t n_pairs, void *d_table, uint64_t n_lines, uint32_t k,
-                          uint32_t m, uint32_t xor_mask, unsigned long long *d_spilled, hipStream_t stream) {
+                          uint32_t m, uint32_t xor_mask, uint32_t cls, unsigned long long *d_spilled, hipStream_t stream) {
   if (hipMemsetAsync(d_table, 0, n_lines * 128, stream) != hipSuccess) return KU_EHIP;
   if (n_pairs == 0) return KU_OK;
   uint64_t nb = (n_pairs + 255) / 256;
   hipLaunchKernelGGL(ku_build_table_kernel, dim3((unsigned)(nb < 8192 ? nb : 8192)), dim3(256), 0, stream, d_pairs,
-                     n_pairs, (uint32_t *)d_table, n_lines, k, m, xor_mask, d_spilled);
+                     n_pairs, (uint32_t *)d_table, n_lines, k, m, xor_mask, cls, d_spilled);
   return hipGetLastError() == hipSuccess ? KU_OK : KU_EHIP;
 }
 
diff --git a/krakenuniq_amd/csrc/ku_mgpu.cpp b/krakenuniq_amd/csrc/ku_mgpu.cpp
--- a/krakenuniq_amd/csrc/ku_mgpu.cpp
+++ b/krakenuniq_amd/csrc/ku_mgpu.cpp
@@ -58,6 +58,7 @@
     r.device = devices[i];
     int st = ku_ctx_create(devices[i], &r.ctx);
     if (st != KU_OK) { ku_mgpu_destroy(m); return st; }
+    if (!(flags & KU_MGPU_REPLICAS)) ku_ctx_join_group(r.ctx);
   }
   if (m->use_rccl) {
     int st = rccl_ready();
diff --git a/krakenuniq_amd/csrc/ku_route.hip b/krakenuniq_amd/csrc/ku_route.hip
--- a/krakenuniq_amd/csrc/ku_route.hip
+++ b/krakenuniq_amd/csrc/ku_route.hip
@@ -241,7 +241,7 @@
         const uint32_t t = ok[j] ? anc - pj : 0u;
         const uint32_t aoff = is_fwd ? t : w - 1 - t;
         const bool plus = ((m1 >> (is_fwd ? 16 : 17)) & 1u) != 0;
-        const uint64_t locus = ku_locus_assemble(canon[j], m0 >> 6, aoff, plus, k, m);
+        const uint64_t locus = ku_locus_assemble(canon[j], m0 >> 6, aoff, plus, k, m, db.cls);
         hh[j] = ku_fmix64(canon[j]);
         const uint64_t line = ku_locus_line(locus, db.n_lines);
         lp[j] = tab + (ok[j] ? line : 0) * KU_LINE_DWORDS;
diff --git a/krakenuniq_amd/csrc/ku_short.hip b/krakenuniq_amd/csrc/ku_short.hip
--- a/krakenuniq_amd/csrc/ku_short.hip
+++ b/krakenuniq_amd/csrc/ku_short.hip
@@ -10,6 +10,9 @@
 #define KS_FLOOR_EVERY 64u
 #define KS_HQ 64
 #define KS_PAD 16
+#ifndef KS_LINE_DIET
+#define KS_LINE_DIET 3
+#endif
 #ifdef KU_ABLATION
 #define KS_ABL(bit) ((ablate & (bit)) != 0)
 #else
@@ -606,7 +609,7 @@
       bool act[ITEMS], ovf[ITEMS];
 #pragma unroll
       for (int j = 0; j < ITEMS; ++j) {
-        const uint64_t locus = ku_locus_assemble(canon[j], key[j], aoff[j], plus[j], k, m);
+        const uint64_t locus = ku_locus_assemble(canon[j], key[j], aoff[j], plus[j], k, m, db.cls);
         hh[j] = ku_fmix64(canon[j]);
         const uint64_t line = ku_locus_line(locus, db.n_lines);
         lp[j] = tab + (ok[j] ? line : 0) * KU_LINE_DWORDS;
@@ -617,89 +620,98 @@
       uint4 h4[ITEMS];
 #pragma unroll
       for (int j = 0; j < ITEMS; ++j) h4[j] = *reinterpret_cast<const uint4 *>(lp[j]);
+      constexpr bool DIET_A = (KS_LINE_DIET & 1) && !(WIN && OUT == 1);
       KsQuad q[ITEMS];
-      const uint32_t *ep[ITEMS];
       bool nxt[ITEMS];
       const uint32_t *const tab_end = tab + db.n_lines * KU_LINE_DWORDS;
+      bool live = false;
 #pragma unroll
       for (int j = 0; j < ITEMS; ++j) {
         cand[j] = ku_tag_matches(h4[j], ku_table_tag(hh[j])) & (act[j] ? 0xFFu : 0u);
         ovf[j] = act[j] && ku_line_spilled(h4[j]);
         nxt[j] = ovf[j] && cand[j] == 0;
-        const uint32_t eo = nxt[j] ? (uint32_t)KU_LINE_DWORDS : KU_LINE_ENTRY0 + 3 * (__builtin_ctz(cand[j] | 0x100u) & 7u);
-        ep[j] = lp[j] + eo;
-        if (ep[j] == tab_end) ep[j] = tab;
-      }
-#pragma unroll
-      for (int j = 0; j < ITEMS; ++j) q[j] = *reinterpret_cast<const KsQuad *>(ep[j]);
-      uint32_t sb[ITEMS];
-      if (OUT == 2 && DO_COUNTS) {
-#pragma unroll
-        for (int j = 0; j < ITEMS; ++j)
-          sb[j] = reinterpret_cast<const uint8_t *>(lp[j] + KU_LINE_SEEN0)[__builtin_ctz(cand[j] | 0x100u) & 7u];
-      }
-#pragma unroll
-      for (int j = 0; j < ITEMS; ++j) {
-        const bool hit = cand[j] != 0 && ks_quad_key(q[j]) == canon[j];
-        v[j] = hit ? q[j].z : 0u;
+        live |= cand[j] != 0 || ovf[j];
+      }
+      if (!(KS_LINE_DIET & 2) || __any(live)) {
+        const uint32_t *ep[ITEMS];
+#pragma unroll
+        for (int j = 0; j < ITEMS; ++j) {
+          const uint32_t eo = nxt[j] ? (uint32_t)KU_LINE_DWORDS : KU_LINE_ENTRY0 + 3 * (__builtin_ctz(cand[j] | 0x100u) & 7u);
+          if (DIET_A && cand[j] == 0 && !ovf[j]) lp[j] = tab;
+          ep[j] = lp[j] + eo;
+          if (ep[j] == tab_end) ep[j] = tab;
+        }
+#pragma unroll
+        for (int j = 0; j < ITEMS; ++j) q[j] = *reinterpret_cast<const KsQuad *>(ep[j]);
+        uint32_t sb[ITEMS];
         if (OUT == 2 && DO_COUNTS) {
-          if (hit && !sb[j] && !KS_ABL(128u)) ku_seen_mark(lp[j], (uint32_t)__builtin_ctz(cand[j]));
-        }
-        cand[j] &= cand[j] - 1;
-        act[j] = !hit && (cand[j] != 0 || ovf[j]);
-      }
-      bool any = false;
-#pragma unroll
-      for (int j = 0; j < ITEMS; ++j) any |= act[j];
-      while (any && !KS_ABL(1024u)) {
-        bool pick[ITEMS], taken = false, fresh = false, ov = false;
-        const uint32_t *l = tab;
-        uint32_t cm = 0;
-        uint64_t hsel = 0;
-        KsQuad hq = {0, 0, 0, 0};
+#pragma unroll
+          for (int j = 0; j < ITEMS; ++j)
+            sb[j] = reinterpret_cast<const uint8_t *>(lp[j] + KU_LINE_SEEN0)[__builtin_ctz(cand[j] | 0x100u) & 7u];
+        }
 #pragma unroll
         for (int j = 0; j < ITEMS; ++j) {
-          pick[j] = act[j] && !taken;
-          taken |= act[j];
-          if (pick[j]) { hsel = hh[j]; l = lp[j]; cm = cand[j]; ov = ovf[j]; fresh = nxt[j]; hq = q[j]; }
-        }
-        const uint32_t t = ku_table_tag(hsel);
-        if (fresh) {
-          l += KU_LINE_DWORDS;
-          if (l == tab_end) l = tab;
-        }
-        for (;;) {
-          if (fresh) {
-            cm = ku_tag_matches(ks_quad_header(hq), t);
-            ov = ku_line_spilled(ks_quad_header(hq));
+          const bool hit = cand[j] != 0 && ks_quad_key(q[j]) == canon[j];
+          v[j] = hit ? q[j].z : 0u;
+          if (OUT == 2 && DO_COUNTS) {
+            if (hit && !sb[j] && !KS_ABL(128u)) ku_seen_mark(lp[j], (uint32_t)__builtin_ctz(cand[j]));
           }
-          if (cm == 0 && !ov) break;
-          fresh = cm == 0;
+          cand[j] &= cand[j] - 1;
+          act[j] = !hit && (cand[j] != 0 || ovf[j]);
+        }
+        bool any = false;
+#pragma unroll
+        for (int j = 0; j < ITEMS; ++j) any |= act[j];
+        while (any && !KS_ABL(1024u)) {
+          bool pick[ITEMS], taken = false, fresh = false, ov = false;
+          const uint32_t *l = tab;
+          uint32_t cm = 0;
+          uint64_t hsel = 0;
+          KsQuad hq = {0, 0, 0, 0};
+#pragma unroll
+          for (int j = 0; j < ITEMS; ++j) {
+            pick[j] = act[j] && !taken;
+            taken |= act[j];
+            if (pick[j]) { hsel = hh[j]; l = lp[j]; cm = cand[j]; ov = ovf[j]; fresh = nxt[j]; hq = q[j]; }
+          }
+          const uint32_t t = ku_table_tag(hsel);
           if (fresh) {
             l += KU_LINE_DWORDS;
             if (l == tab_end) l = tab;
           }
-          const uint32_t ei = (uint32_t)__builtin_ctz(cm | 0x100u) & 7u;
-          hq = *reinterpret_cast<const KsQuad *>(fresh ? l : l + KU_LINE_ENTRY0 + 3 * ei);
-          if (!fresh) {
-            cm &= cm - 1;
-            bool same = false;
-#pragma unroll
-            for (int j = 0; j < ITEMS; ++j) same |= pick[j] && ks_quad_key(hq) == canon[j];
-            if (same) {
-#pragma unroll
-              for (int j = 0; j < ITEMS; ++j)
-                if (pick[j]) v[j] = hq.z;
-              if (OUT == 2 && DO_COUNTS && !KS_ABL(128u)) ku_seen_mark(l, ei);
-              break;
+          for (;;) {
+            if (fresh) {
+              cm = ku_tag_matches(ks_quad_header(hq), t);
+              ov = ku_line_spilled(ks_quad_header(hq));
+            }
+            if (cm == 0 && !ov) break;
+            fresh = cm == 0;
+            if (fresh) {
+              l += KU_LINE_DWORDS;
+              if (l == tab_end) l = tab;
+            }
+            const uint32_t ei = (uint32_t)__builtin_ctz(cm | 0x100u) & 7u;
+            hq = *reinterpret_cast<const KsQuad *>(fresh ? l : l + KU_LINE_ENTRY0 + 3 * ei);
+            if (!fresh) {
+              cm &= cm - 1;
+              bool same = false;
+#pragma unroll
+              for (int j = 0; j < ITEMS; ++j) same |= pick[j] && ks_quad_key(hq) == canon[j];
+              if (same) {
+#pragma unroll
+                for (int j = 0; j < ITEMS; ++j)
+                  if (pick[j]) v[j] = hq.z;
+                if (OUT == 2 && DO_COUNTS && !KS_ABL(128u)) ku_seen_mark(l, ei);
+                break;
+              }
             }
           }
-        }
-        any = false;
-#pragma unroll
-        for (int j = 0; j < ITEMS; ++j) {
-          if (pick[j]) act[j] = false;
-          any |= act[j];
+          any = false;
+#pragma unroll
+          for (int j = 0; j < ITEMS; ++j) {
+            if (pick[j]) act[j] = false;
+            any |= act[j];
+          }
         }
       }
 
```
